# liron88/HM-16.2

Hardware: AMD Instinct MI355X
Metric: CTUs/sec (enc) at 4K main10; bit-exact CU partition vs HM (higher is better)
Workload: dtype int32+f64

## Files before the change

### __graft_entry__.py

```python
import os
import subprocess
import sys

ROOT = os.path.dirname(os.path.abspath(__file__))
PKG = os.path.join(ROOT, "hm-16.2_amd")
for p in (ROOT, PKG, os.path.join(ROOT, "oracle")):
    if p not in sys.path:
        sys.path.insert(0, p)


def _newer(target, sources):
    if not os.path.exists(target):
        return True
    t = os.path.getmtime(target)
    return any(os.path.getmtime(s) > t for s in sources)


def build_product():
    src = os.path.join(PKG, "csrc")
    out = os.path.join(PKG, "libhm355.so")
    deps = [os.path.join(src, f) for f in ("hm355.hip", "hm355_core.h", "hm355_inter.h", "hm355_inter_cu.h", "hm355_dbk.h", "hm355_sao.h", "hm355_bits.h", "hm355_bits_kernel.h", "hm355_ingest.h", "hm355_picstat.h", "hm355_types.h", "hm355_host_common.h", "hm355_simt.h", "hm355_simt4.h", "hm355_simt8.h", "hm355_team.h")] + [os.path.join(ROOT, "include", "hm355.h")]
    if _newer(out, deps):
        import hashlib
        h = hashlib.sha1()
        for d in sorted(deps):
            h.update(open(d, "rb").read())
        build_id = h.hexdigest()[:12]
        hipcc = "/opt/rocm/bin/hipcc" if os.path.exists("/opt/rocm/bin/hipcc") else "hipcc"
        cmd = [hipcc, "-O3", "--offload-arch=gfx950", "-ffp-contract=off", "-fPIC", "-shared", "-std=c++17", "-Wno-unused-value", "-Wno-sizeof-array-div",
               f'-DHM355_BUILD_ID="{build_id}"', "-o", out, os.path.join(src, "hm355.hip")]
        subprocess.run(cmd, check=True)
    host = os.path.join(PKG, "host")
    exe = os.path.join(PKG, "hm355_encmain")
    if _newer(exe, [os.path.join(host, f) for f in ("encmain.cpp", "TEncTop.cpp", "TEncTop.h")] + [out]):
        subprocess.run(["g++", "-O2", "-std=c++14", "-Wall", "-o", exe, os.path.join(host, "encmain.cpp"), os.path.join(host, "TEncTop.cpp"),
                        "-L" + PKG, "-lhm355", "-Wl,-rpath,$ORIGIN"], check=True)
    return out


def build_oracle():
    subprocess.run(["make", "-s", "-C", os.path.join(ROOT, "oracle"),
                    os.path.join(ROOT, "oracle", "libhm_oracle.so"), os.path.join(ROOT, "oracle", "hm_oracle_cli")], check=True)
    if os.path.isdir("/root/reference/source"):
        subprocess.run(["make", "-s", "-C", os.path.join(ROOT, "oracle"), "ref"], check=True, stdout=subprocess.DEVNULL)


def build():
    build_product()
    build_oracle()
    import hm355
    hm355.load_library()


def smoke():
    import numpy as np
    import hm355
    import oracle
    import synth
    w, h, bd, qp = 128, 64, 8, 32
    planes = synth.frame(w, h, bd, 0, 1234)
    enc = hm355.Encoder(w, h, bd, 1, 1)
    (rec, ctus, stats), = enc.compress([planes], qp)
    (subs, nxt, bins), = enc.encode_slices_run([dict(slice_type=2, qp=qp)])
    pstat, = enc.picture_stats_run([dict(hash_method=1)])
    enc.close()
    import hashlib
    for k in range(3):
        d = planes[k].astype(np.int64) - rec[k].astype(np.int64)
        assert pstat["ssd"][k] == int((d * d).sum()), "smoke: SSD of the picture statistics differs from numpy"
        assert pstat["digest"][k] == hashlib.md5(rec[k].astype(np.uint8).tobytes()).digest(), "smoke: MD5 of the reconstruction differs from hashlib"
    want_rec, want_ctus = oracle.compress(planes, bd, qp, 1)
    for f in ("total_bits", "total_dist", "depth", "part_size", "intra_dir_luma", "intra_dir_chroma", "tr_idx", "cbf", "coeff_y"):
        assert np.array_equal(ctus[f], want_ctus[f]), f"smoke: {f} differs from the oracle"
    for k in range(3):
        assert np.array_equal(rec[k], want_rec[k]), "smoke: reconstruction differs from the oracle"
    want_subs, want_nxt, want_bins = oracle.encode_slice(w, h, bd, 1, 2, qp, want_ctus)
    assert subs == want_subs and (nxt, bins) == (want_nxt, want_bins), "smoke: slice data differs from the oracle"
    print("smoke ok: 2 CTUs,", int(stats[0]), "bits,", sum(len(x) for x in subs), "bytes of slice data, bit-exact vs oracle;" + pstat["psnr_string"], "MD5", pstat["digest_string"][:32])
    import math
    n = len(ctus)
    mot = np.zeros(n, [("pred_mode", "u1", 256), ("mv0", "<i2", (256, 2)), ("ref_idx0", "i1", 256), ("mv1", "<i2", (256, 2)), ("ref_idx1", "i1", 256)])
    mot["pred_mode"] = 1; mot["ref_idx0"] = -1; mot["ref_idx1"] = -1
    ref_poc = np.zeros((2, 16), np.int32)
    final = {"poc": 0, "slice_type": 2, "rec": rec, "motion": mot, "num_ref_idx": (0, 0), "ref_poc": ref_poc, "ref_long_term": ref_poc}
    lam = 0.578 * 2.0 ** ((qp + 2 - 12) / 3.0) * 2.0
    srec = {"poc": 1, "slice_type": 0, "qp": qp + 2, "lambda": lam, "weight_cb": hm355.intra_lambda(qp + 2)[1], "cabac_init_type": 0,
            "num_ref_idx": (1, 1), "ref_poc": ref_poc, "col_from_l0": 1, "col_ref_idx": 0, "tmvp": 1, "mvd_l1_zero": 1, "max_merge_cand": 5,
            "check_ldc": 1, "lambda_motion_sad": int(math.floor(65536.0 * math.sqrt(lam))), "lambda_motion_sse": int(math.floor(65536.0 * lam))}
    cur = synth.frame(w, h, bd, 1, 1234)
    want_rec, want_ctus, want_ictus = oracle.compress_inter(cur, bd, srec, {0: final}, wpp=1)
    sp = dict(srec); sp["chroma_weight"] = srec["weight_cb"]
    refs = {0: dict(slice_type=2, rec=rec, pred_mode=mot["pred_mode"], mv=[mot["mv0"], mot["mv1"]], ref_idx=[mot["ref_idx0"], mot["ref_idx1"]],
                    num_ref_idx=(0, 0), ref_poc=ref_poc, ref_long_term=ref_poc)}
    enc = hm355.Encoder(w, h, bd, 1, 1)
    brec, bctus, bictus, bstats = enc.compress_inter(cur, sp, refs)
    (bsubs, bnxt, bbins), = enc.encode_slices_run([dict(slice_type=0, qp=qp + 2, cabac_init_type=0, num_ref_idx=(1, 1), mvd_l1_zero=1, max_merge_cand=5)])
    enc.close()
    for f in ("total_bits", "total_dist", "depth", "part_size", "pred_mode", "tr_idx", "cbf", "coeff_y"):
        assert np.array_equal(bctus[f], want_ctus[f]), f"smoke (B slice): {f} differs from the oracle"
    for f in ("skip", "merge_flag", "merge_idx", "inter_dir", "mv", "mvd", "ref_idx", "mvp_idx"):
        assert np.array_equal(bictus[f], want_ictus[f]), f"smoke (B slice): {f} differs from the oracle"
    for k in range(3):
        assert np.array_equal(brec[k], want_rec[k]), "smoke (B slice): reconstruction differs from the oracle"
    want_bsubs, want_bnxt, want_bbins = oracle.encode_slice(w, h, bd, 1, 0, qp + 2, want_ctus, want_ictus, cabac_init_type=0, num_ref_idx=(1, 1), mvd_l1_zero=1, max_merge_cand=5)
    assert bsubs == want_bsubs and (bnxt, bbins) == (want_bnxt, want_bbins), "smoke (B slice): slice data differs from the oracle"
    print("smoke ok: B slice,", int(bstats[0]), "bits,", sum(len(x) for x in bsubs), "bytes of slice data,", int((bictus["inter_dir"] == 3).sum()), "bi-predicted partitions, bit-exact vs oracle")


if __name__ == "__main__":
    build()
    if len(sys.argv) > 1 and sys.argv[1] == "smoke":
        smoke()
```

### hm-16.2_amd/csrc/hm355_core.h

```cpp
#pragma once
#include <stddef.h>
#include "hm355_types.h"

#ifdef HM355_HOSTSIM
#include <string.h>
#include <math.h>
#include <stdlib.h>
#define HM_DEV static
#define HM_FINL static inline
#define HM_FINL_M inline
#define HM_LAMBDA_INL
#define HM_NOINLINE __attribute__((noinline))
#define HM_CONST static const
#define HM_ASSUME_LDS(p) ((void)0)
#define HM_ASSUME_GLB(p) ((void)0)
#define HM_NT 1
static inline int hm_lane() { return 0; }
#define HM_SYNC() ((void)0)
static inline uint32_t hm_wave_sum(uint32_t v) { return v; }
static inline int hm_wave_sum_i(int v) { return v; }
static inline int hm_wave_max_i(int v) { return v; }
#define HM_UNI(x) (x)
#define HM_UCALL(x) (x)
#define hm_uni_ptr(p) (p)
#define hm_uni_struct(v) (v)
#define HM_ENTRY(e) ((void)0)
#define HM_LDS_ADD(p, v) (*(p) += (v))
#ifdef HM355_HOSTSIM_REVERSE
#define HM_PAR_FOR_XY(x, y, w, n) for (int i_ = (n) - 1, y = i_ / (w), x = i_ - y * (w); i_ >= 0; i_--, x--, (x < 0 ? (x = (w) - 1, y--) : 0))
#define HM_PAR_FOR(i, n) for (int i = (n) - 1; i >= 0; i--)
#define HM_WAVE_FOR(k) for (int k = 63; k >= 0; k--)
#else
#define HM_PAR_FOR_XY(x, y, w, n) for (int i_ = 0, y = 0, x = 0; i_ < (n); i_++, x++, (x >= (w) ? (x = 0, y++) : 0))
#define HM_PAR_FOR(i, n) for (int i = 0; i < (n); i++)
#define HM_WAVE_FOR(k) for (int k = 0; k < 64; k++)
#endif
#define HM_LV(T, name) T name[64]
#define HM_LVARG(T, name) const T *name
#define HM_LVK(name, k) name[k]
#define HM_LV_GET(name, i) (name[i])
#define HM_LV_GETD(name, i) (name[i])
#define HM_LV_SET(name, i, v) (name[i] = (v))
#define HM_LV_SETD(name, i, v) (name[i] = (v))
#define HM_LV_GATHER(name, idx) (name[idx])
#define HM_BALLOT(m, k, cond) do { if (cond) (m) |= 1ull << (k); } while (0)
#define HM_ORDERED_ADD16(acc, name) do { for (int k_ = 15; k_ >= 0; k_--) (acc) += name[k_]; } while (0)
#define HM_ORDERED_CHAIN16(acc, a, b, pre) do { for (int k_ = 15; k_ >= 0; k_--) { pre[k_] = (acc); (acc) -= a[k_]; (acc) += b[k_]; } } while (0)
#else
#define HM_DEV __device__
#define HM_FINL __device__ __forceinline__
#define HM_FINL_M __device__ __forceinline__
#define HM_LAMBDA_INL __attribute__((always_inline))
#define HM_NOINLINE __attribute__((noinline))
#define HM_CONST __device__ const
#if defined(__HIP_DEVICE_COMPILE__)
#define HM_ASSUME_LDS(p) __builtin_assume(__builtin_amdgcn_is_shared((const void *)(p)))
#define HM_ASSUME_GLB(p) __builtin_assume(!__builtin_amdgcn_is_shared((const void *)(p)) && !__builtin_amdgcn_is_private((const void *)(p)))
#else
#define HM_ASSUME_LDS(p) ((void)0)
#define HM_ASSUME_GLB(p) ((void)0)
#endif
#define HM_NT 64
__device__ __forceinline__ int hm_lane() { return (int)(threadIdx.x & 63u); }
#define HM_SYNC() do { __builtin_amdgcn_fence(__ATOMIC_RELEASE, "wavefront"); __builtin_amdgcn_wave_barrier(); __builtin_amdgcn_fence(__ATOMIC_ACQUIRE, "wavefront"); } while (0)
template <int CTRL> __device__ __forceinline__ int hm_dpp(int old, int v) { return __builtin_amdgcn_update_dpp(old, v, CTRL, 0xf, 0xf, false); }
__device__ __forceinline__ int hm_wave_sum_i(int v)
{
  v += hm_dpp<0x111>(0, v); v += hm_dpp<0x112>(0, v); v += hm_dpp<0x114>(0, v); v += hm_dpp<0x118>(0, v);
  return __builtin_amdgcn_readlane(v, 15) + __builtin_amdgcn_readlane(v, 31) + __builtin_amdgcn_readlane(v, 47) + __builtin_amdgcn_readlane(v, 63);
}
__device__ __forceinline__ uint32_t hm_wave_sum(uint32_t v) { return (uint32_t)hm_wave_sum_i((int)v); }
__device__ __forceinline__ int hm_wave_max_i(int v)
{
  int t;
  t = hm_dpp<0x111>(v, v); v = t > v ? t : v; t = hm_dpp<0x112>(v, v); v = t > v ? t : v;
  t = hm_dpp<0x114>(v, v); v = t > v ? t : v; t = hm_dpp<0x118>(v, v); v = t > v ? t : v;
  const int a = __builtin_amdgcn_readlane(v, 15), b = __builtin_amdgcn_readlane(v, 31), c = __builtin_amdgcn_readlane(v, 47), d = __builtin_amdgcn_readlane(v, 63);
  const int ab = a > b ? a : b, cd = c > d ? c : d;
  return ab > cd ? ab : cd;
}
#define HM_LDS_ADD(p, v) atomicAdd((p), (v))
#define HM_UNI(x) __builtin_amdgcn_readfirstlane((int)(x))
template <class T> __device__ __forceinline__ T *hm_uni_ptr(T *p)
{
  const unsigned long long v = (unsigned long long)p;
  const unsigned lo = (unsigned)__builtin_amdgcn_readfirstlane((int)(unsigned)v), hi = (unsigned)__builtin_amdgcn_readfirstlane((int)(unsigned)(v >> 32));
  return (T *)(((unsigned long long)hi << 32) | lo);
}
template <class T> __device__ __forceinline__ T hm_uni_struct(T v)
{
  static_assert(sizeof(T) % 4 == 0, "dword-sized aggregates only");
  int w[sizeof(T) / 4];
  __builtin_memcpy(w, &v, sizeof(T));
#pragma unroll
  for (unsigned i = 0; i < sizeof(T) / 4; i++) w[i] = __builtin_amdgcn_readfirstlane(w[i]);
  __builtin_memcpy(&v, w, sizeof(T));
  return v;
}
#define HM_ENTRY(e) do { (e) = hm_uni_ptr(e); HM_ASSUME_LDS(e); } while (0)
#define HM_UCALL(x) ((uint32_t)__builtin_amdgcn_readfirstlane((int)(x)))
#define HM_PAR_FOR(i, n) for (int i = hm_lane(); i < (n); i += HM_NT)
#define HM_PAR_FOR_XY(x, y, w, n) \
  for (int i_ = hm_lane(), sy_ = HM_NT / (w), sx_ = HM_NT - sy_ * (w), y = i_ / (w), x = i_ - y * (w); i_ < (n); \
       i_ += HM_NT, x += sx_, y += sy_, (x >= (w) ? (x -= (w), y++) : 0))
#define HM_WAVE_FOR(k) for (int k = hm_lane(), k##_once = 1; k##_once; k##_once = 0)
#define HM_LV(T, name) T name
#define HM_LVARG(T, name) const T name
#define HM_LVK(name, k) name
#define HM_LV_GET(name, i) __builtin_amdgcn_readlane((int)(name), (int)(i))
#define HM_LV_GETD(name, i) hm_readlane_d((name), (int)(i))
#define HM_LV_SET(name, i, v) ((name) = (hm_lane() == (int)(i)) ? (v) : (name))
#define HM_LV_SETD(name, i, v) ((name) = (hm_lane() == (int)(i)) ? (v) : (name))
#define HM_LV_GATHER(name, idx) __builtin_amdgcn_ds_bpermute((int)(idx) << 2, (int)(name))
#define HM_BALLOT(m, k, cond) ((m) = __ballot(cond))
#define HM_ORDERED_ADD16(acc, name) do { _Pragma("unroll") for (int k_ = 15; k_ >= 0; k_--) (acc) += hm_readlane_d((name), k_); } while (0)
#define HM_ORDERED_CHAIN16(acc, a, b, pre) do { _Pragma("unroll") for (int k_ = 15; k_ >= 0; k_--) { \
    (pre) = (hm_lane() == k_) ? (acc) : (pre); (acc) -= hm_readlane_d((a), k_); (acc) += hm_readlane_d((b), k_); } } while (0)
__device__ __forceinline__ double hm_readlane_d(double v, int i)
{ return __hiloint2double(__builtin_amdgcn_readlane(__double2hiint(v), i), __builtin_amdgcn_readlane(__double2loint(v), i)); }
#endif

#if defined(HM355_PROFILE) && !defined(HM355_HOSTSIM)
#define HM_PROF_N 44
#define HM_PROF_BEGIN(e, id) const unsigned long long prof_t0_##id = __builtin_readcyclecounter()
#define HM_PROF_END(e, id) do { (e)->prof[id] += __builtin_readcyclecounter() - prof_t0_##id; (e)->profCnt[id] += 1; } while (0)
#else
#define HM_PROF_BEGIN(e, id) ((void)0)
#define HM_PROF_END(e, id) ((void)0)
#endif
enum { PR_RDOQ = 0, PR_BITS, PR_ADI, PR_PRED, PR_FWD, PR_INV, PR_SATD35, PR_TUBLK, PR_SAVE, PR_CHROMA, PR_LUMA, PR_ENCCU, PR_TOTAL,
       PR_S4L = 32, PR_S4C, PR_D0, PR_D1, PR_D2, PR_D3, PR_NXN, PR_S8L, PR_S4LEAF, PR_S4CLEAF, PR_S8C,
       PR_ME_INT = 16, PR_ME_FRAC, PR_AMVP, PR_MRG_EST, PR_MC, PR_IRQ, PR_IRES, PR_MRG2N, PR_INTERCU, PR_INTRA_IN_P, PR_IQ_FULL, PR_IQ_FWD, PR_IQ_RDOQ, PR_IQ_BITS, PR_IQ_INV, PR_IQ_ENC };

#define HM_MAX_DOUBLE 1.7e+308
#define PLANAR_IDX 0
#define DC_IDX 1
#define HOR_IDX 10
#define VER_IDX 26
#define DM_CHROMA_IDX 36
#define SIZE_2Nx2N 0
#define SIZE_NxN 3
#define SIZE_NONE 8
#define MODE_INTRA 1
#define MODE_NONE 2
#define SCAN_DIAG 0
#define SCAN_HOR 1
#define SCAN_VER 2

HM_CONST uint8_t HM_NEXT_LPS[128] __attribute__((aligned(4))) = {
  1, 0, 0, 1, 2, 3, 4, 5, 4, 5, 8, 9, 8, 9, 10, 11, 12, 13, 14, 15, 16, 17, 18, 19, 18, 19, 22, 23, 22, 23, 24, 25,
  26, 27, 26, 27, 30, 31, 30, 31, 32, 33, 32, 33, 36, 37, 36, 37, 38, 39, 38, 39, 42, 43, 42, 43, 44, 45, 44, 45, 46, 47, 48, 49,
  48, 49, 50, 51, 52, 53, 52, 53, 54, 55, 54, 55, 56, 57, 58, 59, 58, 59, 60, 61, 60, 61, 60, 61, 62, 63, 64, 65, 64, 65, 66, 67,
  66, 67, 66, 67, 68, 69, 68, 69, 70, 71, 70, 71, 70, 71, 72, 73, 72, 73, 72, 73, 74, 75, 74, 75, 74, 75, 76, 77, 76, 77, 126, 127 };
HM_CONST int32_t HM_ENTROPY_BITS[128] = {
  0x07b23, 0x085f9, 0x074a0, 0x08cbc, 0x06ee4, 0x09354, 0x067f4, 0x09c1b, 0x060b0, 0x0a62a, 0x05a9c, 0x0af5b, 0x0548d, 0x0b955, 0x04f56, 0x0c2a9,
  0x04a87, 0x0cbf7, 0x045d6, 0x0d5c3, 0x04144, 0x0e01b, 0x03d88, 0x0e937, 0x039e0, 0x0f2cd, 0x03663, 0x0fc9e, 0x03347, 0x10600, 0x03050, 0x10f95,
  0x02d4d, 0x11a02, 0x02ad3, 0x12333, 0x0286e, 0x12cad, 0x02604, 0x136df, 0x02425, 0x13f48, 0x021f4, 0x149c4, 0x0203e, 0x1527b, 0x01e4d, 0x15d00,
  0x01c99, 0x166de, 0x01b18, 0x17017, 0x019a5, 0x17988, 0x01841, 0x18327, 0x016df, 0x18d50, 0x015d9, 0x19547, 0x0147c, 0x1a083, 0x0138e, 0x1a8a3,
  0x01251, 0x1b418, 0x01166, 0x1bd27, 0x01068, 0x1c77b, 0x00f7f, 0x1d18e, 0x00eda, 0x1d91a, 0x00e19, 0x1e254, 0x00d4f, 0x1ec9a, 0x00c90, 0x1f6e0,
  0x00c01, 0x1fef8, 0x00b5f, 0x208b1, 0x00ab6, 0x21362, 0x00a15, 0x21e46, 0x00988, 0x2285d, 0x00934, 0x22ea8, 0x008a8, 0x239b2, 0x0081d, 0x24577,
  0x007c9, 0x24ce6, 0x00763, 0x25663, 0x00710, 0x25e8f, 0x006a0, 0x26a26, 0x00672, 0x26f23, 0x005e8, 0x27ef8, 0x005ba, 0x284b5, 0x0055e, 0x29057,
  0x0050c, 0x29bab, 0x004c1, 0x2a674, 0x004a7, 0x2aa5e, 0x0046f, 0x2b32f, 0x0041f, 0x2c0ad, 0x003e7, 0x2ca8d, 0x003ba, 0x2d323, 0x0010c, 0x3bfbb };
HM_CONST uint8_t HM_CTX_INIT_I[HM_NUM_CTX] = {
   139, 141, 157,
   184, 154, 154, 154,
   184,
   63, 139,
   153, 138, 138,
   111, 141, 154, 154, 154,   94, 138, 182, 154, 154,
   91, 171, 134, 141,
   111, 111, 125, 110, 110, 94, 124, 108, 124, 107, 125, 141, 179, 153, 125, 107, 125, 141, 179, 153, 125, 107, 125, 141, 179, 153, 125, 141,
   140, 139, 182, 182, 152, 136, 152, 136, 153, 136, 139, 111, 136, 139, 111, 111,
   110, 110, 124, 125, 140, 153, 125, 127, 140, 109, 111, 143, 127, 111, 79,  108, 123, 63, 154, 154, 154, 154, 154, 154, 154, 154, 154, 154, 154, 154,
   110, 110, 124, 125, 140, 153, 125, 127, 140, 109, 111, 143, 127, 111, 79,  108, 123, 63, 154, 154, 154, 154, 154, 154, 154, 154, 154, 154, 154, 154,
   140, 92, 137, 138, 140, 152, 138, 139, 153, 74, 149, 92, 139, 107, 122, 152,  140, 179, 166, 182, 140, 227, 122, 197,
   138, 153, 136, 167, 152, 152,
   139, 139,
   154, 154, 154,  154, 154,  154,  154, 154, 154, 154, 154,  154, 154,
   154, 154,  154,  154,  154, 154, 154
};
HM_CONST uint8_t HM_CTX_INIT_P[HM_NUM_CTX] = {
   107, 139, 126,
   154, 139, 154, 154,
   154,
   152, 139,
   124, 138, 94,
   153, 111, 154, 154, 154,   149, 107, 167, 154, 154,
   121, 140, 61, 154,
   155, 154, 139, 153, 139, 123, 123, 63, 153, 166, 183, 140, 136, 153, 154, 166, 183, 140, 136, 153, 154, 166, 183, 140, 136, 153, 154, 140,
   170, 153, 123, 123, 107, 121, 107, 121, 167, 151, 183, 140, 151, 183, 140, 140,
   125, 110, 94, 110, 95, 79, 125, 111, 110, 78, 110, 111, 111, 95, 94,  108, 123, 108, 154, 154, 154, 154, 154, 154, 154, 154, 154, 154, 154, 154,
   125, 110, 94, 110, 95, 79, 125, 111, 110, 78, 110, 111, 111, 95, 94,  108, 123, 108, 154, 154, 154, 154, 154, 154, 154, 154, 154, 154, 154, 154,
   154, 196, 196, 167, 154, 152, 167, 182, 182, 134, 149, 136, 153, 121, 136, 137,  169, 194, 166, 167, 154, 167, 137, 182,
   107, 167, 91, 122, 107, 167,
   139, 139,
   197, 185, 201,  110, 122,  149,  95, 79, 63, 31, 31,  140, 198,
   153, 153,  79,  168,  154, 154, 154
};
HM_CONST uint8_t HM_CTX_INIT_B[HM_NUM_CTX] = {
   107, 139, 126,
   154, 139, 154, 154,
   183,
   152, 139,
   224, 167, 122,
   153, 111, 154, 154, 154,   149, 92, 167, 154, 154,
   121, 140, 61, 154,
   170, 154, 139, 153, 139, 123, 123, 63, 124, 166, 183, 140, 136, 153, 154, 166, 183, 140, 136, 153, 154, 166, 183, 140, 136, 153, 154, 140,
   170, 153, 138, 138, 122, 121, 122, 121, 167, 151, 183, 140, 151, 183, 140, 140,
   125, 110, 124, 110, 95, 94, 125, 111, 111, 79, 125, 126, 111, 111, 79,  108, 123, 93, 154, 154, 154, 154, 154, 154, 154, 154, 154, 154, 154, 154,
   125, 110, 124, 110, 95, 94, 125, 111, 111, 79, 125, 126, 111, 111, 79,  108, 123, 93, 154, 154, 154, 154, 154, 154, 154, 154, 154, 154, 154, 154,
   154, 196, 167, 167, 154, 152, 167, 182, 182, 134, 149, 136, 153, 121, 136, 122,  169, 208, 166, 167, 154, 152, 167, 182,
   107, 167, 91, 107, 107, 167,
   139, 139,
   197, 185, 201,  154, 137,  134,  95, 79, 63, 31, 31,  169, 198,
   153, 153,  79,  168,  154, 154, 154
};
HM_CONST int8_t HM_DCT_C[33] = {64, 90, 90, 90, 89, 88, 87, 85, 83, 82, 80, 78, 75, 73, 70, 67, 64, 61, 57, 54, 50, 46, 43, 38, 36, 31, 25, 22, 18, 13, 9, 4, 0};
HM_CONST int8_t HM_DST4[16] = {29, 55, 74, 84, 74, 74, 0, -74, 84, -29, -74, 55, 55, -84, 74, -29};
HM_CONST int32_t HM_QUANT_SCALES[6] = {26214, 23302, 20560, 18396, 16384, 14564};
HM_CONST int32_t HM_INV_QUANT_SCALES[6] = {40, 45, 51, 57, 64, 72};
HM_CONST uint8_t HM_GROUP_IDX[32] = {0,1,2,3,4,4,5,5,6,6,6,6,7,7,7,7,8,8,8,8,8,8,8,8,9,9,9,9,9,9,9,9};
HM_CONST uint8_t HM_CTX_IND_MAP_4x4[16] = {0,1,4,5, 2,3,4,5, 6,6,8,8, 7,7,8,8};
HM_CONST uint8_t HM_INTRA_MODE_NUM_FAST[6] = {3, 8, 8, 3, 3, 3};
HM_CONST uint8_t HM_INTRA_FILTER[5] = {10, 7, 1, 0, 10};
HM_CONST int8_t HM_ANG_TABLE[9] = {0, 2, 5, 9, 13, 17, 21, 26, 32};
HM_CONST int16_t HM_INV_ANG_TABLE[9] = {0, 4096, 1638, 910, 630, 482, 390, 315, 256};

struct TU {
  int16_t cuParts, parts, cParts, cOff;
  uint8_t cuZ, cuDepth, relZ, trDepth, log2, section, x, y;
  uint8_t cW, cCodeAll, cTrDepth, cRelZ, cx, cy, pad_[2];
};
static_assert(sizeof(TU) == 24, "TU layout");
struct TuWalk { TU node[5]; int8_t next[5]; int sp; };
struct RqtFrame {
  TU t; int8_t phase, child, checkFull, checkSplit, bestModeId; uint32_t singleDist, singleCbf, splitDist, splitCbf, singleBits; double singleCost, splitCost;
};
struct CuFrame { int16_t cuZ; int8_t phase, sub, boundary, parentPart, ampSens, pad_; double bestCost, splitCost; uint32_t bestBits, bestDist, splitBits, splitDist; };
struct MvFieldD { MvD mv; int ref; };
struct MergeList { MvFieldD f[5][2]; uint8_t dir[5]; int num; };
struct AmvpInfo { MvD cand[3]; int n; };
struct TZ {
  const Pel *org; int orgStride, w, h;
  const Pel *ref; int refStride;
  uint32_t bestSad; int bestX, bestY, bestDist, bestRound, pointNr;
  int16_t l, r, t, b;
  int16_t subShift, pad_;
  int16_t lx[16], ly[16]; int8_t lp[16], ld[16];
  int16_t wx0, wy0, ww, wh;
};
struct IrqFrame {
  TU t; int8_t phase, child, checkFull, checkSplit, zero; uint8_t bestTS[3];
  uint32_t absSum[3], bestCBF[3], singleBits, singleDist, subBits, subDist; double singleCost, subCost;
};

#define HM_TSTRIDE 33
#define HM_RQ_LDS 256
struct RqLds {
  int32_t lvl[HM_RQ_LDS];
  uint16_t pos[HM_RQ_LDS];
  uint16_t dec[HM_RQ_LDS];
  int16_t cur[HM_RQ_LDS];
  uint8_t ctxSig[HM_RQ_LDS];
  uint8_t code[HM_RQ_LDS];
  uint8_t cgCtxSet[64];
  uint8_t cgFlag[64];
};
struct RefLds {
  Pel refTop[2][132], refLeft[2][132];
  Pel refMain[200], refSide[200];
  Pel line[272];
};
#define HM_SLOT(d, ci) ((d) * CI_NUM + (ci) - ((d) == 4 ? 2 : 0))
#define HM_NUM_SLOTS (4 * CI_NUM + 3)
struct Team;
#define HM_CTU_WAVES 12
struct LdsTables {
  int8_t tmat[32 * HM_TSTRIDE];
  int8_t dst4[16];
  int32_t ebits[128];
};
#if defined(HM355_HOSTSIM)
static LdsTables g_lt;
#else
__shared__ LdsTables g_lt;
#endif
#define HM_LT() (&g_lt)
struct Shared {
  Cabac cur;
  int32_t bufA[32 * HM_TSTRIDE];
  union {
    int32_t bufB[32 * HM_TSTRIDE];
    RqLds rq;
    RefLds ref;
  } u;
  TuWalk walkOuter, walkInner;
  CuFrame cuf[4];
  double outCost; uint32_t outBits, outDist; double outRdCost;
  int32_t mpmZ;
  int32_t s8Winner, s8Reuse;
  InterMeta *im;
  uint32_t mcost; MvD mvPredictor; int32_t costScale;
  union {
    struct {
      uint8_t flags[72];
      RqtFrame rqt[4]; uint32_t rqtRetDist[5], rqtRetBits[5]; double rqtRetCost[5];
      int32_t rdModeList[12];
      uint32_t outDistY;
      uint32_t satd[36];
      int32_t mpmNum, mpmPreds[3];
    };
    struct {
      int32_t absCoeff[10];
      TZ tz; MvD outMv; MergeList ml; AmvpInfo amvp; MvFieldD mrgField[2]; int32_t mrgDir, mrgIdx; uint32_t mrgCost, irqZeroDist;
      IrqFrame irq[4];
    };
  };
  int32_t width, height, bitDepth, wCtu, stride[3];
  const Params *P; FrameBuf fb; WorkSpace *ws; const Tables *tab;
  CtuMeta meta;
  TCoeff *cc;
  int32_t ctuX, ctuY, ctuAddr;
#if defined(HM355_PROFILE) && !defined(HM355_HOSTSIM)
  unsigned long long prof[HM_PROF_N]; unsigned long long profCnt[HM_PROF_N];
#endif
};

#if defined(HM355_TRACE) && defined(HM355_HOSTSIM)
#include <stdio.h>
static FILE *g_hm_trace;
#define HM_TRACE(e, tag, a, b, c) do { if (g_hm_trace) fprintf(g_hm_trace, "%d %d %u %u %.3f\n", (int)(tag), (e)->ctuAddr, (unsigned)(a), (unsigned)(b), (double)(c)); } while (0)
#elif defined(HM355_TRACE)
#define HM_TRACE_CAP (1u << 21)
__device__ inline void hm_trace(Shared *e, int tag, uint32_t a, uint32_t b, double c)
{
  if (hm_lane() == 0) {
    unsigned long long *t = e->P->prof; const unsigned long long n = atomicAdd(t, 1ull);
    if (n < HM_TRACE_CAP) { t[1 + n * 3] = ((unsigned long long)(uint32_t)tag << 32) | (uint32_t)e->ctuAddr; t[2 + n * 3] = ((unsigned long long)a << 32) | b; t[3 + n * 3] = (unsigned long long)__double_as_longlong(c); }
  }
}
#define HM_TRACE(e, tag, a, b, c) hm_trace((e), (tag), (uint32_t)(a), (uint32_t)(b), (double)(c))
#else
#define HM_TRACE(e, tag, a, b, c) ((void)0)
#endif

#ifndef HM355_HOSTSIM
__shared__ Shared g_sh;
__shared__ Shared g_shs[HM_CTU_WAVES];
#endif
#if !defined(HM355_PROFILE)
static_assert(HM_CTU_WAVES * (sizeof(Shared) + 16) + sizeof(LdsTables) <= 163840 / (12 / HM_CTU_WAVES) && sizeof(Shared) % 8 == 0, "two workgroups of HM_CTU_WAVES searches (+ work items, + the shared tables) per CU: 12 CTU searches in 160 KB of LDS");
#endif
static_assert(offsetof(Shared, bufA) % 8 == 0 && (16 * HM_TSTRIDE * 4) % 8 == 0, "the RDOQ cost array aliases the lower half of bufA as doubles");
static_assert(offsetof(Shared, u) == offsetof(Shared, bufA) + sizeof(((Shared *)0)->bufA), "the motion search stages its reference window across bufA and the union behind it");
#define HM_TZ_WIN_SAMPLES ((int)((sizeof(((Shared *)0)->bufA) + sizeof(((Shared *)0)->u)) / sizeof(Pel)))

HM_DEV inline int hm_clip3(int lo, int hi, int v) { return v < lo ? lo : (v > hi ? hi : v); }
HM_DEV inline int hm_abs(int v) { return v < 0 ? -v : v; }
HM_DEV inline int hm_z2r(int z)
{
  const int x = (z & 1) | ((z >> 1) & 2) | ((z >> 2) & 4) | ((z >> 3) & 8);
  const int y = ((z >> 1) & 1) | ((z >> 2) & 2) | ((z >> 3) & 4) | ((z >> 4) & 8);
  return (y << 4) | x;
}
HM_DEV inline int hm_spread4(int v) { return (v & 1) | ((v & 2) << 1) | ((v & 4) << 2) | ((v & 8) << 3); }
HM_DEV inline int hm_r2z(int r) { return hm_spread4(r & 15) | (hm_spread4(r >> 4) << 1); }
HM_DEV inline int hm_log2(int n) { return n >= 64 ? 6 : (n >= 32 ? 5 : (n >= 16 ? 4 : (n >= 8 ? 3 : 2))); }

HM_DEV inline void par_set8(uint8_t *p, int v, int n) { HM_PAR_FOR(i, n) p[i] = (uint8_t)v; HM_SYNC(); }
HM_DEV inline void par_copy8(uint8_t *d, const uint8_t *s, int n) { HM_PAR_FOR(i, n) d[i] = s[i]; HM_SYNC(); }
HM_DEV inline void par_copy32(TCoeff *d, const TCoeff *s, int n) { HM_PAR_FOR(i, n) d[i] = s[i]; HM_SYNC(); }
HM_DEV inline void par_zero32(TCoeff *d, int n) { HM_PAR_FOR(i, n) d[i] = 0; HM_SYNC(); }
HM_DEV inline void par_copy_blk(Pel *d, int ds, const Pel *s, int ss, int n)
{
  const int l2 = hm_log2(n);
  HM_PAR_FOR(i, n * n) { const int y = i >> l2, x = i & (n - 1); d[y * ds + x] = s[y * ss + x]; }
  HM_SYNC();
}

HM_DEV inline void cabac_copy(Cabac *d, const Cabac *s)
{
  const uint64_t *sp = (const uint64_t *)s; uint64_t *dp = (uint64_t *)d;
  HM_PAR_FOR(i, (int)(sizeof(Cabac) / 8)) dp[i] = sp[i];
  HM_SYNC();
}
#if defined(HM355_HOSTSIM)
typedef Cabac CabacHold;
static inline CabacHold cabac_hold(const Cabac *s) { return *s; }
static inline void cabac_put(Cabac *d, const CabacHold &h) { *d = h; }
#else
typedef uint64_t CabacHold;
__device__ __forceinline__ CabacHold cabac_hold(const Cabac *s)
{ const int l = hm_lane(); return l < (int)(sizeof(Cabac) / 8) ? ((const uint64_t *)s)[l] : 0ull; }
__device__ __forceinline__ void cabac_put(Cabac *d, CabacHold h)
{ const int l = hm_lane(); if (l < (int)(sizeof(Cabac) / 8)) ((uint64_t *)d)[l] = h; HM_SYNC(); }
#endif
HM_DEV inline void cabac_init(Cabac *c, int qp, int initType = 2)
{
  qp = hm_clip3(0, 51, qp);
  HM_PAR_FOR(i, HM_NUM_CTX) {
    const int iv = initType == 2 ? HM_CTX_INIT_I[i] : (initType == 1 ? HM_CTX_INIT_P[i] : HM_CTX_INIT_B[i]);
    const int slope = (iv >> 4) * 5 - 45, offset = ((iv & 15) << 3) - 16;
    int st = ((slope * qp) >> 4) + offset; st = st < 1 ? 1 : (st > 126 ? 126 : st);
    const int mps = st >= 64;
    c->s[i] = (uint8_t)(((mps ? (st - 64) : (63 - st)) << 1) + mps);
  }
  c->frac = 0;
  HM_SYNC();
}
HM_DEV inline int hm_next_state(int st, int bin) { return bin == (st & 1) ? (st < 124 ? st + 2 : st) : HM_NEXT_LPS[st]; }
HM_DEV inline void enc_bin(const Shared *e, Cabac *c, int ctx, int bin)
{
  const int st = c->s[ctx];
  c->frac += (uint64_t)HM_LT()->ebits[st ^ bin];
  c->s[ctx] = hm_next_state(st, bin);
}
HM_DEV inline void enc_ep(Cabac *c, int n) { c->frac += (uint64_t)32768 * (uint64_t)n; }
HM_DEV inline void enc_trm(const Shared *e, Cabac *c, int bin) { c->frac += (uint64_t)HM_ENTROPY_BITS[126 ^ bin]; }
HM_DEV inline void reset_bits(Cabac *c) { c->frac &= 32767; }
HM_DEV inline uint32_t num_bits(const Cabac *c) { return (uint32_t)(c->frac >> 15); }

HM_DEV inline double calc_rd_cost(const Shared *e, uint32_t bits, uint32_t dist)
{
  const double t = (double)bits * e->fb.lambda;
  const double u = (double)dist + t;
  return floor(u + 0.5);
}

struct Rect;
template <class C> HM_DEV inline void code_skip_flag(Shared *e, C *c, int z);

HM_DEV inline uint32_t dist_sse(const Pel *org, int so, const Pel *cur, int sc, int n, int bitDepth)
{
  const int shift = (bitDepth - 8) << 1, l2 = hm_log2(n);
  uint32_t sum = 0;
  HM_PAR_FOR(i, n * n) { const int y = i >> l2, x = i & (n - 1); const int d = org[y * so + x] - cur[y * sc + x]; sum += (uint32_t)((d * d) >> shift); }
  return hm_wave_sum(sum);
}
HM_DEV inline uint32_t had8(const Pel *org, int so, const Pel *cur, int sc)
{
  int d[64];
#pragma unroll
  for (int y = 0; y < 8; y++)
#pragma unroll
    for (int x = 0; x < 8; x++) d[y * 8 + x] = org[y * so + x] - cur[y * sc + x];
#pragma unroll
  for (int y = 0; y < 8; y++) {
#pragma unroll
    for (int len = 1; len < 8; len <<= 1)
#pragma unroll
      for (int b = 0; b < 8; b += len << 1)
#pragma unroll
        for (int k = 0; k < len; k++) { const int a0 = d[y * 8 + b + k], a1 = d[y * 8 + b + k + len]; d[y * 8 + b + k] = a0 + a1; d[y * 8 + b + k + len] = a0 - a1; }
  }
  uint32_t s = 0;
#pragma unroll
  for (int x = 0; x < 8; x++) {
#pragma unroll
    for (int len = 1; len < 8; len <<= 1)
#pragma unroll
      for (int b = 0; b < 8; b += len << 1)
#pragma unroll
        for (int k = 0; k < len; k++) { const int a0 = d[(b + k) * 8 + x], a1 = d[(b + k + len) * 8 + x]; d[(b + k) * 8 + x] = a0 + a1; d[(b + k + len) * 8 + x] = a0 - a1; }
#pragma unroll
    for (int y = 0; y < 8; y++) s += (uint32_t)hm_abs(d[y * 8 + x]);
  }
  return (s + 2) >> 2;
}
HM_DEV inline uint32_t had4(const Pel *org, int so, const Pel *cur, int sc)
{
  int d[16];
#pragma unroll
  for (int y = 0; y < 4; y++)
#pragma unroll
    for (int x = 0; x < 4; x++) d[y * 4 + x] = org[y * so + x] - cur[y * sc + x];
#pragma unroll
  for (int y = 0; y < 4; y++) {
    const int a = d[y * 4] + d[y * 4 + 1], b = d[y * 4] - d[y * 4 + 1], c = d[y * 4 + 2] + d[y * 4 + 3], e = d[y * 4 + 2] - d[y * 4 + 3];
    d[y * 4] = a + c; d[y * 4 + 1] = b + e; d[y * 4 + 2] = a - c; d[y * 4 + 3] = b - e;
  }
  uint32_t s = 0;
#pragma unroll
  for (int x = 0; x < 4; x++) {
    const int a = d[x] + d[4 + x], b = d[x] - d[4 + x], c = d[8 + x] + d[12 + x], e = d[8 + x] - d[12 + x];
    s += (uint32_t)(hm_abs(a + c) + hm_abs(b + e) + hm_abs(a - c) + hm_abs(b - e));
  }
  return (s + 1) >> 1;
}
HM_DEV inline uint32_t dist_hads(const Pel *org, int so, const Pel *cur, int sc, int n, int bitDepth)
{
  uint32_t sum = 0; const int l2 = hm_log2(n);
  if (n >= 8) { const int nb = n >> 3; HM_PAR_FOR(b, nb * nb) { const int by = b >> (l2 - 3), bx = b & (nb - 1); sum += had8(org + by * 8 * so + bx * 8, so, cur + by * 8 * sc + bx * 8, sc); } }
  else { HM_PAR_FOR(b, 1) sum += had4(org, so, cur, sc); }
  return hm_wave_sum(sum) >> (bitDepth - 8);
}
HM_DEV inline uint32_t dist_sad(const Pel *org, int so, const Pel *cur, int sc, int n, int subShift, int bitDepth)
{
  const int l2 = hm_log2(n), rows = n >> subShift;
  uint32_t sum = 0;
  HM_PAR_FOR(i, rows * n) { const int y = (i >> l2) << subShift, x = i & (n - 1); sum += (uint32_t)hm_abs(org[y * so + x] - cur[y * sc + x]); }
  return (hm_wave_sum(sum) << subShift) >> (bitDepth - 8);
}

HM_DEV inline void load_tables()
{
  HM_PAR_FOR(i, 1024) {
    const int k = i >> 5, n = i & 31, m = (k * (2 * n + 1)) & 127;
    int v;
    if (m <= 32) v = HM_DCT_C[m]; else if (m <= 64) v = -HM_DCT_C[64 - m]; else if (m <= 96) v = -HM_DCT_C[m - 64]; else v = HM_DCT_C[128 - m];
    HM_LT()->tmat[k * HM_TSTRIDE + n] = (int8_t)v;
  }
  HM_PAR_FOR(i, 16) HM_LT()->dst4[i] = HM_DST4[i];
  HM_PAR_FOR(i, 128) HM_LT()->ebits[i] = HM_ENTROPY_BITS[i];
  HM_SYNC();
}
HM_DEV inline int tm(const Shared *e, int n, int dst, int k, int j) { return dst ? HM_LT()->dst4[k * 4 + j] : HM_LT()->tmat[(k * (32 / n)) * HM_TSTRIDE + j]; }

HM_DEV inline void fold_rows(int32_t *X, int n, int l2)
{
  const int h = n >> 1, q = n >> 2;
  HM_PAR_FOR(o, n * q) {
    const int j = o >> (l2 - 2), i = o & (q - 1);
    int32_t *r = X + j * HM_TSTRIDE;
    const int32_t a = r[i], b = r[n - 1 - i], c = r[h - 1 - i], d = r[h + i];
    r[i] = a + b; r[h + i] = a - b; r[h - 1 - i] = c + d; r[n - 1 - i] = c - d;
  }
  HM_SYNC();
}
HM_DEV HM_NOINLINE void fwd_transform(Shared *e, int n, int useDst, int bitDepth)
{
  HM_ENTRY(e); n = HM_UNI(n); useDst = HM_UNI(useDst); bitDepth = HM_UNI(bitDepth);
  const int l2 = hm_log2(n), s1 = l2 + bitDepth + 6 - 15, s2 = l2 + 6;
  const int a1 = s1 > 0 ? 1 << (s1 - 1) : 0, a2 = 1 << (s2 - 1);
  int32_t *A = e->bufA, *B = e->u.bufB;
  if (useDst) {
    HM_PAR_FOR(o, n * n) {
      const int j = o >> l2, k = o & (n - 1);
      int32_t acc = 0;
      for (int i = 0; i < n; i++) acc += tm(e, n, 1, k, i) * A[j * HM_TSTRIDE + i];
      B[k * HM_TSTRIDE + j] = (acc + a1) >> s1;
    }
    HM_SYNC();
    HM_PAR_FOR(o, n * n) {
      const int j = o >> l2, k = o & (n - 1);
      int32_t acc = 0;
      for (int i = 0; i < n; i++) acc += tm(e, n, 1, k, i) * B[j * HM_TSTRIDE + i];
      A[k * HM_TSTRIDE + j] = (acc + a2) >> s2;
    }
    HM_SYNC();
    return;
  }
  const int h = n >> 1, step = 32 / n;
  fold_rows(A, n, l2);
  HM_PAR_FOR(o, n * n) {
    const int j = o >> l2, k = o & (n - 1);
    const int32_t *x = A + j * HM_TSTRIDE + ((k & 1) ? h : 0); const int8_t *t = HM_LT()->tmat + (k * step) * HM_TSTRIDE;
    int32_t acc = 0;
    for (int i = 0; i < h; i++) acc += t[i] * x[i];
    B[k * HM_TSTRIDE + j] = (acc + a1) >> s1;
  }
  HM_SYNC();
  fold_rows(B, n, l2);
  HM_PAR_FOR(o, n * n) {
    const int j = o >> l2, k = o & (n - 1);
    const int32_t *x = B + j * HM_TSTRIDE + ((k & 1) ? h : 0); const int8_t *t = HM_LT()->tmat + (k * step) * HM_TSTRIDE;
    int32_t acc = 0;
    for (int i = 0; i < h; i++) acc += t[i] * x[i];
    A[k * HM_TSTRIDE + j] = (acc + a2) >> s2;
  }
  HM_SYNC();
}
HM_DEV HM_NOINLINE void inv_transform(Shared *e, int n, int useDst, int bitDepth)
{
  HM_ENTRY(e); n = HM_UNI(n); useDst = HM_UNI(useDst); bitDepth = HM_UNI(bitDepth);
  const int l2 = hm_log2(n), s1 = 7, s2 = 20 - bitDepth;
  int32_t *A = e->bufA, *B = e->u.bufB;
  if (useDst) {
    HM_PAR_FOR(o, n * n) {
      const int j = o >> l2, i = o & (n - 1);
      int32_t acc = 0;
      for (int k = 0; k < n; k++) acc += tm(e, n, 1, k, i) * A[k * HM_TSTRIDE + j];
      B[j * HM_TSTRIDE + i] = hm_clip3(-32768, 32767, (acc + (1 << (s1 - 1))) >> s1);
    }
    HM_SYNC();
    HM_PAR_FOR(o, n * n) {
      const int j = o >> l2, i = o & (n - 1);
      int32_t acc = 0;
      for (int k = 0; k < n; k++) acc += tm(e, n, 1, k, i) * B[k * HM_TSTRIDE + j];
      A[j * HM_TSTRIDE + i] = hm_clip3(-32768, 32767, (acc + (1 << (s2 - 1))) >> s2);
    }
    HM_SYNC();
    return;
  }
  const int h = n >> 1, step = 32 / n;
  HM_PAR_FOR(o, n * h) {
    const int j = o >> (l2 - 1), i = o & (h - 1);
    int32_t ev = 0, od = 0;
    for (int k = 0; k < n; k += 2) { ev += HM_LT()->tmat[(k * step) * HM_TSTRIDE + i] * A[k * HM_TSTRIDE + j]; od += HM_LT()->tmat[((k + 1) * step) * HM_TSTRIDE + i] * A[(k + 1) * HM_TSTRIDE + j]; }
    B[j * HM_TSTRIDE + i] = hm_clip3(-32768, 32767, (ev + od + (1 << (s1 - 1))) >> s1);
    B[j * HM_TSTRIDE + n - 1 - i] = hm_clip3(-32768, 32767, (ev - od + (1 << (s1 - 1))) >> s1);
  }
  HM_SYNC();
  HM_PAR_FOR(o, n * h) {
    const int j = o >> (l2 - 1), i = o & (h - 1);
    int32_t ev = 0, od = 0;
    for (int k = 0; k < n; k += 2) { ev += HM_LT()->tmat[(k * step) * HM_TSTRIDE + i] * B[k * HM_TSTRIDE + j]; od += HM_LT()->tmat[((k + 1) * step) * HM_TSTRIDE + i] * B[(k + 1) * HM_TSTRIDE + j]; }
    A[j * HM_TSTRIDE + i] = hm_clip3(-32768, 32767, (ev + od + (1 << (s2 - 1))) >> s2);
    A[j * HM_TSTRIDE + n - 1 - i] = hm_clip3(-32768, 32767, (ev - od + (1 << (s2 - 1))) >> s2);
  }
  HM_SYNC();
}

HM_DEV inline TU tu_root(const Shared *e, int cuZ, int cuDepth)
{
  TU t;
  t.cuZ = (int16_t)cuZ; t.cuDepth = (int16_t)cuDepth; t.cuParts = (int16_t)(256 >> (2 * cuDepth));
  t.relZ = 0; t.trDepth = 0; t.log2 = (int16_t)(6 - cuDepth); t.parts = t.cuParts; t.section = 0;
  const int r = hm_z2r(cuZ);
  t.x = (int16_t)((r & 15) * 4); t.y = (int16_t)((r >> 4) * 4);
  t.cW = (int16_t)(1 << (t.log2 - 1)); t.cCodeAll = 1; t.cTrDepth = 0; t.cRelZ = 0; t.cParts = t.parts; t.cOff = (int16_t)(cuZ * 4);
  t.cx = t.x >> 1; t.cy = t.y >> 1;
  return t;
}
HM_DEV inline TU tu_child(const TU *p, int section, int processLast)
{
  TU t = *p;
  t.log2 = p->log2 - 1; t.trDepth = p->trDepth + 1; t.parts = p->parts >> 2; if (t.parts < 1) t.parts = 1;
  t.relZ = (int16_t)(p->relZ + section * t.parts); t.section = (int16_t)section;
  t.x = (int16_t)(p->x + (section & 1) * (1 << t.log2)); t.y = (int16_t)(p->y + (section >> 1) * (1 << t.log2));
  if (t.log2 >= 3) {
    t.cW = (int16_t)(1 << (t.log2 - 1)); t.cCodeAll = 1; t.cTrDepth = t.trDepth; t.cRelZ = t.relZ; t.cParts = t.parts;
    t.cOff = (int16_t)((t.cuZ + t.relZ) * 4); t.cx = t.x >> 1; t.cy = t.y >> 1;
  } else {
    t.cCodeAll = 0; t.cTrDepth = p->cTrDepth; t.cRelZ = t.relZ & ~3; t.cParts = (int16_t)(t.parts * 4);
    t.cOff = p->cOff; t.cx = p->cx; t.cy = p->cy;
    t.cW = (section == (processLast ? 3 : 0)) ? 4 : 0;
  }
  return t;
}
template <class Enter, class Leave> HM_FINL void tu_walk(TuWalk &w, const TU *root, int processLast, Enter enter, Leave leave)
{
  w.node[0] = *root; w.next[0] = -1; w.sp = 0;
  while (w.sp >= 0) {
    TU *t = &w.node[w.sp];
    if (w.next[w.sp] < 0) { if (!enter((const TU *)t)) { w.sp--; continue; } w.next[w.sp] = 0; }
    if (w.next[w.sp] == 4) { leave((const TU *)t); w.sp--; continue; }
    const int s = w.next[w.sp]++;
    w.node[w.sp + 1] = tu_child(t, s, processLast); w.next[w.sp + 1] = -1; w.sp++;
  }
}
template <class Enter> HM_FINL void tu_walk(TuWalk &w, const TU *root, int processLast, Enter enter) { tu_walk(w, root, processLast, enter, [](const TU *) {}); }

HM_DEV inline const CtuMeta *meta_at(const Shared *e, int x4, int y4, int *z)
// ... 853 lines not shown
    HM_LV(int32_t, vCtx); HM_LV(int32_t, vAbs);
    uint64_t nz = 0, g1 = 0, g2 = 0, ng = 0;
    HM_WAVE_FOR(k) {
      const int kk = k & 15, sp = subPos + kk;
      const int a = (kk <= top) ? hm_abs((int)lv[sp]) : 0;
      if (real) HM_BALLOT(ng, k, kk <= top && lv[sp] < 0 && k < 16);
      HM_LVK(vAbs, k) = a;
      HM_LVK(vCtx, k) = sig_ctx_inc(pattern, firstCtx, sposArr[sp], log2n, chroma);
      HM_BALLOT(nz, k, a != 0 && k < 16); HM_BALLOT(g1, k, a > 1 && k < 16); HM_BALLOT(g2, k, a > 2 && k < 16);
    }
    HM_BPROF(PR_SATD35);
    {
      int seen = isLastSet ? 1 : 0;
      for (int p = isLastSet ? top - 1 : 15; p >= 0; p--) {
        const int sig = (int)((nz >> p) & 1);
        if (p > 0 || subSet == 0 || seen) enc_bin(e, &r, sigOff + HM_LV_GET(vCtx, p), sig);
        seen += sig;
      }
    }
    HM_BPROF(PR_TUBLK);
    const int numNonZero = __builtin_popcountll(nz);
    if (numNonZero > 0) {
      const int lastNZ = 63 - __builtin_clzll(nz), firstNZ = __builtin_ctzll(nz);
      const int signHidden = (lastNZ - firstNZ >= 4);
      const int ctxSet = ctx_set_index(chroma, subSet, c1 == 0);
      c1 = 1;
      int firstC2 = -1, escape = 0, idx = 0;
      for (uint64_t m = nz; m && idx < 8; idx++) {
        const int p = 63 - __builtin_clzll(m); m &= ~(1ull << p);
        const int sym = (int)((g1 >> p) & 1);
        enc_bin(e, &r, C_ONE + 4 * ctxSet + c1, sym);
        if (sym) { c1 = 0; if (firstC2 == -1) firstC2 = p; else escape = 1; }
        else if (c1 < 3 && c1 > 0) c1++;
      }
      if (c1 == 0 && firstC2 != -1) { const int sym = (int)((g2 >> firstC2) & 1); enc_bin(e, &r, C_ABS + ctxSet, sym); if (sym) escape = 1; }
      escape = escape || (numNonZero > 8);
      uint32_t signs = 0;
      if (real) { for (uint64_t m = nz; m;) { const int p = 63 - __builtin_clzll(m); m &= ~(1ull << p); signs = (signs << 1) | (uint32_t)((ng >> p) & 1); } if (signHidden) signs >>= 1; }
      enc_epv(&r, signs, signHidden ? numNonZero - 1 : numNonZero);
      if (escape) {
        int firstCoeff2 = 1; uint32_t goRice = 0; idx = 0;
        for (uint64_t m = nz; m; idx++) {
          const int p = 63 - __builtin_clzll(m); m &= ~(1ull << p);
          const int a = HM_LV_GET(vAbs, p);
          const int baseLevel = (idx < 8) ? (2 + firstCoeff2) : 1;
          if (a >= baseLevel) {
            uint32_t sym = (uint32_t)(a - baseLevel);
            if (sym < (3u << goRice)) { const uint32_t len = sym >> goRice; enc_epv(&r, (((1u << (len + 1)) - 2) << goRice) | (sym & ((1u << goRice) - 1)), (int)(len + 1 + goRice)); }
            else { sym -= (3u << goRice); const uint32_t len = coef_remain_suffix(&sym, goRice);
                   if (real) { enc_epv(&r, (1u << (3 + len + 1 - goRice)) - 2, (int)(3 + len + 1 - goRice)); enc_epv(&r, sym, (int)len); }
                   else enc_epv(&r, 0, (int)(3 + len + 1 - goRice + len)); }
            if ((uint32_t)a > (3u << goRice)) goRice = goRice + 1 < 4 ? goRice + 1 : 4;
          }
          if (a >= 2) firstCoeff2 = 0;
        }
      }
    }
    HM_BPROF(PR_CHROMA);
  }
  cabr_store(r, c);
#if defined(HM355_PROFILE) && !defined(HM355_HOSTSIM)
  if (real) { e->prof[PR_FWD] += __builtin_readcyclecounter() - profT0; e->profCnt[PR_FWD] += 1; }
#endif
}


template <class C> HM_DEV inline void code_intra_dir_luma(Shared *e, C *c, int z, int multiple)
{
  const CtuMeta *m = (&e->meta);
  const int partNum = multiple ? (m->part[z] == SIZE_NxN ? 4 : 1) : 1;
  const int partOffset = (256 >> (m->depth[z] << 1)) >> 2;
  int predIdx[4] = {-1, -1, -1, -1};
  for (int j = 0; j < partNum; j++) {
    int preds[3];
    const int dir = m->dirL[z + partOffset * j];
    if (!multiple && z == e->mpmZ) { preds[0] = e->mpmPreds[0]; preds[1] = e->mpmPreds[1]; preds[2] = e->mpmPreds[2]; }
    else intra_dir_predictor(e, z + partOffset * j, preds);
    for (int i = 0; i < 3; i++) if (dir == preds[i]) predIdx[j] = i;
    enc_bin(e, c, C_INTRA_LUMA, predIdx[j] != -1);
  }
  for (int j = 0; j < partNum; j++) {
    if (predIdx[j] != -1) { if (predIdx[j]) enc_epv(c, 2u | (uint32_t)(predIdx[j] - 1), 2); else enc_epv(c, 0, 1); }
    else {
      uint32_t rem = 0;
      if (EngOf<C>::REAL) {
        int p[3]; intra_dir_predictor(e, z + partOffset * j, p);
        int d = m->dirL[z + partOffset * j];
        rem = (uint32_t)(d - (d > p[0]) - (d > p[1]) - (d > p[2]));
      }
      enc_epv(c, rem, 5);
    }
  }
}
template <class C> HM_DEV inline void code_intra_dir_chroma(Shared *e, C *c, int z)
{
  if ((&e->meta)->dirC[z] == DM_CHROMA_IDX) enc_bin(e, c, C_CHROMA_PRED, 0);
  else {
    enc_bin(e, c, C_CHROMA_PRED, 1);
    uint32_t idx = 0;
    if (EngOf<C>::REAL) {
      const int luma = (&e->meta)->dirL[z], dc = (&e->meta)->dirC[z];
      const int list[4] = { PLANAR_IDX, VER_IDX, HOR_IDX, DC_IDX };
      for (int i = 3; i >= 0; i--) if ((list[i] == luma ? 34 : list[i]) == dc) idx = (uint32_t)i;
    }
    enc_epv(c, idx, 2);
  }
}
template <class C> HM_DEV inline void code_qt_cbf(Shared *e, C *c, const TU *t, int comp, int lowestLevel)
{
  const int z = t->cuZ + (comp ? t->cRelZ : t->relZ);
  const int ctx = comp ? t->trDepth : (t->trDepth == 0 ? 1 : 0);
  const int width = comp ? (1 << (t->log2 - 1)) : (1 << t->log2);
  const int canQuadSplit = width >= 8;
  const int lowestTUDepth = t->trDepth + ((!lowestLevel && !canQuadSplit) ? 1 : 0);
  enc_bin(e, c, C_QT_CBF + (comp ? 5 : 0) + ctx, ((&e->meta)->cbf[comp][z] >> lowestTUDepth) & 1);
}

HM_DEV inline int tr_min_size_in_cu(int cuLog2, int nxn)
{
  if (cuLog2 < 2 + 3 - 1 + nxn) return 2;
  const int v = cuLog2 - (3 - 1 + nxn);
  return v > 5 ? 5 : v;
}
HM_DEV inline int codes_subdiv_flag(const CtuMeta *m, const TU *t, int intra)
{
  const int nxn = intra && m->part[t->cuZ] == SIZE_NxN;
  if (nxn && t->trDepth == 0) return 0;
  if (t->log2 > 5) return 0;
  if (t->log2 == 2) return 0;
  if (t->log2 == tr_min_size_in_cu(6 - t->cuDepth, nxn)) return 0;
  return 1;
}
template <class C> HM_DEV inline void code_chroma_cbfs(Shared *e, C *c, const TU *t, int subdiv)
{
  const CtuMeta *m = (&e->meta); const int z = t->cuZ + t->relZ;
  for (int comp = 1; comp < 3; comp++)
    if (t->trDepth == 0 || (t->cCodeAll && ((m->cbf[comp][z] >> (t->trDepth - 1)) & 1))) code_qt_cbf(e, c, t, comp, subdiv == 0);
}
template <class C> HM_DEV inline void code_tu_coeff(Shared *e, C *c, const TU *t, int comp, const TCoeff *planes, int intra)
{
  const CtuMeta *m = (&e->meta); const int z = t->cuZ + t->relZ;
  if ((comp && !t->cW) || !((m->cbf[comp][z] >> t->trDepth) & 1)) return;
  const int n = comp ? t->cW : (1 << t->log2), zc = t->cuZ + (comp ? t->cRelZ : t->relZ);
  const TCoeff *coef = planes + HM_PLANE_OFF(comp) + (comp ? t->cOff : z * 16);
  code_coeff_nxn(e, c, coef, n, comp, intra ? coef_scan_idx(m, zc, n, comp) : SCAN_DIAG, m->ts[comp][zc]);
}

template <class C> HM_DEV inline void enc_subdiv_cbf_qt(Shared *e, C *c, const TU *root, int bLuma, int bChroma)
{
  const CtuMeta *m = (&e->meta);
  tu_walk(e->walkInner, root, 0, [&](const TU *t) {
    const int subdiv = m->tr[t->cuZ + t->relZ] > t->trDepth;
    if (bLuma && codes_subdiv_flag(m, t, 1)) enc_bin(e, c, C_SUBDIV + (5 - t->log2), subdiv);
    if (bChroma) code_chroma_cbfs(e, c, t, subdiv);
    if (!subdiv && bLuma) code_qt_cbf(e, c, t, 0, 1);
    return subdiv;
  });
}
HM_DEV inline void enc_coeff_qt(Shared *e, const TU *root, int comp)
{
  const CtuMeta *m = (&e->meta);
  tu_walk(e->walkInner, root, 0, [&](const TU *t) {
    if (m->tr[t->cuZ + t->relZ] > t->trDepth) return 1;
    code_tu_coeff(e, &e->cur, t, comp, e->ws->qtCoef[5 - t->log2], 1);
    return 0;
  });
}
template <class C> HM_DEV inline void enc_intra_header(Shared *e, C *c, const TU *t, int bLuma, int bChroma)
{
  const CtuMeta *m = (&e->meta); const int relZ = t->relZ;
  if (bLuma) {
    if (relZ == 0 && e->im) { code_skip_flag(e, c, t->cuZ); enc_bin(e, c, C_PRED_MODE, 1); }
    if (relZ == 0 && t->cuDepth == 3) enc_bin(e, c, C_PART, m->part[t->cuZ] == SIZE_2Nx2N);
    if (m->part[t->cuZ] == SIZE_2Nx2N) { if (relZ == 0) code_intra_dir_luma(e, c, t->cuZ, 0); }
    else { const int q = t->cuParts >> 2; if (t->trDepth > 0 && (relZ & (q - 1)) == 0) code_intra_dir_luma(e, c, t->cuZ + relZ, 0); }
  }
  if (bChroma && relZ == 0) code_intra_dir_chroma(e, c, t->cuZ + relZ);
}
HM_DEV HM_NOINLINE uint32_t intra_bits_qt(Shared *e, TU tv, int bLuma, int bChroma)
{
  HM_ENTRY(e); bLuma = HM_UNI(bLuma); bChroma = HM_UNI(bChroma); tv = hm_uni_struct(tv);
  const TU *t = &tv;
  HM_PROF_BEGIN(e, PR_BITS);
  {
    CabacR r; cabr_load(e, r, &e->cur);
    r.frac &= 32767;
    enc_intra_header(e, &r, t, bLuma, bChroma);
    enc_subdiv_cbf_qt(e, &r, t, bLuma, bChroma);
    cabr_store(r, &e->cur);
  }
  if (bLuma) enc_coeff_qt(e, t, 0);
  if (bChroma) { enc_coeff_qt(e, t, 1); enc_coeff_qt(e, t, 2); }
  HM_PROF_END(e, PR_BITS);
  return num_bits(&e->cur);
}

HM_DEV HM_NOINLINE uint32_t intra_coding_tu_block(Shared *e, TU tv, int comp, int save1load2)
{
  HM_ENTRY(e); comp = HM_UNI(comp); save1load2 = HM_UNI(save1load2); tv = hm_uni_struct(tv);
  const TU *t = &tv;
  CtuMeta *m = (&e->meta); WorkSpace *ws = e->ws;
  if (comp && !t->cW) return 0;
  const int n = comp ? t->cW : (1 << t->log2), l2 = hm_log2(n);
  const int relZ = comp ? t->cRelZ : t->relZ, z = t->cuZ + relZ;
  const int bx = comp ? t->cx : t->x, by = comp ? t->cy : t->y;
  const int st = HM_PLANE_STRIDE(comp), po = HM_PLANE_OFF(comp);
  const int layer = 5 - t->log2, parts = comp ? t->cParts : t->parts;
  const int ps = e->stride[comp], bitDepth = e->bitDepth;
  const Pel *org = e->fb.org[comp] + (e->ctuY * st + by) * ps + e->ctuX * st + bx;
  Pel *recPic = e->fb.rec[comp] + (e->ctuY * st + by) * ps + e->ctuX * st + bx;
  Pel *pred = ws->pred + po + by * st + bx, *resi = ws->resi + po + by * st + bx;
  Pel *recQt = ws->qtRec[layer] + po + by * st + bx;
  TCoeff *coef = ws->qtCoef[layer] + po + (comp ? t->cOff : z * 16);
  const int tskip = m->ts[comp][z];
  int mode = comp ? m->dirC[z] : m->dirL[z];
  if (comp && mode == DM_CHROMA_IDX) mode = m->dirL[z & ~3];
  if (save1load2 != 2) {
    const int filt = use_filtered_refs(comp, mode, n);
    const int r = hm_z2r(z);
    { HM_PROF_BEGIN(e, PR_ADI); init_adi_pattern(e, comp, e->ctuX * st + bx, e->ctuY * st + by, n, e->ctuX * 16 + (r & 15), e->ctuY * 16 + (r >> 4), comp ? n / 2 : n / 4, filt); HM_PROF_END(e, PR_ADI); }
    { HM_PROF_BEGIN(e, PR_PRED); pred_intra(e, comp, mode, n, filt, pred, st); HM_PROF_END(e, PR_PRED); }
    if (save1load2 == 1) { HM_PAR_FOR(i, 16) e->ws->tsPred[comp][i] = pred[(i >> 2) * st + (i & 3)]; HM_SYNC(); }
  } else { HM_PAR_FOR(i, 16) pred[(i >> 2) * st + (i & 3)] = e->ws->tsPred[comp][i]; HM_SYNC(); }
  if (comp == 0) par_set8(m->tr + z, t->trDepth, parts);
  const int tshift = 15 - bitDepth - l2;
  HM_PAR_FOR(i, n * n) {
    const int y = i >> l2, x = i & (n - 1);
    const int r = org[y * ps + x] - pred[y * st + x];
    resi[y * st + x] = (Pel)r;
    e->bufA[y * HM_TSTRIDE + x] = tskip ? r * (1 << tshift) : r;
  }
  HM_SYNC();
  { HM_PROF_BEGIN(e, PR_FWD); if (!tskip) fwd_transform(e, n, comp == 0 && n == 4, bitDepth); HM_PROF_END(e, PR_FWD); }
  const int cbfCtx = comp ? 5 + t->trDepth : (t->trDepth == 0 ? 1 : 0);
  HM_PROF_BEGIN(e, PR_RDOQ);
  const int absSum = rdoq_is_empty(e, n, comp) ? 0 : (int)HM_UCALL(rdoq(e, coef, n, comp, coef_scan_idx(m, z, n, comp), cbfCtx));
  HM_PROF_END(e, PR_RDOQ);
#if defined(HM355_PROFILE) && !defined(HM355_HOSTSIM)
  { const int pid = l2 == 2 ? (absSum ? 13 : 7) : (l2 == 3 ? 14 : (l2 == 4 ? 15 : 43)); e->prof[pid] += __builtin_readcyclecounter() - prof_t0_PR_RDOQ; e->profCnt[pid] += 1; }
#endif
  par_set8(m->cbf[comp] + z, (absSum > 0 ? 1 : 0) << t->trDepth, parts);
  HM_PROF_BEGIN(e, PR_INV);
  if (absSum > 0) {
    const int rightShift = 6 - (tshift + e->fb.qpPer[comp != 0]);
    const int scale = HM_INV_QUANT_SCALES[e->fb.qpRem[comp != 0]];
    int tgt = 25 + rightShift; if (tgt > 16) tgt = 16;
    const int imin = -(1 << (tgt - 1)), imax = (1 << (tgt - 1)) - 1;
    HM_PAR_FOR(i, n * n) {
      const int y = i >> l2, x = i & (n - 1);
      const int c = hm_clip3(imin, imax, coef[i]);
      int v;
      if (rightShift > 0) v = (c * scale + (1 << (rightShift - 1))) >> rightShift;
      else v = (int)((unsigned)(c * scale) << (-rightShift));
      e->bufA[y * HM_TSTRIDE + x] = hm_clip3(-32768, 32767, v);
    }
    HM_SYNC();
    if (!tskip) inv_transform(e, n, comp == 0 && n == 4, bitDepth);
    const int off = tshift == 0 ? 0 : (1 << (tshift - 1));
    HM_PAR_FOR(i, n * n) {
      const int y = i >> l2, x = i & (n - 1);
      const int v = e->bufA[y * HM_TSTRIDE + x];
      resi[y * st + x] = (Pel)(tskip ? ((v + off) >> tshift) : v);
    }
  } else {
    HM_PAR_FOR(i, n * n) { const int y = i >> l2, x = i & (n - 1); coef[i] = 0; resi[y * st + x] = 0; }
  }
  HM_SYNC();
  HM_PROF_END(e, PR_INV);
  const int maxv = (1 << bitDepth) - 1, shiftSse = (bitDepth - 8) << 1;
  uint32_t sse = 0;
  HM_PAR_FOR(i, n * n) {
    const int y = i >> l2, x = i & (n - 1);
    const int r = hm_clip3(0, maxv, pred[y * st + x] + resi[y * st + x]);
    pred[y * st + x] = (Pel)r; recQt[y * st + x] = (Pel)r; recPic[y * ps + x] = (Pel)r;
    const int d = org[y * ps + x] - r; sse += (uint32_t)((d * d) >> shiftSse);
  }
  uint32_t d = hm_wave_sum(sse);
  HM_SYNC();
  if (comp) d = (uint32_t)(e->fb.chromaWeight * (double)d);
  return d;
}

HM_DEV inline void store_intra_result_qt(Shared *e, const TU *t, int comp)
{
  const int st = HM_PLANE_STRIDE(comp), po = HM_PLANE_OFF(comp), layer = 5 - t->log2;
  const int bx = comp ? t->cx : t->x, by = comp ? t->cy : t->y;
  const TCoeff *coef = e->ws->qtCoef[layer] + po + (comp ? t->cOff : (t->cuZ + t->relZ) * 16);
  const Pel *rq = e->ws->qtRec[layer] + po + by * st + bx;
  HM_PAR_FOR(i, 16) { e->ws->tsCoef[comp][i] = coef[i]; e->ws->tsRec[comp][i] = rq[(i >> 2) * st + (i & 3)]; }
  HM_SYNC();
}
HM_DEV inline void load_intra_result_qt(Shared *e, const TU *t, int comp)
{
  const int st = HM_PLANE_STRIDE(comp), po = HM_PLANE_OFF(comp), layer = 5 - t->log2, ps = e->stride[comp];
  const int bx = comp ? t->cx : t->x, by = comp ? t->cy : t->y;
  TCoeff *coef = e->ws->qtCoef[layer] + po + (comp ? t->cOff : (t->cuZ + t->relZ) * 16);
  Pel *rq = e->ws->qtRec[layer] + po + by * st + bx;
  Pel *recPic = e->fb.rec[comp] + (e->ctuY * st + by) * ps + e->ctuX * st + bx;
  HM_PAR_FOR(i, 16) { coef[i] = e->ws->tsCoef[comp][i]; const Pel v = e->ws->tsRec[comp][i]; rq[(i >> 2) * st + (i & 3)] = v; recPic[(i >> 2) * ps + (i & 3)] = v; }
  HM_SYNC();
}

HM_DEV HM_NOINLINE void simt4_luma_leaf(Shared *e, TU tv);
HM_DEV HM_NOINLINE void simt8_luma_winner_as_single_tu(Shared *e, TU tv);
HM_DEV HM_NOINLINE void recur_intra_coding_qt(Shared *e, TU rootv, int checkFirst)
{
  HM_ENTRY(e); checkFirst = HM_UNI(checkFirst); rootv = hm_uni_struct(rootv);
  CtuMeta *m = (&e->meta);
  RqtFrame *fr = e->rqt; int sp = 0;
  uint32_t *retDist = e->rqtRetDist, *retBits = e->rqtRetBits; double *retCost = e->rqtRetCost;
  fr[0].t = rootv; fr[0].phase = 0; retDist[0] = 0; retBits[0] = 0; retCost[0] = 0.0;
  while (sp >= 0) {
    RqtFrame *f = &fr[sp]; const TU *t = &f->t;
    const int z = t->cuZ + t->relZ, fullDepth = t->cuDepth + t->trDepth, log2 = t->log2;
    if (f->phase == 0) {
      const int nxn = m->part[t->cuZ] == SIZE_NxN;
      f->checkFull = log2 <= 5;
      f->checkSplit = log2 > tr_min_size_in_cu(6 - t->cuDepth, nxn);
      if (checkFirst && f->checkFull) f->checkSplit = 0;
      f->singleCost = HM_MAX_DOUBLE; f->singleDist = 0; f->singleCbf = 0; f->bestModeId = 0; f->singleBits = 0;
      const int checkTS = (log2 == 2) && (m->part[z] == SIZE_NxN);
      if (f->checkFull) {
        if (checkTS) {
          cabac_copy(&e->ws->slot[HM_SLOT(fullDepth, CI_QT_TRAFO_ROOT)], &e->cur);
          for (int modeId = 0; modeId < 2; modeId++) {
            double costTmp;
            par_set8(m->ts[0] + z, modeId, t->parts);
            const uint32_t distTmp = HM_UCALL(intra_coding_tu_block(e, *t, 0, modeId == 0 ? 1 : 2));
            const uint32_t cbfTmp = (m->cbf[0][z] >> t->trDepth) & 1;
            if (modeId == 1 && cbfTmp == 0) costTmp = HM_MAX_DOUBLE;
            else { const uint32_t bits = HM_UCALL(intra_bits_qt(e, *t, 1, 0)); costTmp = calc_rd_cost(e, bits, distTmp); }
            if (costTmp < f->singleCost) {
              f->singleCost = costTmp; f->singleDist = distTmp; f->singleCbf = cbfTmp; f->bestModeId = (int8_t)modeId;
              if (modeId == 0) { store_intra_result_qt(e, t, 0); cabac_copy(&e->ws->slot[HM_SLOT(fullDepth, CI_TEMP_BEST)], &e->cur); }
            }
            if (modeId == 0) cabac_copy(&e->cur, &e->ws->slot[HM_SLOT(fullDepth, CI_QT_TRAFO_ROOT)]);
          }
          par_set8(m->ts[0] + z, f->bestModeId, t->parts);
          if (f->bestModeId == 0) {
            load_intra_result_qt(e, t, 0);
            par_set8(m->cbf[0] + z, (int)(f->singleCbf << t->trDepth), t->parts);
            cabac_copy(&e->cur, &e->ws->slot[HM_SLOT(fullDepth, CI_TEMP_BEST)]);
          }
        } else if (log2 == 2 && e->P->fewWaves) {
          par_set8(m->ts[0] + z, 0, t->parts);
          HM_PROF_BEGIN(e, PR_S4LEAF);
          simt4_luma_leaf(e, *t);
          HM_PROF_END(e, PR_S4LEAF);
          f->singleDist = e->outDistY; f->singleBits = e->outBits;
          f->singleCost = calc_rd_cost(e, e->outBits, f->singleDist);
        } else if (sp == 0 && e->s8Reuse == 1) {
          e->s8Reuse = 0;
          cabac_copy(&e->ws->slot[HM_SLOT(fullDepth, CI_QT_TRAFO_ROOT)], &e->cur);
          par_set8(m->ts[0] + z, 0, t->parts);
          par_set8(m->tr + z, t->trDepth, t->parts);
          simt8_luma_winner_as_single_tu(e, *t);
          f->singleDist = e->outDistY; f->singleCbf = e->outDist;
          par_set8(m->cbf[0] + z, (int)(f->singleCbf << t->trDepth), t->parts);
          f->singleCost = calc_rd_cost(e, e->outBits, f->singleDist);
        } else if (sp == 0 && e->s8Reuse == 2) {
          e->s8Reuse = 0;
          cabac_copy(&e->ws->slot[HM_SLOT(fullDepth, CI_QT_TRAFO_ROOT)], &e->cur);
          par_set8(m->ts[0] + z, 0, t->parts);
          par_set8(m->tr + z, t->trDepth, t->parts);
          {
            const int n = 1 << log2, layer = 5 - log2;
            par_copy32(e->ws->qtCoef[layer] + z * 16, e->cc + z * 16, n * n);
            par_copy_blk(e->ws->qtRec[layer] + t->y * 64 + t->x, 64, e->ws->reco + t->y * 64 + t->x, 64, n);
          }
          f->singleCbf = e->ws->tmpCbf[0][0] & 1;
          par_set8(m->cbf[0] + z, (int)(f->singleCbf << t->trDepth), t->parts);
          f->singleDist = e->outDistY; f->singleCost = e->outRdCost;
          cabac_copy(&e->cur, &e->ws->slot[HM_SLOT(fullDepth, CI_QT_TRAFO_TEST)]);
        } else {
          if (f->checkSplit) cabac_copy(&e->ws->slot[HM_SLOT(fullDepth, CI_QT_TRAFO_ROOT)], &e->cur);
          par_set8(m->ts[0] + z, 0, t->parts);
          f->singleDist = HM_UCALL(intra_coding_tu_block(e, *t, 0, 0));
          if (f->checkSplit) f->singleCbf = (m->cbf[0][z] >> t->trDepth) & 1;
          const uint32_t bits = HM_UCALL(intra_bits_qt(e, *t, 1, 0));
          f->singleCost = calc_rd_cost(e, bits, f->singleDist); f->singleBits = bits;
        }
      }
      if (!f->checkSplit) { retDist[sp] += f->singleDist; retBits[sp] += f->singleBits; retCost[sp] += f->singleCost; sp--; continue; }
      if (f->checkFull) { cabac_copy(&e->ws->slot[HM_SLOT(fullDepth, CI_QT_TRAFO_TEST)], &e->cur); cabac_copy(&e->cur, &e->ws->slot[HM_SLOT(fullDepth, CI_QT_TRAFO_ROOT)]); }
      else cabac_copy(&e->ws->slot[HM_SLOT(fullDepth, CI_QT_TRAFO_ROOT)], &e->cur);
      f->splitCost = 0.0; f->splitDist = 0; f->splitCbf = 0; f->child = 0; f->phase = 1;
      retDist[sp + 1] = 0; retBits[sp + 1] = 0; retCost[sp + 1] = 0.0;
    }
    if (f->phase == 1) {
      int splitLost = 0;
      if (f->child > 0) {
        const TU ch = tu_child(t, f->child - 1, 0);
        f->splitCbf |= (m->cbf[0][ch.cuZ + ch.relZ] >> ch.trDepth) & 1;
        const uint32_t lbBits = retBits[sp + 1] > (uint32_t)f->child ? retBits[sp + 1] - (uint32_t)f->child : 0;
        if (f->checkFull) splitLost = !(calc_rd_cost(e, lbBits, retDist[sp + 1]) < f->singleCost);
        else if (sp == 0 && !(calc_rd_cost(e, lbBits, retDist[1]) < e->outCost)) {
          e->outDistY = 0; e->outRdCost = HM_MAX_DOUBLE; return;
        }
      }
      if (!splitLost) {
        if (f->child < 4) {
          fr[sp + 1].t = tu_child(t, f->child, 0); fr[sp + 1].phase = 0; f->child++;
          sp++; continue;
        }
        f->splitDist = retDist[sp + 1];
        if (f->splitCbf) { HM_PAR_FOR(o, t->parts) m->cbf[0][z + o] |= (uint8_t)(1 << t->trDepth); HM_SYNC(); }
        cabac_copy(&e->cur, &e->ws->slot[HM_SLOT(fullDepth, CI_QT_TRAFO_ROOT)]);
        const uint32_t splitBits = HM_UCALL(intra_bits_qt(e, *t, 1, 0));
        f->splitCost = calc_rd_cost(e, splitBits, f->splitDist);
        if (f->splitCost < f->singleCost) { retDist[sp] += f->splitDist; retBits[sp] += splitBits; retCost[sp] += f->splitCost; sp--; continue; }
      }
      cabac_copy(&e->cur, &e->ws->slot[HM_SLOT(fullDepth, CI_QT_TRAFO_TEST)]);
      par_set8(m->tr + z, t->trDepth, t->parts);
      par_set8(m->cbf[0] + z, (int)(f->singleCbf << t->trDepth), t->parts);
      par_set8(m->ts[0] + z, f->bestModeId, t->parts);
      {
        const int n = 1 << log2, layer = 5 - log2, ps = e->stride[0];
        par_copy_blk(e->fb.rec[0] + (e->ctuY * 64 + t->y) * ps + e->ctuX * 64 + t->x, ps, e->ws->qtRec[layer] + t->y * 64 + t->x, 64, n);
      }
      retDist[sp] += f->singleDist; retBits[sp] += f->singleBits; retCost[sp] += f->singleCost; sp--; continue;
    }
  }
  e->outDistY = retDist[0]; e->outRdCost = retCost[0];
}

HM_DEV inline void set_intra_result_qt(Shared *e, const TU *root)
{
  const CtuMeta *m = (&e->meta);
  for (int rel = root->relZ; rel < root->relZ + root->parts;) {
    const int z = root->cuZ + rel, trd = m->tr[z];
    const int log2 = 6 - root->cuDepth - trd, n = 1 << log2, layer = 5 - log2;
    const int parts = root->cuParts >> (2 * trd) > 0 ? root->cuParts >> (2 * trd) : 1;
    const int r = hm_z2r(z), x = (r & 15) * 4, y = (r >> 4) * 4;
    par_copy32(e->cc + z * 16, e->ws->qtCoef[layer] + z * 16, n * n);
    par_copy_blk(e->ws->reco + y * 64 + x, 64, e->ws->qtRec[layer] + y * 64 + x, 64, n);
    rel += parts;
  }
}

#include "hm355_simt.h"
#include "hm355_simt4.h"
#include "hm355_simt8.h"

HM_DEV HM_NOINLINE uint32_t est_intra_pred_qt(Shared *e, int cuZ, int cuDepth)
{
  HM_ENTRY(e); cuZ = HM_UNI(cuZ); cuDepth = HM_UNI(cuDepth);
  CtuMeta *m = (&e->meta); WorkSpace *ws = e->ws;
  const int cuParts = 256 >> (2 * cuDepth);
  const int nxn = m->part[cuZ] == SIZE_NxN;
  const int numPU = nxn ? 4 : 1, puParts = cuParts / numPU;
  const int puLog2 = 6 - cuDepth - nxn, n = 1 << puLog2;
  const int bitDepth = e->bitDepth, ps = e->stride[0];
  uint32_t overallDistY = 0;
  const TU root = tu_root(e, cuZ, cuDepth);
  for (int pu = 0; pu < numPU; pu++) {
    const TU t = nxn ? tu_child(&root, pu, 0) : root;
    const int z = cuZ + t.relZ;
    int numModesForFullRD = HM_INTRA_MODE_NUM_FAST[puLog2 - 1];
    int32_t *rdModeList = e->rdModeList;
    {
      const int r = hm_z2r(z);
      init_adi_pattern(e, 0, e->ctuX * 64 + t.x, e->ctuY * 64 + t.y, n, e->ctuX * 16 + (r & 15), e->ctuY * 16 + (r >> 4), n / 4, 1);
      const Pel *org = e->fb.org[0] + (e->ctuY * 64 + t.y) * ps + e->ctuX * 64 + t.x;
      Pel *pred = ws->pred + t.y * 64 + t.x;
      int preds[3];
      const int numMpm = intra_dir_predictor(e, z, preds);
      e->mpmZ = z; e->mpmNum = numMpm; e->mpmPreds[0] = preds[0]; e->mpmPreds[1] = preds[1]; e->mpmPreds[2] = preds[2];
      const uint64_t frac0 = e->ws->slot[HM_SLOT(cuDepth, CI_CURR_BEST)].frac & 32767;
      const uint8_t st0 = e->ws->slot[HM_SLOT(cuDepth, CI_CURR_BEST)].s[C_INTRA_LUMA];
      HM_PROF_BEGIN(e, PR_SATD35);
      if (n <= 16) satd_all_modes_small(e, org, ps, n);
      else {
        for (int mode = 0; mode < 35; mode++) {
          pred_intra(e, 0, mode, n, use_filtered_refs(0, mode, n), pred, 64);
          const uint32_t sad = dist_hads(org, ps, pred, 64, n, bitDepth);
          if (hm_lane() == 0) e->satd[mode] = sad;
        }
        HM_SYNC();
      }
      {
        HM_LV(double, vCost);
        HM_WAVE_FOR(k) {
          double cost = HM_MAX_DOUBLE;
          if (k < 35) {
            int predIdx = -1;
            for (int i = 0; i < 3; i++) if (k == preds[i]) predIdx = i;
            uint64_t fb = frac0 + (uint64_t)HM_LT()->ebits[st0 ^ (predIdx != -1)];
            fb += (uint64_t)32768 * (uint64_t)(predIdx == -1 ? 5 : (predIdx ? 2 : 1));
            const uint32_t modeBits = (uint32_t)(fb >> 15);
            cost = (double)e->satd[k] + (double)modeBits * e->fb.sqrtLambda;
          }
          HM_LVK(vCost, k) = cost;
        }
        HM_WAVE_FOR(k) {
          const double ck = HM_LVK(vCost, k);
          int rank = 0;
          for (int j = 0; j < 35; j++) { const double cj = HM_LV_GETD(vCost, j); rank += (cj < ck || (cj == ck && j < k)) ? 1 : 0; }
          if (k < 35 && rank < numModesForFullRD) rdModeList[rank] = k;
        }
        HM_SYNC();
      }
      HM_PROF_END(e, PR_SATD35);
      for (int j = 0; j < numMpm; j++) {
        int included = 0;
        for (int i = 0; i < numModesForFullRD; i++) included |= (preds[j] == rdModeList[i]);
        if (!included) rdModeList[numModesForFullRD++] = preds[j];
      }
    }
    if (n == 4) {
      cabac_copy(&e->cur, &e->ws->slot[HM_SLOT(cuDepth, CI_CURR_BEST)]);
      { HM_PROF_BEGIN(e, PR_S4L); simt4_luma_pu(e, t, numModesForFullRD); HM_PROF_END(e, PR_S4L); }
      overallDistY += e->outDistY;
      if (pu != numPU - 1)
        par_copy_blk(e->fb.rec[0] + (e->ctuY * 64 + t.y) * ps + e->ctuX * 64 + t.x, ps, ws->reco + t.y * 64 + t.x, 64, n);
      continue;
    }
    int bestPUMode = 0; uint32_t bestPUDistY = 0; double bestPUCost = HM_MAX_DOUBLE;
    int firstPass = 0;
    if (n == 8) {
      cabac_copy(&e->cur, &e->ws->slot[HM_SLOT(cuDepth, CI_CURR_BEST)]);
      HM_PROF_BEGIN(e, PR_S8L);
      bestPUMode = HM_UCALL(simt8_luma_first_pass(e, t, numModesForFullRD));
      HM_PROF_END(e, PR_S8L);
      firstPass = numModesForFullRD;
      e->s8Reuse = 1;
    }
    for (int pass = firstPass; pass <= numModesForFullRD; pass++) {
      const int last = (pass == numModesForFullRD);
      const int orgMode = last ? bestPUMode : rdModeList[pass];
      par_set8(m->dirL + z, orgMode, puParts);
      cabac_copy(&e->cur, &e->ws->slot[HM_SLOT(cuDepth, CI_CURR_BEST)]);
      e->outCost = bestPUCost;
      if (last && (n == 16 || n == 32) && numModesForFullRD > 0) { e->s8Reuse = 2; e->outDistY = bestPUDistY; e->outRdCost = bestPUCost; }
      recur_intra_coding_qt(e, t, !last);
      const uint32_t puDistY = e->outDistY; const double puCost = e->outRdCost;
      if (puCost < bestPUCost) {
        bestPUMode = orgMode; bestPUDistY = puDistY; bestPUCost = puCost;
        set_intra_result_qt(e, &t);
        HM_PAR_FOR(i, puParts) { ws->tmpTr[i] = m->tr[z + i]; for (int c = 0; c < 3; c++) { ws->tmpCbf[c][i] = m->cbf[c][z + i]; ws->tmpTs[c][i] = m->ts[c][z + i]; } }
        HM_SYNC();
        if (!last && (n == 16 || n == 32)) cabac_copy(&e->ws->slot[HM_SLOT(cuDepth, CI_QT_TRAFO_TEST)], &e->cur);
      }
    }
    overallDistY += bestPUDistY;
    HM_PAR_FOR(i, puParts) { m->tr[z + i] = ws->tmpTr[i]; for (int c = 0; c < 3; c++) { m->cbf[c][z + i] = ws->tmpCbf[c][i]; m->ts[c][z + i] = ws->tmpTs[c][i]; } m->dirL[z + i] = (uint8_t)bestPUMode; }
    HM_SYNC();
    if (pu != numPU - 1)
      par_copy_blk(e->fb.rec[0] + (e->ctuY * 64 + t.y) * ps + e->ctuX * 64 + t.x, ps, ws->reco + t.y * 64 + t.x, 64, n);
  }
  e->mpmZ = -1;
  if (numPU > 1) {
    uint8_t comb[3] = {0, 0, 0};
    for (int p = 0; p < 4; p++) for (int c = 0; c < 3; c++) comb[c] |= (m->cbf[c][cuZ + p * puParts] >> 1) & 1;
    HM_PAR_FOR(o, cuParts) for (int c = 0; c < 3; c++) m->cbf[c][cuZ + o] |= comb[c];
    HM_SYNC();
  }
  cabac_copy(&e->cur, &e->ws->slot[HM_SLOT(cuDepth, CI_CURR_BEST)]);
  return overallDistY;
}

HM_DEV inline uint32_t chroma_tu(Shared *e, const TU *t)
{
  CtuMeta *m = (&e->meta); const int z = t->cuZ + t->relZ;
  const int fullDepth = t->cuDepth + t->trDepth;
  int checkTS = (t->cW == 4) && (t->log2 == 2);
  if (checkTS) { int nb = 0; for (int s = 0; s < 4; s++) nb += m->ts[0][z + s]; checkTS = nb > 0; }
  const int zc = t->cuZ + t->cRelZ;
  if (t->cW == 4 && !checkTS) {
    cabac_copy(&e->ws->slot[HM_SLOT(fullDepth, CI_QT_TRAFO_ROOT)], &e->cur);
    HM_PROF_BEGIN(e, PR_S4CLEAF);
    const uint32_t d2 = HM_UCALL(simt4_chroma_leaf(e, *t));
    HM_PROF_END(e, PR_S4CLEAF);
    return d2;
  }
  uint32_t dist = 0;
  for (int comp = 1; comp < 3; comp++) {
    cabac_copy(&e->ws->slot[HM_SLOT(fullDepth, CI_QT_TRAFO_ROOT)], &e->cur);
    double singleCost = HM_MAX_DOUBLE, costTmp = 0; uint32_t singleDistC = 0, singleCbfC = 0; int bestTS = 0, bestModeId = 0, currModeId = 0;
    const int total = checkTS ? 2 : 1;
    for (int tsMode = 0; tsMode < total; tsMode++) {
      par_set8(m->ts[comp] + zc, tsMode, t->cParts);
      currModeId++;
      const int isOne = (total == 1), isLast = (currModeId == total);
      const uint32_t distTmp = HM_UCALL(intra_coding_tu_block(e, *t, comp, isOne ? 0 : (tsMode == 0 ? 1 : 2)));
      const uint32_t cbfTmp = (m->cbf[comp][zc] >> t->trDepth) & 1;
      if (tsMode == 1 && cbfTmp == 0) costTmp = HM_MAX_DOUBLE;
      else if (!isOne) { reset_bits(&e->cur); enc_coeff_qt(e, t, comp); costTmp = calc_rd_cost(e, num_bits(&e->cur), distTmp); }
      if (costTmp < singleCost) {
        singleCost = costTmp; singleDistC = distTmp; bestTS = tsMode; bestModeId = currModeId; singleCbfC = cbfTmp;
        if (!isOne && !isLast) { store_intra_result_qt(e, t, comp); cabac_copy(&e->ws->slot[HM_SLOT(fullDepth, CI_TEMP_BEST)], &e->cur); }
      }
      if (!isOne && !isLast) cabac_copy(&e->cur, &e->ws->slot[HM_SLOT(fullDepth, CI_QT_TRAFO_ROOT)]);
    }
    if (bestModeId < total) {
      load_intra_result_qt(e, t, comp);
      par_set8(m->cbf[comp] + zc, (int)(singleCbfC << t->trDepth), t->cParts);
      cabac_copy(&e->cur, &e->ws->slot[HM_SLOT(fullDepth, CI_TEMP_BEST)]);
    }
    par_set8(m->ts[comp] + zc, bestTS, t->cParts);
    dist += singleDistC;
  }
  return dist;
}
HM_DEV HM_NOINLINE uint32_t recur_intra_chroma_coding_qt(Shared *e, TU rootv)
{
  HM_ENTRY(e); rootv = hm_uni_struct(rootv);
  const TU *root = &rootv;
  CtuMeta *m = (&e->meta);
  uint32_t dist = 0;
  tu_walk(e->walkOuter, root, 0,
    [&](const TU *t) {
      if (m->tr[t->cuZ + t->relZ] != t->trDepth) return 1;
      if (t->cW) dist += chroma_tu(e, t);
      return 0;
    },
    [&](const TU *t) {
      const int z = t->cuZ + t->relZ, q = t->parts >> 2;
      int any = 0;
      for (int c = 1; c < 3; c++) for (int s = 0; s < 4; s++) any |= ((m->cbf[c][z + s * q] >> (t->trDepth + 1)) & 1) << c;
      HM_PAR_FOR(o, t->parts) for (int c = 1; c < 3; c++) if ((any >> c) & 1) m->cbf[c][z + o] |= (uint8_t)(1 << t->trDepth);
      HM_SYNC();
    });
  return dist;
}
HM_DEV inline void set_intra_result_chroma_qt(Shared *e, const TU *root)
{
  const CtuMeta *m = (&e->meta);
  tu_walk(e->walkOuter, root, 0, [&](const TU *t) {
    if (!t->cW) return 0;
    if (m->tr[t->cuZ + t->relZ] != t->trDepth) return 1;
    const int n = t->cW, layer = 5 - t->log2;
    for (int c = 1; c < 3; c++) {
      const int po = HM_PLANE_OFF(c);
      par_copy32(e->cc + po + t->cOff, e->ws->qtCoef[layer] + po + t->cOff, n * n);
      par_copy_blk(e->ws->reco + po + t->cy * 32 + t->cx, 32, e->ws->qtRec[layer] + po + t->cy * 32 + t->cx, 32, n);
    }
    return 0;
  });
}
HM_DEV HM_NOINLINE uint32_t est_intra_pred_chroma_qt(Shared *e, int cuZ, int cuDepth)
{
  HM_ENTRY(e); cuZ = HM_UNI(cuZ); cuDepth = HM_UNI(cuDepth);
  CtuMeta *m = (&e->meta); WorkSpace *ws = e->ws; const int cuParts = 256 >> (2 * cuDepth);
  const TU t = tu_root(e, cuZ, cuDepth);
  if (cuDepth == 3) {
    const int split = m->tr[cuZ] != 0;
    int tsLuma = 0;
    if (split) for (int s = 0; s < 4; s++) tsLuma += m->ts[0][cuZ + s];
    if (!tsLuma) {
      cabac_copy(&e->cur, &e->ws->slot[HM_SLOT(cuDepth, CI_CURR_BEST)]);
      HM_PROF_BEGIN(e, PR_S4C);
      const uint32_t d = HM_UCALL(simt4_chroma_cu(e, split ? tu_child(&t, 0, 0) : t, cuZ));
      HM_PROF_END(e, PR_S4C);
      cabac_copy(&e->cur, &e->ws->slot[HM_SLOT(cuDepth, CI_CURR_BEST)]);
      return d;
    }
  }
  if (cuDepth == 2) {
    int split = 0;
    for (int i = 0; i < 16; i += 4) split |= m->tr[cuZ + i];
    if (!split) {
      cabac_copy(&e->cur, &e->ws->slot[HM_SLOT(cuDepth, CI_CURR_BEST)]);
      HM_PROF_BEGIN(e, PR_S8C);
      const uint32_t d = HM_UCALL(simt8_chroma_cu16(e, cuZ));
      HM_PROF_END(e, PR_S8C);
      cabac_copy(&e->cur, &e->ws->slot[HM_SLOT(cuDepth, CI_CURR_BEST)]);
      return d;
    }
  }
  int bestMode = 0; uint32_t bestDist = 0; double bestCost = HM_MAX_DOUBLE;
  int modeList[5];
  allowed_chroma_dirs(m->dirL[cuZ], modeList);
  for (int mi = 0; mi < 5; mi++) {
    cabac_copy(&e->cur, &e->ws->slot[HM_SLOT(cuDepth, CI_CURR_BEST)]);
    par_set8(m->dirC + cuZ, modeList[mi], cuParts);
    const uint32_t dist = HM_UCALL(recur_intra_chroma_coding_qt(e, t));
    cabac_copy(&e->cur, &e->ws->slot[HM_SLOT(cuDepth, CI_CURR_BEST)]);
    const uint32_t bits = HM_UCALL(intra_bits_qt(e, t, 0, 1));
    const double cost = calc_rd_cost(e, bits, dist);
    if (cost < bestCost) {
      bestCost = cost; bestDist = dist; bestMode = modeList[mi];
      set_intra_result_chroma_qt(e, &t);
      HM_PAR_FOR(i, cuParts) for (int c = 1; c < 3; c++) { ws->saveCbf[c][i] = m->cbf[c][cuZ + i]; ws->saveTs[c][i] = m->ts[c][cuZ + i]; }
      HM_SYNC();
    }
  }
  HM_PAR_FOR(i, cuParts) { for (int c = 1; c < 3; c++) { m->cbf[c][cuZ + i] = ws->saveCbf[c][i]; m->ts[c][cuZ + i] = ws->saveTs[c][i]; } m->dirC[cuZ + i] = (uint8_t)bestMode; }
  HM_SYNC();
  cabac_copy(&e->cur, &e->ws->slot[HM_SLOT(cuDepth, CI_CURR_BEST)]);
  return bestDist;
}

template <class C> HM_DEV inline void code_delta_qp(Shared *e, C *c, int dqp)
{
  const int off = 6 * (e->bitDepth - 8);
  dqp = (dqp + 78 + off + (off / 2)) % (52 + off) - 26 - (off / 2);
  const uint32_t a = (uint32_t)hm_abs(dqp), tu = a < 5 ? a : 5;
  enc_bin(e, c, C_DQP, tu ? 1 : 0);
  if (tu) { for (uint32_t k = tu; --k;) enc_bin(e, c, C_DQP + 1, 1); if (5 > tu) enc_bin(e, c, C_DQP + 1, 0); }
  if (a >= 5) {
    uint32_t sym = a - 5, count = 0, bins = 0; int nb = 0;
    while (sym >= (1u << count)) { bins = 2 * bins + 1; nb++; sym -= 1u << count; count++; }
    bins = 2 * bins; nb++;
    bins = (bins << count) | sym; nb += (int)count;
    enc_epv(c, bins, nb);
  }
  if (a > 0) enc_epv(c, dqp > 0 ? 0u : 1u, 1);
}
template <class C> HM_DEV inline void code_dqp_if_due(Shared *e, C *c)
{
  if (!e->fb.dqp) return;
  WorkSpace *ws = e->ws;
  if (!HM_UNI(ws->dq.flag)) return;
  code_delta_qp(e, c, HM_UNI(ws->dq.ctuQp) - HM_UNI(ws->dq.refQp));
  HM_SYNC();
  if (hm_lane() == 0) ws->dq.flag = 0;
  HM_SYNC();
}
HM_DEV inline void check_dqp(Shared *e, int cuZ, int cuDepth)
{
  if (!e->fb.dqp || cuDepth != 0) return;
  const CtuMeta *m = &e->meta;
  if (!(((m->cbf[0][cuZ] | m->cbf[1][cuZ] | m->cbf[2][cuZ]) & 1))) return;
  reset_bits(&e->cur);
  code_delta_qp(e, &e->cur, HM_UNI(e->ws->dq.ctuQp) - HM_UNI(e->ws->dq.refQp));
  e->outBits += num_bits(&e->cur);
  e->outCost = calc_rd_cost(e, e->outBits, e->outDist);
}
HM_DEV inline int first_coded_cu(const Shared *e)
{
  const CtuMeta *m = &e->meta;
  int best = 256;
  HM_PAR_FOR(z, 256) if (m->cbf[0][z] | m->cbf[1][z] | m->cbf[2][z]) { const int zz = z & ~((256 >> (2 * m->depth[z])) - 1); if (zz < best) best = zz; }
  return -hm_wave_max_i(-best);
}

template <class C> HM_DEV inline void encode_transform(Shared *e, C *c, const TU *root, int intra, int codeDqp)
{
  const CtuMeta *m = (&e->meta);
  tu_walk(e->walkOuter, root, 1, [&](const TU *t) {
    const int z = t->cuZ + t->relZ, subdiv = m->tr[z] > t->trDepth;
    if (codes_subdiv_flag(m, t, intra)) enc_bin(e, c, C_SUBDIV + (5 - t->log2), subdiv);
    code_chroma_cbfs(e, c, t, subdiv);
    if (subdiv) return 1;
    if (intra || t->trDepth || ((m->cbf[1][z] | m->cbf[2][z]) & 1)) code_qt_cbf(e, c, t, 0, 1);
    if (codeDqp && (((m->cbf[0][z] | m->cbf[1][z] | m->cbf[2][z]) >> t->trDepth) & 1)) code_dqp_if_due(e, c);
    for (int comp = 0; comp < 3; comp++) code_tu_coeff(e, c, t, comp, e->cc, intra);
    return 0;
  });
}
template <class C> HM_DEV HM_NOINLINE void encode_cu_syntax(Shared *e, C *c, int cuZ, int cuDepth)
{
  HM_ENTRY(e); cuZ = HM_UNI(cuZ); cuDepth = HM_UNI(cuDepth); c = hm_uni_ptr(c); HM_ASSUME_LDS(c);
  const CtuMeta *m = (&e->meta);
  if (e->im) { code_skip_flag(e, c, cuZ); enc_bin(e, c, C_PRED_MODE, 1); }
  if (cuDepth == 3) enc_bin(e, c, C_PART, m->part[cuZ] == SIZE_2Nx2N);
#if defined(HM355_PROFILE) && !defined(HM355_HOSTSIM)
  const unsigned long long profDir0 = __builtin_readcyclecounter();
#endif
  code_intra_dir_luma(e, c, cuZ, 1);
  code_intra_dir_chroma(e, c, cuZ);
#if defined(HM355_PROFILE) && !defined(HM355_HOSTSIM)
  if (EngOf<C>::REAL) { e->prof[PR_SAVE] += __builtin_readcyclecounter() - profDir0; e->profCnt[PR_SAVE] += 1; }
#endif
  const TU root = tu_root(e, cuZ, cuDepth);
  encode_transform(e, c, &root, 1, 1);
}

#include "hm355_inter.h"

HM_DEV inline void init_est_data(Shared *e, int cuZ, int cuDepth)
{
  CtuMeta *m = (&e->meta); const int parts = 256 >> (2 * cuDepth);
  HM_PAR_FOR(i, parts) {
    const int z = cuZ + i;
    m->depth[z] = (uint8_t)cuDepth; m->part[z] = SIZE_NONE; m->pred[z] = MODE_NONE; m->dirL[z] = DC_IDX; m->dirC[z] = 0; m->tr[z] = 0;
    for (int c = 0; c < 3; c++) { m->cbf[c][z] = 0; m->ts[c][z] = 0; }
  }
  HM_PAR_FOR(i, parts * 16) e->cc[cuZ * 16 + i] = 0;
  HM_PAR_FOR(i, parts * 4) { e->cc[4096 + cuZ * 4 + i] = 0; e->cc[5120 + cuZ * 4 + i] = 0; }
  HM_SYNC();
  if (e->im) init_est_data_inter(e, cuZ, cuDepth);
}
HM_DEV inline void meta_copy_range(CtuMeta *d, const CtuMeta *s, int z0, int parts)
{
  HM_PAR_FOR(i, parts) {
    const int z = z0 + i;
    d->depth[z] = s->depth[z]; d->part[z] = s->part[z]; d->pred[z] = s->pred[z]; d->dirL[z] = s->dirL[z]; d->dirC[z] = s->dirC[z]; d->tr[z] = s->tr[z];
    for (int c = 0; c < 3; c++) { d->cbf[c][z] = s->cbf[c][z]; d->ts[c][z] = s->ts[c][z]; }
  }
}
HM_DEV HM_NOINLINE void save_best(Shared *e, int cuZ, int cuDepth)
{
  HM_ENTRY(e); cuZ = HM_UNI(cuZ); cuDepth = HM_UNI(cuDepth);
  HM_PROF_BEGIN(e, PR_SAVE);
  Best *b = &e->ws->best[cuDepth]; const int parts = 256 >> (2 * cuDepth);
  meta_copy_range(&b->m, (&e->meta), cuZ, parts);
  if (e->im) imeta_copy_range(&b->im, e->im, cuZ, parts);
  HM_PAR_FOR(i, parts * 16) b->coef[cuZ * 16 + i] = e->cc[cuZ * 16 + i];
  HM_PAR_FOR(i, parts * 4) { b->coef[4096 + cuZ * 4 + i] = e->cc[4096 + cuZ * 4 + i]; b->coef[5120 + cuZ * 4 + i] = e->cc[5120 + cuZ * 4 + i]; }
  const int r = hm_z2r(cuZ), x = (r & 15) * 4, y = (r >> 4) * 4, n = 64 >> cuDepth, l2 = 6 - cuDepth;
  HM_PAR_FOR(i, n * n) { const int yy = i >> l2, xx = i & (n - 1); b->reco[(y + yy) * 64 + x + xx] = e->ws->reco[(y + yy) * 64 + x + xx]; }
  HM_PAR_FOR(i, (n * n) >> 2) {
    const int yy = i >> (l2 - 1), xx = i & ((n >> 1) - 1), o = ((y >> 1) + yy) * 32 + (x >> 1) + xx;
    b->reco[4096 + o] = e->ws->reco[4096 + o]; b->reco[5120 + o] = e->ws->reco[5120 + o];
  }
  HM_SYNC();
  HM_PROF_END(e, PR_SAVE);
}
HM_DEV HM_NOINLINE void restore_best_from(Shared *e, const Best *b, int cuZ, int cuDepth)
{
  HM_ENTRY(e); cuZ = HM_UNI(cuZ); cuDepth = HM_UNI(cuDepth); b = hm_uni_ptr(b); HM_ASSUME_GLB(b);
  const int parts = 256 >> (2 * cuDepth);
  meta_copy_range((&e->meta), &b->m, cuZ, parts);
  if (e->im) imeta_copy_range(e->im, &b->im, cuZ, parts);
  HM_PAR_FOR(i, parts * 16) e->cc[cuZ * 16 + i] = b->coef[cuZ * 16 + i];
  HM_PAR_FOR(i, parts * 4) { e->cc[4096 + cuZ * 4 + i] = b->coef[4096 + cuZ * 4 + i]; e->cc[5120 + cuZ * 4 + i] = b->coef[5120 + cuZ * 4 + i]; }
  const int r = hm_z2r(cuZ), x = (r & 15) * 4, y = (r >> 4) * 4, n = 64 >> cuDepth, l2 = 6 - cuDepth;
  Pel *ry = e->fb.rec[0] + (e->ctuY * 64 + y) * e->stride[0] + e->ctuX * 64 + x;
  HM_PAR_FOR(i, n * n) { const int yy = i >> l2, xx = i & (n - 1); ry[yy * e->stride[0] + xx] = b->reco[(y + yy) * 64 + x + xx]; }
  Pel *ru = e->fb.rec[1] + (e->ctuY * 32 + (y >> 1)) * e->stride[1] + e->ctuX * 32 + (x >> 1);
  Pel *rv = e->fb.rec[2] + (e->ctuY * 32 + (y >> 1)) * e->stride[2] + e->ctuX * 32 + (x >> 1);
  HM_PAR_FOR(i, (n * n) >> 2) {
    const int yy = i >> (l2 - 1), xx = i & ((n >> 1) - 1), o = ((y >> 1) + yy) * 32 + (x >> 1) + xx;
    ru[yy * e->stride[1] + xx] = b->reco[4096 + o]; rv[yy * e->stride[2] + xx] = b->reco[5120 + o];
  }
  HM_SYNC();
}
HM_DEV inline void restore_best(Shared *e, int cuZ, int cuDepth) { restore_best_from(e, &e->ws->best[cuDepth], cuZ, cuDepth); }

HM_DEV HM_NOINLINE void check_rd_cost_intra(Shared *e, int cuZ, int cuDepth, int partSize)
{
  HM_ENTRY(e); cuZ = HM_UNI(cuZ); cuDepth = HM_UNI(cuDepth); partSize = HM_UNI(partSize);
  CtuMeta *m = (&e->meta); const int parts = 256 >> (2 * cuDepth);
#if defined(HM355_PROFILE) && !defined(HM355_HOSTSIM)
  const unsigned long long profCu0 = __builtin_readcyclecounter();
#endif
  init_est_data(e, cuZ, cuDepth);
  HM_PAR_FOR(i, parts) { m->part[cuZ + i] = (uint8_t)partSize; m->pred[cuZ + i] = MODE_INTRA; }
  HM_SYNC();
  HM_PROF_BEGIN(e, PR_LUMA);
  uint32_t d = HM_UCALL(est_intra_pred_qt(e, cuZ, cuDepth));
  HM_PROF_END(e, PR_LUMA);
  {
// ... 257 lines not shown
```

### hm-16.2_amd/csrc/hm355_simt.h

```cpp
#pragma once

template <int L2> struct SimtDim {
  enum { NC = 1 << (2 * L2), NCG = NC / 16, NSIG = L2 == 2 ? 9 : 21, NSET = NCG == 1 ? 1 : 4, NGRP = 2 * L2, NCGC = NCG == 1 ? 0 : 2,
         X_SIG = 0, X_ONE = NSIG, X_ABS = X_ONE + 4 * NSET, X_LX = X_ABS + NSET, X_LY = X_LX + 3, X_CG = X_LY + 3, X_CBF = X_CG + NCGC,
         X_MODE = X_CBF + 1, X_TSKIP = X_MODE + 1, NCTX = X_TSKIP + (L2 == 2 ? 1 : 0),
         T_SIG = 0, T_ONE = 2 * NSIG, T_ABS = T_ONE + 8 * NSET, T_LASTX = T_ABS + 2 * NSET, T_LASTY = T_LASTX + NGRP, T_CG = T_LASTY + NGRP,
         T_CBF = T_CG + 2 * NCGC, T_N = T_CBF + 2 };
};
template <int L2> struct Simt;
template <int L2> struct SimtPrices {
  const int32_t *tab;
  HM_FINL_M int one(int i) const { return tab[SimtDim<L2>::T_ONE + i]; }
  HM_FINL_M int abs2(int i) const { return tab[SimtDim<L2>::T_ABS + i]; }
};

struct SimtPar {
  int chroma, bitDepth, qBits, quantCoef, tshift; double errScale, lambda; int64_t rdFactor;
  int dqShift, dqScale, dqMin, dqMax;
};
template <int L2> HM_DEV inline SimtPar simt_params(const Shared *e, int chroma)
{
  SimtPar p;
  p.chroma = chroma; p.bitDepth = e->bitDepth; p.tshift = 15 - e->bitDepth - L2;
  p.qBits = 14 + e->fb.qpPer[chroma] + p.tshift; p.quantCoef = HM_QUANT_SCALES[e->fb.qpRem[chroma]];
  p.errScale = e->fb.errScale[chroma][L2 - 2]; p.lambda = chroma ? e->fb.lambdaC : e->fb.lambda; p.rdFactor = e->fb.rdFactor[chroma];
  p.dqShift = 6 - (p.tshift + e->fb.qpPer[chroma]); p.dqScale = HM_INV_QUANT_SCALES[e->fb.qpRem[chroma]];
  int tgt = 25 + p.dqShift; if (tgt > 16) tgt = 16;
  p.dqMin = -(1 << (tgt - 1)); p.dqMax = (1 << (tgt - 1)) - 1;
  return p;
}
HM_FINL int32_t simt_level_double(int sc, const SimtPar &p)
{
  const int64_t cap = 2147483647LL - (1LL << (p.qBits - 1));
  const int64_t tl = (int64_t)hm_abs(sc) * p.quantCoef;
  return (int32_t)(tl < cap ? tl : cap);
}
HM_FINL int simt_dequant(const SimtPar &p, int level)
{
  const int c = hm_clip3(p.dqMin, p.dqMax, level);
  int v;
  if (p.dqShift > 0) v = (c * p.dqScale + (1 << (p.dqShift - 1))) >> p.dqShift;
  else v = (int)((unsigned)(c * p.dqScale) << (-p.dqShift));
  return hm_clip3(-32768, 32767, v);
}

template <int L2> HM_FINL int simt_ctx_index(int j, int chroma, int cbfCodeCtx, int modeCtx)
{
  typedef SimtDim<L2> D;
  const int lastOff = chroma ? 15 : (L2 == 2 ? 0 : 3);
  if (j < D::X_ONE) return C_SIG + (chroma ? 28 : 0) + (chroma && j >= 16 ? 0 : j);
  if (j < D::X_ABS) return C_ONE + (chroma ? 16 + ((j - D::X_ONE) & 7) : j - D::X_ONE);
  if (j < D::X_LX) return C_ABS + (chroma ? 4 + ((j - D::X_ABS) & 1) : j - D::X_ABS);
  if (j < D::X_LY) return C_LASTX + lastOff + (j - D::X_LX);
  if (j < D::X_CG) return C_LASTY + lastOff + (j - D::X_LY);
  if (j < D::X_CBF) return C_SIG_CG + (chroma ? 2 : 0) + (j - D::X_CG);
  if (j == D::X_CBF) return C_QT_CBF + cbfCodeCtx;
  if (j == D::X_MODE) return modeCtx;
  return C_TSKIP + (chroma ? 1 : 0);
}
template <int L2> HM_DEV inline void simt_setup(Shared *e, const Simt<L2> &S, const Cabac *cb, int jobs, int chroma, int cbfCtx, int cbfCodeCtx, int modeCtx)
{
  typedef SimtDim<L2> D;
  HM_PAR_FOR(i, D::T_N) {
    const int bin = i & 1;
    int v = 0;
    if (i < D::T_LASTX) {
      const int j = i >> 1, none = chroma && ((j < D::X_ONE && j >= 16) || (j >= D::X_ONE && j < D::X_ABS && j - D::X_ONE >= 8) || (j >= D::X_ABS && j - D::X_ABS >= 2));
      if (!none) v = HM_LT()->ebits[cb->s[simt_ctx_index<L2>(j, chroma, 0, 0)] ^ bin];
    } else if (i < D::T_CG) {
      const int g = (i - D::T_LASTX) % D::NGRP, x0 = i < D::T_LASTY ? D::X_LX : D::X_LY;
      for (int c = 0; c < g; c++) v += HM_LT()->ebits[cb->s[simt_ctx_index<L2>(x0 + (c >> (L2 - 2)), chroma, 0, 0)] ^ 1];
      if (g < D::NGRP - 1) v += HM_LT()->ebits[cb->s[simt_ctx_index<L2>(x0 + (g >> (L2 - 2)), chroma, 0, 0)] ^ 0];
      if (g > 3) v += 32768 * ((g - 2) >> 1);
    } else if (i < D::T_CBF) v = HM_LT()->ebits[cb->s[simt_ctx_index<L2>(D::X_CG + ((i - D::T_CG) >> 1), chroma, 0, 0)] ^ bin];
    else v = HM_LT()->ebits[cb->s[C_QT_CBF + cbfCtx] ^ bin];
    S.A->tab[i] = v;
  }
  HM_PAR_FOR(i, 128) S.A->lps[i] = HM_NEXT_LPS[i];
  HM_PAR_FOR(i, D::NCTX * S.JOBS) {
    const int j = i / S.JOBS, k = i - j * S.JOBS;
    if (k < jobs) S.A->ctx[j][k] = cb->s[simt_ctx_index<L2>(j, chroma, cbfCodeCtx, modeCtx)];
  }
  S.load_scans(e);
  HM_SYNC();
}
template <int L2> HM_FINL void simt_store_contexts(const Simt<L2> &S, int k, Cabac *cb, int cbfCodeCtx)
{
  HM_PAR_FOR(j, SimtDim<L2>::NCTX) cb->s[simt_ctx_index<L2>(j, 0, cbfCodeCtx, C_INTRA_LUMA)] = S.A->ctx[j][k];
}

template <int L2> HM_DEV inline void simt_bin(const Shared *e, const Simt<L2> &S, int k, uint32_t *frac, int c, int bin)
{
  const int st = S.A->ctx[c][k];
  *frac += (uint32_t)HM_LT()->ebits[st ^ bin];
  S.A->ctx[c][k] = (uint8_t)(bin == (st & 1) ? (st < 124 ? st + 2 : st) : S.A->lps[st]);
}
HM_FINL int simt_cg_pattern(int cgBlkPos, int cgMask)
{
  const int cgx = cgBlkPos & 1, cgy = cgBlkPos >> 1;
  const int sigRight = cgx < 1 ? ((cgMask >> (cgBlkPos + 1)) & 1) : 0, sigLower = cgy < 1 ? ((cgMask >> (cgBlkPos + 2)) & 1) : 0;
  return sigRight + (sigLower << 1);
}
template <int L2> HM_FINL void simt_last_xy(int blkPos, int scanType, int *px, int *py)
{
  const int y = blkPos >> L2, x = blkPos & ((1 << L2) - 1);
  *px = scanType == SCAN_VER ? y : x; *py = scanType == SCAN_VER ? x : y;
}

template <int L2> HM_DEV inline int simt_rdoq(const Simt<L2> &S, const SimtPar &p, int k, int scanType)
{
  typedef SimtDim<L2> D;
  const int32_t *tab = S.A->tab; const SimtPrices<L2> prices = { tab };
  const int qBits = p.qBits, half = 1 << (qBits - 1);
  const double lambda = p.lambda, errScale = p.errScale;
  const int firstCtx = first_sig_ctx(1 << L2, scanType, p.chroma), lumaSets = p.chroma ? 0 : 2;
  double blockUncoded = 0, baseCost = 0;
  double cgSig1 = 0, cgSig2 = 0, cgSig3 = 0;
  int last = -1, cgLast = -1, ctxSet = 0;
  int cgMask = 0, cgSets = 0;
  LevelChain ch;
  for (int cg = D::NCG - 1; cg >= 0; cg--) {
    const int cgBlkPos = S.cg_pos(scanType, cg), cgBit = 1 << cgBlkPos, pattern = simt_cg_pattern(cgBlkPos, cgMask);
    double sigCost = 0, sigCost0 = 0, codedLevelAndDist = 0, uncodedDist = 0; int nnzBeforePos0 = 0;
    cgSets |= ctxSet << (2 * cg);
    for (int q = 15; q >= 0; q--) {
      const int sp = cg * 16 + q;
      const int32_t lvlD = simt_level_double(S.cs(sp, k), p);
      uint32_t mx = (uint32_t)((lvlD + half) >> qBits); if (mx > 32767u) mx = 32767u;
      const double err = (double)lvlD, c0 = err * err * errScale;
      blockUncoded += c0;
      if (mx > 0 && last < 0) { last = sp; cgLast = cg; ctxSet = cg > 0 ? lumaSets : 0; cgSets = ctxSet << (2 * cg); }
      uint32_t level = 0; double cSig = 0, cCoeff = c0;
      if (last >= 0) {
        const int isLast = (sp == last);
        const int si = isLast ? 0 : S.sig_inc(scanType, firstCtx, pattern, sp, p.chroma);
        if (!isLast && mx < 3) { cSig = lambda * (double)tab[D::T_SIG + si * 2]; cCoeff = c0 + cSig; }
        else cCoeff = HM_MAX_DOUBLE;
        if (mx > 0) {
          double currCostSig = 0;
          if (!isLast) currCostSig = lambda * (double)tab[D::T_SIG + si * 2 + 1];
          const uint32_t minAbs = mx > 1 ? mx - 1 : 1;
          for (int al = (int)mx; al >= (int)minAbs; al--) {
            const double de = (double)(lvlD - (int32_t)((uint32_t)al << qBits));
            const double dist = de * de * errScale;
            const double rc = lambda * (double)ic_rate(prices, (uint32_t)al, 4 * ctxSet + ch.c1, ctxSet, ch);
            double cc = dist + rc;
            cc += currCostSig;
            if (cc < cCoeff) { level = (uint32_t)al; cCoeff = cc; cSig = currCostSig; }
          }
        }
        S.keep_cost(sp, k, cCoeff);
        baseCost += cCoeff;
        ch.step(level);
        if (q == 0 && cg > 0) { ctxSet = ((cg - 1) > 0 ? lumaSets : 0) + (ch.c1 == 0 ? 1 : 0); ch = LevelChain(); }
      } else baseCost += c0;
      sigCost += cSig;
      if (q == 0) sigCost0 = cSig;
      if (level) {
        cgMask |= cgBit;
        codedLevelAndDist += cCoeff - cSig;
        uncodedDist += c0;
        if (q != 0) nnzBeforePos0++;
      }
      S.B->dc[sp][k] = (int32_t)level;
    }
    if (cgLast >= 0) {
      if (cg) {
        const int cgCtx = (pattern != 0) * 2;
        double cgs = 0;
        if (!(cgMask & cgBit)) {
          const double r0 = lambda * (double)tab[D::T_CG + cgCtx];
          baseCost += r0 - sigCost;
          cgs = r0;
        } else if (cg < cgLast) {
          if (nnzBeforePos0 == 0) { baseCost -= sigCost0; sigCost -= sigCost0; }
          double costZeroCG = baseCost;
          const double r0 = lambda * (double)tab[D::T_CG + cgCtx], r1 = lambda * (double)tab[D::T_CG + cgCtx + 1];
          baseCost += r1;
          costZeroCG += r0;
          cgs = r1;
          costZeroCG += uncodedDist; costZeroCG -= codedLevelAndDist; costZeroCG -= sigCost;
          if (costZeroCG < baseCost) {
            cgMask &= ~cgBit; baseCost = costZeroCG; cgs = r0;
            for (int q = 15; q >= 0; q--) S.B->dc[cg * 16 + q][k] |= 0x40000000;
          }
        }
        if (cg == 1) cgSig1 = cgs; else if (cg == 2) cgSig2 = cgs; else cgSig3 = cgs;
      } else cgMask |= cgBit;
    }
  }
  if (last < 0) return 0;
  double bestCost = blockUncoded + lambda * (double)tab[D::T_CBF];
  baseCost += lambda * (double)tab[D::T_CBF + 1];
  int bestLastP1 = 0, found = 0;
  for (int cg = cgLast; cg >= 0 && !found; cg--) {
    if (cg) baseCost -= (cg == 1 ? cgSig1 : (cg == 2 ? cgSig2 : cgSig3));
    if (!((cgMask >> S.cg_pos(scanType, cg)) & 1)) continue;
    const int wSet = (cgSets >> (2 * cg)) & 3, pattern = simt_cg_pattern(S.cg_pos(scanType, cg), cgMask); LevelChain walk;
    for (int q = (cg == cgLast ? (last & 15) : 15); q >= 0; q--) {
      const int sp = cg * 16 + q, lev = S.B->dc[sp][k] & 0xffff;
      const int si = sp == last ? 0 : S.sig_inc(scanType, firstCtx, pattern, sp, p.chroma);
      if (lev) {
        int px, py; simt_last_xy<L2>(S.B->scan[scanType][sp], scanType, &px, &py);
        const double costLast = lambda * (double)(tab[D::T_LASTX + hm_group_idx(px)] + tab[D::T_LASTY + hm_group_idx(py)]);
        const double cSig = (sp == last) ? 0.0 : lambda * (double)tab[D::T_SIG + si * 2 + 1];
        const double t1 = baseCost + costLast;
        const double totalCost = t1 - cSig;
        if (totalCost < bestCost) { bestLastP1 = sp + 1; bestCost = totalCost; }
        if (lev > 1) { found = 1; break; }
        const int32_t lvlD = simt_level_double(S.cs(sp, k), p);
        const double err = (double)lvlD;
        double cc;
        if (S.KEEPS_COST) cc = S.cost_at(sp, k);
        else {
          const double de = (double)(lvlD - (int32_t)((uint32_t)lev << qBits));
          const double dist = de * de * errScale;
          const double rc = lambda * (double)ic_rate(prices, (uint32_t)lev, 4 * wSet + walk.c1, wSet, walk);
          cc = dist + rc;
          cc += cSig;
          walk.step((uint32_t)lev);
        }
        baseCost -= cc; baseCost += err * err * errScale;
      } else baseCost -= lambda * (double)tab[D::T_SIG + si * 2];
    }
  }
  int absSum = 0;
  for (int sp = 0; sp < D::NC; sp++) {
    const int v = S.B->dc[sp][k], dec = v & 0xffff, lv = (sp < bestLastP1 && !(v & 0x40000000)) ? dec : 0;
    absSum += lv;
    S.B->dc[sp][k] = dec | (int32_t)((uint32_t)(S.cs(sp, k) < 0 ? -lv : lv) << 16);
  }
  if (absSum >= 2) {
    int lastCG = -1;
    for (int subSet = D::NCG - 1; subSet >= 0; subSet--) {
      const int subPos = subSet << 4;
      int lastNZ = -1, firstNZ = 16, parity = 0;
      for (int q = 0; q < 16; q++) { const int lv = S.B->dc[subPos + q][k] >> 16; if (lv) { lastNZ = q; if (firstNZ == 16) firstNZ = q; } parity ^= lv & 1; }
      if (lastNZ >= 0 && lastCG == -1) lastCG = 1;
      if (lastNZ - firstNZ >= 4) {
        const uint32_t signbit = (S.B->dc[subPos + firstNZ][k] >> 16) > 0 ? 0 : 1;
        if (signbit != (uint32_t)parity) {
          const int64_t I64MAX = 0x7fffffffffffffffLL;
          int64_t minCostInc = I64MAX, curCost = I64MAX; int minK = -1, finalChange = 0, curChange = 0;
          const int wSet = (cgSets >> (2 * subSet)) & 3; LevelChain walk;
          const int top = (subPos + 15 <= last) ? 15 : (last - subPos), kStart = (lastCG == 1 ? lastNZ : 15);
          const int pattern = simt_cg_pattern(S.cg_pos(scanType, subSet), cgMask);
          for (int q = top; q >= 0; --q) {
            const int v = S.B->dc[subPos + q][k]; const uint32_t dec = (uint32_t)(v & 0xffff); const int dv = v >> 16;
            const int ctxOne = 4 * wSet + walk.c1; const LevelChain at = walk;
            walk.step(dec);
            if (q > kStart) continue;
            const int sc = S.cs(subPos + q, k);
            const int32_t lvlD = simt_level_double(sc, p);
            const int32_t deltaU = (int32_t)((lvlD - (int32_t)(dec << qBits)) >> (qBits - 8));
            const int si = (subPos + q == last) ? 0 : S.sig_inc(scanType, firstCtx, pattern, subPos + q, p.chroma);
            const int sigRateDelta = (subPos + q == last) ? 0 : tab[D::T_SIG + si * 2 + 1] - tab[D::T_SIG + si * 2];
            int rateIncUp, rateIncDown = 0;
            if (dec > 0) {
              const int rateNow = ic_rate(prices, dec, ctxOne, wSet, at);
              rateIncUp = ic_rate(prices, dec + 1, ctxOne, wSet, at) - rateNow;
              rateIncDown = ic_rate(prices, dec - 1, ctxOne, wSet, at) - rateNow;
            } else rateIncUp = prices.one(ctxOne * 2);
            if (dv != 0) {
              const int64_t costUp = p.rdFactor * (-deltaU) + rateIncUp;
              int64_t costDown = p.rdFactor * (deltaU) + rateIncDown - ((hm_abs(dv) == 1) ? sigRateDelta : 0);
              if (lastCG == 1 && lastNZ == q && hm_abs(dv) == 1) costDown -= (4 << 15);
              if (costUp < costDown) { curCost = costUp; curChange = 1; }
              else { curChange = -1; if (q == firstNZ && hm_abs(dv) == 1) curCost = I64MAX; else curCost = costDown; }
            } else {
              curCost = p.rdFactor * (-(hm_abs(deltaU))) + (1 << 15) + rateIncUp + sigRateDelta;
              curChange = 1;
              if (q < firstNZ) { const uint32_t thissign = sc < 0 ? 1u : 0u; if (thissign != signbit) curCost = I64MAX; }
            }
            if (curCost < minCostInc) { minCostInc = curCost; finalChange = curChange; minK = q; }
          }
          if (minK >= 0) {
            const int v = S.B->dc[subPos + minK][k]; int mv = v >> 16;
            if (mv == 32767 || mv == -32768) finalChange = -1;
            mv = (S.cs(subPos + minK, k) < 0) ? mv - finalChange : mv + finalChange;
            S.B->dc[subPos + minK][k] = (v & 0xffff) | (int32_t)((uint32_t)mv << 16);
          }
        }
      }
      if (lastCG == 1) lastCG = 0;
    }
  }
  return absSum;
}

template <int L2> HM_DEV inline void simt_code_coeff(const Shared *e, const Simt<L2> &S, int k, int src, int chroma, int scanType, uint32_t *frac)
{
  typedef SimtDim<L2> D;
  int last = -1, cgMask = 0;
  for (int sp = 0; sp < D::NC; sp++)
    if ((S.B->dc[sp][src] >> 16) != 0) { last = sp; cgMask |= 1 << S.cg_pos(scanType, sp >> 4); }
  {
    int px, py; simt_last_xy<L2>(S.B->scan[scanType][last], scanType, &px, &py);
    const int gx = hm_group_idx(px), gy = hm_group_idx(py);
    int q;
    for (q = 0; q < gx; q++) simt_bin(e, S, k, frac, D::X_LX + (q >> (L2 - 2)), 1);
    if (gx < D::NGRP - 1) simt_bin(e, S, k, frac, D::X_LX + (q >> (L2 - 2)), 0);
    for (q = 0; q < gy; q++) simt_bin(e, S, k, frac, D::X_LY + (q >> (L2 - 2)), 1);
    if (gy < D::NGRP - 1) simt_bin(e, S, k, frac, D::X_LY + (q >> (L2 - 2)), 0);
    if (gx > 3) *frac += 32768u * (uint32_t)((gx - 2) >> 1);
    if (gy > 3) *frac += 32768u * (uint32_t)((gy - 2) >> 1);
  }
  const int firstCtx = first_sig_ctx(1 << L2, scanType, chroma), lastSet = last >> 4;
  int c1 = 1;
  for (int subSet = lastSet; subSet >= 0; subSet--) {
    const int subPos = subSet << 4, isLastSet = subSet == lastSet;
    const int cgBlkPos = S.cg_pos(scanType, subSet), pattern = simt_cg_pattern(cgBlkPos, cgMask);
    if (isLastSet || subSet == 0) cgMask |= 1 << cgBlkPos;
    else simt_bin(e, S, k, frac, D::X_CG + (pattern != 0), (cgMask >> cgBlkPos) & 1);
    if (!((cgMask >> cgBlkPos) & 1)) continue;
    const int top = isLastSet ? (last & 15) : 15;
    int numNonZero = isLastSet ? 1 : 0, firstNZ = isLastSet ? top : 16, lastNZ = isLastSet ? top : -1;
    for (int q = isLastSet ? top - 1 : 15; q >= 0; q--) {
      const int sig = (S.B->dc[subPos + q][src] >> 16) != 0;
      if (q > 0 || subSet == 0 || numNonZero) simt_bin(e, S, k, frac, D::X_SIG + S.sig_inc(scanType, firstCtx, pattern, subPos + q, chroma), sig);
      if (sig) { numNonZero++; firstNZ = q; if (lastNZ < 0) lastNZ = q; }
    }
    if (numNonZero > 0) {
      const int signHidden = (lastNZ - firstNZ >= 4);
      const int ctxSet = ((subSet > 0 && !chroma) ? 2 : 0) + (c1 == 0 ? 1 : 0);
      c1 = 1;
      int firstC2 = -1, escape = 0, idx = 0;
      for (int q = lastNZ; q >= 0 && idx < 8; q--) {
        const int a = hm_abs(S.B->dc[subPos + q][src] >> 16);
        if (!a) continue;
        const int sym = a > 1;
        simt_bin(e, S, k, frac, D::X_ONE + 4 * ctxSet + c1, sym);
        if (sym) { c1 = 0; if (firstC2 == -1) firstC2 = q; else escape = 1; }
        else if (c1 < 3 && c1 > 0) c1++;
        idx++;
      }
      if (c1 == 0 && firstC2 != -1) { const int sym = hm_abs(S.B->dc[subPos + firstC2][src] >> 16) > 2; simt_bin(e, S, k, frac, D::X_ABS + ctxSet, sym); if (sym) escape = 1; }
      escape = escape || (numNonZero > 8);
      *frac += 32768u * (uint32_t)(signHidden ? numNonZero - 1 : numNonZero);
      if (escape) {
        int firstCoeff2 = 1; uint32_t goRice = 0; idx = 0;
        for (int q = lastNZ; q >= 0; q--) {
          const int a = hm_abs(S.B->dc[subPos + q][src] >> 16);
          if (!a) continue;
          const int baseLevel = (idx < 8) ? (2 + firstCoeff2) : 1;
          if (a >= baseLevel) {
            *frac += 32768u * coef_remain_len((uint32_t)(a - baseLevel), goRice);
            if ((uint32_t)a > (3u << goRice)) goRice = goRice + 1 < 4 ? goRice + 1 : 4;
          }
          if (a >= 2) firstCoeff2 = 0;
          idx++;
        }
      }
    }
  }
}

template <int L2> HM_FINL void simt_luma_mode_bits(const Shared *e, const Simt<L2> &S, int k, uint32_t *frac, int mode)
{
  int predIdx = -1;
  for (int i = 0; i < 3; i++) if (mode == e->mpmPreds[i]) predIdx = i;
  simt_bin(e, S, k, frac, SimtDim<L2>::X_MODE, predIdx != -1);
  *frac += 32768u * (uint32_t)(predIdx == -1 ? 5 : (predIdx ? 2 : 1));
}
HM_FINL void simt_chroma_ref_lines(Shared *e, int px, int py, int n, int x4, int y4)
{
  init_adi_pattern(e, 2, px, py, n, x4, y4, n >> 1, 0);
  HM_PAR_FOR(i, 2 * n + 1) { e->u.ref.refTop[1][i] = e->u.ref.refTop[0][i]; e->u.ref.refLeft[1][i] = e->u.ref.refLeft[0][i]; }
  HM_SYNC();
  init_adi_pattern(e, 1, px, py, n, x4, y4, n >> 1, 0);
}
HM_FINL void allowed_chroma_dirs(int lumaDir, int *list)
{
  list[0] = PLANAR_IDX; list[1] = VER_IDX; list[2] = HOR_IDX; list[3] = DC_IDX; list[4] = DM_CHROMA_IDX;
  for (int i = 0; i < 4; i++) if (lumaDir == list[i]) { list[i] = 34; break; }
}
HM_FINL int chroma_mode_at(const int *list, int mi)
{ return mi == 0 ? list[0] : (mi == 1 ? list[1] : (mi == 2 ? list[2] : (mi == 3 ? list[3] : list[4]))); }
```

### hm-16.2_amd/csrc/hm355_simt4.h

```cpp
#pragma once

#define HM_SL 22
struct Simt4A {
  double cost[16][HM_SL];
  double outCost[HM_SL];
  uint32_t outDist[HM_SL], outBits[HM_SL];
  int32_t tab[SimtDim<2>::T_N];
  uint8_t ctx[SimtDim<2>::NCTX][HM_SL];
  uint8_t outCbf[HM_SL];
  uint8_t lps[128];
};
struct Simt4B {
  int32_t cs[16][HM_SL];
  int32_t dc[16][HM_SL];
  uint8_t scan[3][16];
  uint8_t sigIdx[3][16];
};
static_assert(sizeof(Simt4A) <= sizeof(((Shared *)0)->bufA), "Simt4A overlays bufA");
static_assert(offsetof(RefLds, refMain) + sizeof(Simt4B) <= sizeof(((Shared *)0)->u), "Simt4B overlays the tail of the LDS union");
static_assert(offsetof(RefLds, refMain) % 8 == 0, "alignment of the overlay");
HM_DEV constexpr int s4_scan(int type, int i)
{
  constexpr uint8_t t[3][16] = { {0, 4, 1, 8, 5, 2, 12, 9, 6, 3, 13, 10, 7, 14, 11, 15}, {0, 1, 2, 3, 4, 5, 6, 7, 8, 9, 10, 11, 12, 13, 14, 15},
                                 {0, 4, 8, 12, 1, 5, 9, 13, 2, 6, 10, 14, 3, 7, 11, 15} };
  return t[type][i];
}
HM_DEV constexpr int s4_inv_scan(int type, int r)
{
  constexpr uint8_t t[3][16] = { {0, 2, 5, 9, 1, 4, 8, 12, 3, 7, 11, 14, 6, 10, 13, 15}, {0, 1, 2, 3, 4, 5, 6, 7, 8, 9, 10, 11, 12, 13, 14, 15},
                                 {0, 4, 8, 12, 1, 5, 9, 13, 2, 6, 10, 14, 3, 7, 11, 15} };
  return t[type][r];
}
template <> struct Simt<2> {
  enum { JOBS = HM_SL, KEEPS_COST = 1 };
  Simt4A *A; Simt4B *B;
  HM_FINL_M explicit Simt(Shared *e) : A((Simt4A *)e->bufA), B((Simt4B *)((char *)&e->u + offsetof(RefLds, refMain))) {}
  HM_FINL_M int cs(int sp, int k) const { return B->cs[sp][k]; }
  HM_FINL_M int cg_pos(int, int) const { return 0; }
  HM_FINL_M int sig_inc(int scanType, int, int, int sp, int) const { return B->sigIdx[scanType][sp]; }
  HM_FINL_M void keep_cost(int sp, int k, double c) const { A->cost[sp][k] = c; }
  HM_FINL_M double cost_at(int sp, int k) const { return A->cost[sp][k]; }
  HM_FINL_M void load_scans(const Shared *e) const
  {
    HM_PAR_FOR(i, 48) {
      const int ty = i >> 4, sp = i & 15, blk = e->tab->scan[ty][0][sp];
      B->scan[ty][sp] = (uint8_t)blk; B->sigIdx[ty][sp] = HM_CTX_IND_MAP_4x4[blk];
#ifdef HM355_HOSTSIM
      if (blk != s4_scan(ty, sp) || s4_inv_scan(ty, blk) != sp) abort();
#endif
    }
  }
};
typedef Simt<2> Simt4;

HM_FINL int s4_pred_sample(const Shared *e, int rs, int chroma, int mode, int x, int y, int dcVal, int bitDepth)
{ return intra_pred_sample(e->u.ref.refTop[rs], e->u.ref.refLeft[rs], 4, 2, !chroma, mode, x, y, dcVal, bitDepth); }

HM_FINL int s4_tm(int dst, int k, int j)
{
  if (dst) return HM_DST4[k * 4 + j];
  const int m = (k * 8 * (2 * j + 1)) & 127;
  if (m <= 32) return HM_DCT_C[m]; if (m <= 64) return -HM_DCT_C[64 - m]; if (m <= 96) return -HM_DCT_C[m - 64]; return HM_DCT_C[128 - m];
}
HM_FINL void s4_fwd(int32_t *blk, int dst, int bitDepth)
{
  const int s1 = 2 + bitDepth + 6 - 15, a1 = 1 << (s1 - 1), s2 = 8, a2 = 128;
  int32_t t[16];
#pragma unroll
  for (int j = 0; j < 4; j++)
#pragma unroll
    for (int k = 0; k < 4; k++) { int32_t acc = 0;
#pragma unroll
      for (int i = 0; i < 4; i++) acc += s4_tm(dst, k, i) * blk[j * 4 + i];
      t[k * 4 + j] = (acc + a1) >> s1; }
#pragma unroll
  for (int j = 0; j < 4; j++)
#pragma unroll
    for (int k = 0; k < 4; k++) { int32_t acc = 0;
#pragma unroll
      for (int i = 0; i < 4; i++) acc += s4_tm(dst, k, i) * t[j * 4 + i];
      blk[k * 4 + j] = (acc + a2) >> s2; }
}
HM_FINL void s4_inv(int32_t *blk, int dst, int bitDepth)
{
  const int s1 = 7, s2 = 20 - bitDepth;
  int32_t t[16];
#pragma unroll
  for (int j = 0; j < 4; j++)
#pragma unroll
    for (int i = 0; i < 4; i++) { int32_t acc = 0;
#pragma unroll
      for (int k = 0; k < 4; k++) acc += s4_tm(dst, k, i) * blk[k * 4 + j];
      t[j * 4 + i] = hm_clip3(-32768, 32767, (acc + (1 << (s1 - 1))) >> s1); }
#pragma unroll
  for (int j = 0; j < 4; j++)
#pragma unroll
    for (int i = 0; i < 4; i++) { int32_t acc = 0;
#pragma unroll
      for (int k = 0; k < 4; k++) acc += s4_tm(dst, k, i) * t[k * 4 + j];
      blk[j * 4 + i] = hm_clip3(-32768, 32767, (acc + (1 << (s2 - 1))) >> s2); }
}

HM_FINL void s4_code_coeff(const Shared *e, const Simt4 &S, int k, int src, int chroma, int scanType, int tskipFlag, uint32_t *frac)
{
  simt_bin(e, S, k, frac, SimtDim<2>::X_TSKIP, tskipFlag);
  simt_code_coeff(e, S, k, src, chroma, scanType, frac);
}

#ifdef HM355_HOSTSIM
#define HM_LVA(T, name, n) T name[64][n]
#define HM_LVAK(name, k) name[k]
#else
#define HM_LVA(T, name, n) T name[n]
#define HM_LVAK(name, k) name
#endif

HM_FINL uint32_t s4_eval(Shared *e, const Simt4 &S, const SimtPar &p, int k, int rs, const Pel *org, int ps, int mode, int ts, int scanType,
                               int dcVal, int32_t *rec, int32_t *lv, int *cbf)
{
  int32_t pred[16], blk[16];
#pragma unroll
  for (int i = 0; i < 16; i++) {
    pred[i] = s4_pred_sample(e, rs, p.chroma, mode, i & 3, i >> 2, dcVal, p.bitDepth);
    const int r = org[(i >> 2) * ps + (i & 3)] - pred[i];
    blk[i] = ts ? r * (1 << p.tshift) : r;
  }
  if (!ts) s4_fwd(blk, !p.chroma, p.bitDepth);
#pragma unroll
  for (int i = 0; i < 16; i++)
    S.B->cs[i][k] = scanType == SCAN_HOR ? blk[s4_scan(SCAN_HOR, i)] : (scanType == SCAN_VER ? blk[s4_scan(SCAN_VER, i)] : blk[s4_scan(SCAN_DIAG, i)]);
  const int absSum = simt_rdoq(S, p, k, scanType);
  *cbf = absSum > 0;
#pragma unroll
  for (int i = 0; i < 16; i++) lv[i] = 0;
  if (absSum > 0) {
    int32_t ls[16];
#pragma unroll
    for (int i = 0; i < 16; i++) ls[i] = S.B->dc[i][k] >> 16;
#pragma unroll
    for (int j = 0; j < 16; j++)
      lv[j] = scanType == SCAN_HOR ? ls[s4_inv_scan(SCAN_HOR, j)] : (scanType == SCAN_VER ? ls[s4_inv_scan(SCAN_VER, j)] : ls[s4_inv_scan(SCAN_DIAG, j)]);
#pragma unroll
    for (int i = 0; i < 16; i++) blk[i] = simt_dequant(p, lv[i]);
    if (!ts) s4_inv(blk, !p.chroma, p.bitDepth);
    else {
      const int off = p.tshift == 0 ? 0 : (1 << (p.tshift - 1));
#pragma unroll
      for (int i = 0; i < 16; i++) blk[i] = (int16_t)((blk[i] + off) >> p.tshift);
    }
  } else {
#pragma unroll
    for (int i = 0; i < 16; i++) blk[i] = 0;
  }
  const int maxv = (1 << p.bitDepth) - 1, shiftSse = (p.bitDepth - 8) << 1;
  uint32_t sse = 0;
#pragma unroll
  for (int i = 0; i < 16; i++) {
    const int r = hm_clip3(0, maxv, pred[i] + (int16_t)blk[i]);
    rec[i] = r;
    const int d = org[(i >> 2) * ps + (i & 3)] - r; sse += (uint32_t)((d * d) >> shiftSse);
  }
  return sse;
}

HM_DEV HM_NOINLINE void simt4_luma_pu(Shared *e, TU tv, int numModes)
{
  HM_ENTRY(e); numModes = HM_UNI(numModes); tv = hm_uni_struct(tv);
  const TU *t = &tv; CtuMeta *m = (&e->meta); WorkSpace *ws = e->ws;
  const int z = t->cuZ + t->relZ, ps = e->stride[0], jobs = 2 * numModes;
  uint32_t commonFrac;
  {
    CabacR r; cabr_load(e, r, &e->cur);
    r.frac &= 32767;
    if (t->relZ == 0) {
      if (e->im) { code_skip_flag(e, &r, t->cuZ); enc_bin(e, &r, C_PRED_MODE, 1); }
      if (t->cuDepth == 3) enc_bin(e, &r, C_PART, 0);
    }
    commonFrac = (uint32_t)r.frac;
  }
  const Simt4 S(e); Simt4A *A = S.A;
  simt_setup(e, S, &e->cur, jobs, 0, 0, 0, C_INTRA_LUMA);
  const SimtPar p = simt_params<2>(e, 0);
  const Pel *org = e->fb.org[0] + (e->ctuY * 64 + t->y) * ps + e->ctuX * 64 + t->x;
  const int dcVal = ref_dc_val(e, 0, 4);
  HM_LVA(int32_t, rec, 16); HM_LVA(int32_t, lv, 16);
  HM_WAVE_FOR(k) {
    if (k < jobs) {
      const int mode = e->rdModeList[k >> 1], ts = k & 1, scanType = intra_scan_type(mode);
      int cbf;
      const uint32_t dist = s4_eval(e, S, p, k, 0, org, ps, mode, ts, scanType, dcVal, HM_LVAK(rec, k), HM_LVAK(lv, k), &cbf);
      uint32_t frac = commonFrac;
      simt_luma_mode_bits(e, S, k, &frac, mode);
      simt_bin(e, S, k, &frac, SimtDim<2>::X_CBF, cbf);
      if (cbf) s4_code_coeff(e, S, k, k, 0, scanType, ts, &frac);
      const uint32_t bits = frac >> 15;
      A->outDist[k] = dist; A->outBits[k] = bits; A->outCbf[k] = (uint8_t)cbf;
      A->outCost[k] = calc_rd_cost(e, bits, dist);
    }
  }
  HM_SYNC();
  double bestCost = HM_MAX_DOUBLE; int bestJob = 0;
  for (int c = 0; c < numModes; c++) {
    double single = A->outCost[2 * c]; int pick = 2 * c;
    if (A->outCbf[2 * c + 1]) { const double c1 = A->outCost[2 * c + 1]; if (c1 < single) { single = c1; pick = 2 * c + 1; } }
    if (single < bestCost) { bestCost = single; bestJob = pick; }
  }
  bestJob = HM_UNI(bestJob);
  const int bestMode = e->rdModeList[bestJob >> 1], bestCbf = A->outCbf[bestJob];
  e->outBits = (uint32_t)bestMode; e->outDistY = A->outDist[bestJob]; e->outRdCost = bestCost;
  HM_WAVE_FOR(k) {
    if (k == bestJob) {
      TCoeff *coef = e->cc + z * 16; Pel *ro = ws->reco + t->y * 64 + t->x;
#pragma unroll
      for (int i = 0; i < 16; i++) { coef[i] = HM_LVAK(lv, k)[i]; ro[(i >> 2) * 64 + (i & 3)] = (Pel)HM_LVAK(rec, k)[i]; }
    }
  }
  if (hm_lane() == 0) {
    m->tr[z] = (uint8_t)t->trDepth; m->cbf[0][z] = (uint8_t)(bestCbf << t->trDepth); m->ts[0][z] = (uint8_t)(bestJob & 1); m->dirL[z] = (uint8_t)bestMode;
  }
  HM_SYNC();
}

HM_DEV HM_NOINLINE uint32_t simt4_chroma_cu(Shared *e, TU leafv, int cuZ)
{
  HM_ENTRY(e); cuZ = HM_UNI(cuZ); leafv = hm_uni_struct(leafv);
  const TU *t = &leafv; CtuMeta *m = (&e->meta); WorkSpace *ws = e->ws;
  const int zc = t->cuZ + t->cRelZ, r = hm_z2r(zc);
  const int x4 = e->ctuX * 16 + (r & 15), y4 = e->ctuY * 16 + (r >> 4), px = e->ctuX * 32 + t->cx, py = e->ctuY * 32 + t->cy;
  simt_chroma_ref_lines(e, px, py, 4, x4, y4);
  int modeList[5];
  const int lumaDir = m->dirL[cuZ];
  allowed_chroma_dirs(lumaDir, modeList);
  const Simt4 S(e); Simt4A *A = S.A;
  simt_setup(e, S, &e->cur, 10, 1, 5 + t->trDepth, 5, C_CHROMA_PRED);
  const SimtPar p = simt_params<2>(e, 1);
  const uint32_t baseFrac = (uint32_t)(e->cur.frac & 32767);
  const int dcVal[2] = { ref_dc_val(e, 0, 4), ref_dc_val(e, 1, 4) };
  HM_LVA(int32_t, rec, 16); HM_LVA(int32_t, lv, 16);
  HM_WAVE_FOR(k) {
    if (k < 10) {
      const int c = k & 1, mi = k >> 1, ps = e->stride[1 + c];
      const int dirC = chroma_mode_at(modeList, mi), mode = dirC == DM_CHROMA_IDX ? lumaDir : dirC, scanType = intra_scan_type(mode);
      const Pel *org = e->fb.org[1 + c] + (size_t)py * ps + px;
      int cbf;
      const uint32_t sse = s4_eval(e, S, p, k, c, org, ps, mode, 0, scanType, c ? dcVal[1] : dcVal[0], HM_LVAK(rec, k), HM_LVAK(lv, k), &cbf);
      A->outDist[k] = (uint32_t)(e->fb.chromaWeight * (double)sse);
      A->outCbf[k] = (uint8_t)cbf;
    }
  }
  HM_SYNC();
  HM_WAVE_FOR(k) {
    if (k < 10 && !(k & 1)) {
      const int mi = k >> 1;
      const int dirC = chroma_mode_at(modeList, mi), mode = dirC == DM_CHROMA_IDX ? lumaDir : dirC, scanType = intra_scan_type(mode);
      uint32_t frac = baseFrac;
      simt_bin(e, S, k, &frac, SimtDim<2>::X_MODE, dirC != DM_CHROMA_IDX);
      if (dirC != DM_CHROMA_IDX) frac += 2u * 32768u;
      const int cbfU = A->outCbf[k], cbfV = A->outCbf[k + 1];
      simt_bin(e, S, k, &frac, SimtDim<2>::X_CBF, cbfU);
      simt_bin(e, S, k, &frac, SimtDim<2>::X_CBF, cbfV);
      if (cbfU) s4_code_coeff(e, S, k, k, 1, scanType, 0, &frac);
      if (cbfV) s4_code_coeff(e, S, k, k + 1, 1, scanType, 0, &frac);
      const uint32_t bits = frac >> 15, dist = A->outDist[k] + A->outDist[k + 1];
      A->outBits[k] = dist;
      A->outCost[k] = calc_rd_cost(e, bits, dist);
    }
  }
  HM_SYNC();
  double bestCost = HM_MAX_DOUBLE; int best = 0;
  for (int mi = 0; mi < 5; mi++) { const double c = A->outCost[2 * mi]; if (c < bestCost) { bestCost = c; best = mi; } }
  best = HM_UNI(best);
  const uint32_t bestDist = A->outBits[2 * best];
  const int cbfU = A->outCbf[2 * best], cbfV = A->outCbf[2 * best + 1];
  HM_WAVE_FOR(k) {
    if ((k >> 1) == best && k < 10) {
      const int po = HM_PLANE_OFF(1 + (k & 1));
      TCoeff *coef = e->cc + po + t->cOff; Pel *ro = ws->reco + po + t->cy * 32 + t->cx;
#pragma unroll
      for (int i = 0; i < 16; i++) { coef[i] = HM_LVAK(lv, k)[i]; ro[(i >> 2) * 32 + (i & 3)] = (Pel)HM_LVAK(rec, k)[i]; }
    }
  }
  {
    const int vU = t->trDepth ? 3 * cbfU : cbfU, vV = t->trDepth ? 3 * cbfV : cbfV, bm = chroma_mode_at(modeList, best);
    HM_PAR_FOR(i, 4) { m->cbf[1][cuZ + i] = (uint8_t)vU; m->cbf[2][cuZ + i] = (uint8_t)vV; m->ts[1][cuZ + i] = 0; m->ts[2][cuZ + i] = 0; m->dirC[cuZ + i] = (uint8_t)bm; }
  }
  HM_SYNC();
  return bestDist;
}

HM_DEV HM_NOINLINE void simt4_luma_leaf(Shared *e, TU tv)
{
  HM_ENTRY(e); tv = hm_uni_struct(tv);
  const TU *t = &tv; CtuMeta *m = (&e->meta); WorkSpace *ws = e->ws;
  const int z = t->cuZ + t->relZ, ps = e->stride[0], r = hm_z2r(z), mode = m->dirL[z];
  init_adi_pattern(e, 0, e->ctuX * 64 + t->x, e->ctuY * 64 + t->y, 4, e->ctuX * 16 + (r & 15), e->ctuY * 16 + (r >> 4), 1, 0);
  {
    CabacR cr; cabr_load(e, cr, &e->cur);
    cr.frac &= 32767;
    enc_intra_header(e, &cr, t, 1, 0);
    cabr_store(cr, &e->cur);
  }
  const Simt4 S(e); Simt4A *A = S.A;
  simt_setup(e, S, &e->cur, 1, 0, 0, 0, C_INTRA_LUMA);
  const SimtPar p = simt_params<2>(e, 0);
  const Pel *org = e->fb.org[0] + (e->ctuY * 64 + t->y) * ps + e->ctuX * 64 + t->x;
  const int dcVal = ref_dc_val(e, 0, 4);
  const int scanType = intra_scan_type(mode);
  const uint32_t frac0 = (uint32_t)e->cur.frac;
  HM_WAVE_FOR(k) {
    if (k == 0) {
      int32_t rec[16], lv[16]; int cbf;
      const uint32_t dist = s4_eval(e, S, p, 0, 0, org, ps, mode, 0, scanType, dcVal, rec, lv, &cbf);
      uint32_t frac = frac0;
      simt_bin(e, S, 0, &frac, SimtDim<2>::X_CBF, cbf);
      if (cbf) s4_code_coeff(e, S, 0, 0, 0, scanType, 0, &frac);
      A->outDist[0] = dist; A->outBits[0] = frac; A->outCbf[0] = (uint8_t)cbf;
      TCoeff *coef = ws->qtCoef[3] + z * 16; Pel *rq = ws->qtRec[3] + t->y * 64 + t->x;
      Pel *recPic = e->fb.rec[0] + (e->ctuY * 64 + t->y) * ps + e->ctuX * 64 + t->x;
#pragma unroll
      for (int i = 0; i < 16; i++) { coef[i] = lv[i]; rq[(i >> 2) * 64 + (i & 3)] = (Pel)rec[i]; recPic[(i >> 2) * ps + (i & 3)] = (Pel)rec[i]; }
    }
  }
  HM_SYNC();
  simt_store_contexts(S, 0, &e->cur, 0);
  const int cbf = A->outCbf[0];
  e->cur.frac = (uint64_t)A->outBits[0];
  e->outDistY = A->outDist[0]; e->outBits = A->outBits[0] >> 15;
  if (hm_lane() == 0) { m->tr[z] = (uint8_t)t->trDepth; m->cbf[0][z] = (uint8_t)(cbf << t->trDepth); }
  HM_SYNC();
}

HM_DEV HM_NOINLINE uint32_t simt4_chroma_leaf(Shared *e, TU tv)
{
  HM_ENTRY(e); tv = hm_uni_struct(tv);
  const TU *t = &tv; CtuMeta *m = (&e->meta); WorkSpace *ws = e->ws;
  const int zc = t->cuZ + t->cRelZ, r = hm_z2r(zc), layer = 5 - t->log2;
  const int x4 = e->ctuX * 16 + (r & 15), y4 = e->ctuY * 16 + (r >> 4), px = e->ctuX * 32 + t->cx, py = e->ctuY * 32 + t->cy;
  simt_chroma_ref_lines(e, px, py, 4, x4, y4);
  int mode = m->dirC[zc];
// ... 28 lines not shown
```

### hm-16.2_amd/csrc/hm355_simt8.h

```cpp
#pragma once

#define HM_S8 11
struct Simt8A {
  int32_t tile[2][64];
  int32_t tab[SimtDim<3>::T_N];
  double outCost[HM_S8];
  uint32_t outDist[HM_S8], outFrac[HM_S8];
  int16_t cs[64][HM_S8];
  uint8_t ctx[SimtDim<3>::NCTX][HM_S8];
  uint8_t outCbf[HM_S8], best;
  uint8_t lps[128];
};
struct Simt8B {
  int32_t dc[64][HM_S8];
  uint8_t scan[3][64];
  uint8_t scanCG[3][4];
};
static_assert(sizeof(Simt8A) <= sizeof(((Shared *)0)->bufA), "Simt8A overlays bufA");
static_assert(offsetof(RefLds, refMain) + sizeof(Simt8B) <= sizeof(((Shared *)0)->u), "Simt8B overlays the tail of the LDS union");
template <> struct Simt<3> {
  enum { JOBS = HM_S8, KEEPS_COST = 0 };
  Simt8A *A; Simt8B *B;
  HM_FINL_M explicit Simt(Shared *e) : A((Simt8A *)e->bufA), B((Simt8B *)((char *)&e->u + offsetof(RefLds, refMain))) {}
  HM_FINL_M int cs(int sp, int k) const { return A->cs[sp][k]; }
  HM_FINL_M int cg_pos(int scanType, int cg) const { return B->scanCG[scanType][cg]; }
  HM_FINL_M int sig_inc(int scanType, int firstCtx, int pattern, int sp, int chroma) const { return sig_ctx_inc(pattern, firstCtx, B->scan[scanType][sp], 3, chroma); }
  HM_FINL_M void keep_cost(int, int, double) const {}
  HM_FINL_M double cost_at(int, int) const { return 0; }
  HM_FINL_M void load_scans(const Shared *e) const
  {
    HM_PAR_FOR(i, 192) { const int ty = i >> 6, sp = i & 63; B->scan[ty][sp] = (uint8_t)e->tab->scan[ty][1][sp]; }
    HM_PAR_FOR(i, 12) { const int ty = i >> 2, cg = i & 3; B->scanCG[ty][cg] = (uint8_t)e->tab->scanCG[ty][1][cg]; }
  }
};
typedef Simt<3> Simt8;

template <class Pred> HM_FINL void s8_residual_fwd(const Simt8 &S, const Pel *org, int ps, int bitDepth, int scanType, int job, Pred pred)
{
  Simt8A *A = S.A;
  const int s1 = 3 + bitDepth + 6 - 15, a1 = 1 << (s1 - 1), s2 = 9, a2 = 256;
  HM_PAR_FOR(l, 64) { const int y = l >> 3, x = l & 7; A->tile[0][l] = org[y * ps + x] - pred(x, y); }
  HM_SYNC();
  HM_PAR_FOR(l, 64) {
    const int j = l >> 3, kk = l & 7; int32_t acc = 0;
    for (int i = 0; i < 8; i++) acc += HM_LT()->tmat[(kk * 4) * HM_TSTRIDE + i] * A->tile[0][j * 8 + i];
    A->tile[1][kk * 8 + j] = (acc + a1) >> s1;
  }
  HM_SYNC();
  HM_PAR_FOR(l, 64) {
    const int blkPos = S.B->scan[scanType][l], kk = blkPos >> 3, j = blkPos & 7; int32_t acc = 0;
    for (int i = 0; i < 8; i++) acc += HM_LT()->tmat[(kk * 4) * HM_TSTRIDE + i] * A->tile[1][j * 8 + i];
    A->cs[l][job] = (int16_t)((acc + a2) >> s2);
  }
  HM_SYNC();
}
HM_FINL void s8_dequant_inv1(const Simt8 &S, const SimtPar &p, int scanType, int job, int cbf, TCoeff *coef)
{
  Simt8A *A = S.A;
  if (cbf) {
    HM_PAR_FOR(l, 64) {
      const int lv = S.B->dc[l][job] >> 16, blk = S.B->scan[scanType][l];
      if (coef) coef[blk] = lv;
      A->tile[0][blk] = simt_dequant(p, lv);
    }
    HM_SYNC();
    HM_PAR_FOR(l, 64) {
      const int j = l >> 3, i = l & 7; int32_t acc = 0;
      for (int kk = 0; kk < 8; kk++) acc += HM_LT()->tmat[(kk * 4) * HM_TSTRIDE + i] * A->tile[0][kk * 8 + j];
      A->tile[1][j * 8 + i] = hm_clip3(-32768, 32767, (acc + 64) >> 7);
    }
    HM_SYNC();
  } else if (coef) { HM_PAR_FOR(l, 64) coef[l] = 0; }
}
template <class Pred, class Out> HM_FINL void s8_inv2_recon(const Simt8 &S, int bitDepth, int cbf, Pred pred, Out out)
{
  const int maxv = (1 << bitDepth) - 1, is2 = 20 - bitDepth;
  HM_PAR_FOR(l, 64) {
    const int j = l >> 3, i = l & 7; int resi = 0;
    if (cbf) {
      int32_t acc = 0;
      for (int kk = 0; kk < 8; kk++) acc += HM_LT()->tmat[(kk * 4) * HM_TSTRIDE + i] * S.A->tile[1][kk * 8 + j];
      resi = hm_clip3(-32768, 32767, (acc + (1 << (is2 - 1))) >> is2);
    }
    out(i, j, hm_clip3(0, maxv, pred(i, j) + resi));
  }
}

HM_DEV HM_NOINLINE int simt8_luma_first_pass(Shared *e, TU tv, int numModes)
{
  HM_ENTRY(e); numModes = HM_UNI(numModes); tv = hm_uni_struct(tv);
  const TU *t = &tv;
  const int ps = e->stride[0], bitDepth = e->bitDepth;
  const Simt8 S(e); Simt8A *A = S.A;
  uint32_t commonFrac;
  {
    CabacR r; cabr_load(e, r, &e->cur);
    r.frac &= 32767;
    if (e->im) { code_skip_flag(e, &r, t->cuZ); enc_bin(e, &r, C_PRED_MODE, 1); }
    enc_bin(e, &r, C_PART, 1);
    enc_bin(e, &r, C_SUBDIV + 2, 0);
    commonFrac = (uint32_t)r.frac;
  }
  simt_setup(e, S, &e->cur, numModes, 0, 1, 1, C_INTRA_LUMA);
  const SimtPar p = simt_params<3>(e, 0);
  const Pel *org = e->fb.org[0] + (e->ctuY * 64 + t->y) * ps + e->ctuX * 64 + t->x;
  const int dcVal = ref_dc_val(e, 0, 8);
  for (int c = 0; c < numModes; c++) {
    const int mode = e->rdModeList[c];
    s8_residual_fwd(S, org, ps, bitDepth, intra_scan_type(mode), c, [&](int x, int y) HM_LAMBDA_INL { return pred_sample(e, mode, 8, 3, x, y, dcVal, bitDepth); });
  }
  HM_WAVE_FOR(k) {
    if (k < numModes) A->outCbf[k] = (uint8_t)(simt_rdoq(S, p, k, intra_scan_type(e->rdModeList[k])) > 0);
  }
  HM_SYNC();
  const int shiftSse = (bitDepth - 8) << 1;
  for (int c = 0; c < numModes; c++) {
    const int mode = e->rdModeList[c], cbf = A->outCbf[c];
    s8_dequant_inv1(S, p, intra_scan_type(mode), c, cbf, (TCoeff *)0);
    uint32_t sse = 0;
    s8_inv2_recon(S, bitDepth, cbf, [&](int x, int y) HM_LAMBDA_INL { return pred_sample(e, mode, 8, 3, x, y, dcVal, bitDepth); },
                  [&](int x, int y, int r) HM_LAMBDA_INL { const int d = org[y * ps + x] - r; sse += (uint32_t)((d * d) >> shiftSse); });
    const uint32_t dist = hm_wave_sum(sse);
    if (hm_lane() == 0) A->outDist[c] = dist;
    HM_SYNC();
  }
  HM_WAVE_FOR(k) {
    if (k < numModes) {
      const int mode = e->rdModeList[k], cbf = A->outCbf[k];
      uint32_t frac = commonFrac;
      simt_luma_mode_bits(e, S, k, &frac, mode);
      simt_bin(e, S, k, &frac, SimtDim<3>::X_CBF, cbf);
      if (cbf) simt_code_coeff(e, S, k, k, 0, intra_scan_type(mode), &frac);
      A->outFrac[k] = frac;
      A->outCost[k] = calc_rd_cost(e, frac >> 15, A->outDist[k]);
    }
  }
  HM_SYNC();
  double bestCost = HM_MAX_DOUBLE; int best = 0;
  for (int c = 0; c < numModes; c++) { const double v = A->outCost[c]; if (v < bestCost) { bestCost = v; best = c; } }
  best = HM_UNI(best);
  const int bestMode = e->rdModeList[best];
  e->s8Winner = best;
  HM_SYNC();
  return bestMode;
}

HM_FINL int s8_pred_sample_chroma(const Shared *e, int rs, int mode, int x, int y, int dcVal)
{
  return intra_pred_sample(e->u.ref.refTop[rs], e->u.ref.refLeft[rs], 8, 3, 0, mode, x, y, dcVal, 0);
}
HM_DEV HM_NOINLINE uint32_t simt8_chroma_cu16(Shared *e, int cuZ)
{
  HM_ENTRY(e); cuZ = HM_UNI(cuZ);
  CtuMeta *m = (&e->meta); WorkSpace *ws = e->ws;
  const TU t = tu_root(e, cuZ, 2);
  const int r = hm_z2r(cuZ), bitDepth = e->bitDepth;
  const int x4 = e->ctuX * 16 + (r & 15), y4 = e->ctuY * 16 + (r >> 4), px = e->ctuX * 32 + t.cx, py = e->ctuY * 32 + t.cy;
  simt_chroma_ref_lines(e, px, py, 8, x4, y4);
  int modeList[5];
  const int lumaDir = m->dirL[cuZ];
  allowed_chroma_dirs(lumaDir, modeList);
  const Simt8 S(e); Simt8A *A = S.A;
  simt_setup(e, S, &e->cur, 10, 1, 5, 5, C_CHROMA_PRED);
  const SimtPar p = simt_params<3>(e, 1);
  const uint32_t baseFrac = (uint32_t)(e->cur.frac & 32767);
  const int dcVal[2] = { ref_dc_val(e, 0, 8), ref_dc_val(e, 1, 8) };
  const int shiftSse = (bitDepth - 8) << 1;
  for (int job = 0; job < 10; job++) {
    const int c = job & 1, dirC = modeList[job >> 1], mode = dirC == DM_CHROMA_IDX ? lumaDir : dirC, ps = e->stride[1 + c];
    s8_residual_fwd(S, e->fb.org[1 + c] + (size_t)py * ps + px, ps, bitDepth, SCAN_DIAG, job,
                    [&](int x, int y) HM_LAMBDA_INL { return s8_pred_sample_chroma(e, c, mode, x, y, dcVal[c]); });
  }
  HM_WAVE_FOR(k) { if (k < 10) A->outCbf[k] = (uint8_t)(simt_rdoq(S, p, k, SCAN_DIAG) > 0); }
  HM_SYNC();
  for (int pass = 0; pass < 12; pass++) {
    int job = pass;
    if (pass == 10) {
      HM_WAVE_FOR(k) {
        if (k < 10 && !(k & 1)) {
          const int dirC = modeList[k >> 1];
          uint32_t frac = baseFrac;
          simt_bin(e, S, k, &frac, SimtDim<3>::X_MODE, dirC != DM_CHROMA_IDX);
          if (dirC != DM_CHROMA_IDX) frac += 2u * 32768u;
          const int cbfU = A->outCbf[k], cbfV = A->outCbf[k + 1];
          simt_bin(e, S, k, &frac, SimtDim<3>::X_CBF, cbfU);
          simt_bin(e, S, k, &frac, SimtDim<3>::X_CBF, cbfV);
          if (cbfU) simt_code_coeff(e, S, k, k, 1, SCAN_DIAG, &frac);
          if (cbfV) simt_code_coeff(e, S, k, k + 1, 1, SCAN_DIAG, &frac);
          const uint32_t dist = A->outDist[k] + A->outDist[k + 1];
          A->outCost[k] = calc_rd_cost(e, frac >> 15, dist);
        }
      }
      HM_SYNC();
      double bestCost = HM_MAX_DOUBLE; int best = 0;
      for (int mi = 0; mi < 5; mi++) { const double v = A->outCost[2 * mi]; if (v < bestCost) { bestCost = v; best = mi; } }
      best = HM_UNI(best);
      if (hm_lane() == 0) A->best = (uint8_t)best;
      HM_SYNC();
    }
    const int best = pass >= 10 ? A->best : 0;
    if (pass >= 10) job = 2 * best + (pass - 10);
    const int c = job & 1, dirC = modeList[job >> 1], mode = dirC == DM_CHROMA_IDX ? lumaDir : dirC, ps = e->stride[1 + c], cbf = A->outCbf[job];
    const Pel *org = e->fb.org[1 + c] + (size_t)py * ps + px;
    const int po = HM_PLANE_OFF(1 + c);
    s8_dequant_inv1(S, p, SCAN_DIAG, job, cbf, pass >= 10 ? e->cc + po + t.cOff : (TCoeff *)0);
    uint32_t sse = 0;
    s8_inv2_recon(S, bitDepth, cbf, [&](int x, int y) HM_LAMBDA_INL { return s8_pred_sample_chroma(e, c, mode, x, y, dcVal[c]); },
                  [&](int x, int y, int rr) HM_LAMBDA_INL {
                    const int d = org[y * ps + x] - rr; sse += (uint32_t)((d * d) >> shiftSse);
                    if (pass >= 10) ws->reco[po + (t.cy + y) * 32 + t.cx + x] = (Pel)rr;
                  });
    const uint32_t dsum = hm_wave_sum(sse);
    if (pass < 10 && hm_lane() == 0) A->outDist[job] = (uint32_t)(e->fb.chromaWeight * (double)dsum);
    HM_SYNC();
  }
  const int best = A->best, cbfU = A->outCbf[2 * best], cbfV = A->outCbf[2 * best + 1];
  const uint32_t bestDist = A->outDist[2 * best] + A->outDist[2 * best + 1];
  const int bm = modeList[best];
  HM_PAR_FOR(i, 16) { m->cbf[1][cuZ + i] = (uint8_t)cbfU; m->cbf[2][cuZ + i] = (uint8_t)cbfV; m->ts[1][cuZ + i] = 0; m->ts[2][cuZ + i] = 0; m->dirC[cuZ + i] = (uint8_t)bm; }
  HM_SYNC();
  return bestDist;
}

HM_DEV HM_NOINLINE void simt8_luma_winner_as_single_tu(Shared *e, TU tv)
{
  HM_ENTRY(e); tv = hm_uni_struct(tv);
  const TU *t = &tv; WorkSpace *ws = e->ws;
  const Simt8 S(e); Simt8A *A = S.A;
  const int best = HM_UNI(e->s8Winner), z = t->cuZ + t->relZ, ps = e->stride[0], bitDepth = e->bitDepth;
  const int mode = e->rdModeList[best], cbf = A->outCbf[best];
  const SimtPar p = simt_params<3>(e, 0);
  const int dcVal = ref_dc_val(e, 0, 8);
  Pel *rq = ws->qtRec[2] + t->y * 64 + t->x;
  Pel *recPic = e->fb.rec[0] + (e->ctuY * 64 + t->y) * ps + e->ctuX * 64 + t->x;
  s8_dequant_inv1(S, p, intra_scan_type(mode), best, cbf, ws->qtCoef[2] + z * 16);
  s8_inv2_recon(S, bitDepth, cbf, [&](int x, int y) HM_LAMBDA_INL { return pred_sample(e, mode, 8, 3, x, y, dcVal, bitDepth); },
                [&](int x, int y, int rr) HM_LAMBDA_INL { rq[y * 64 + x] = (Pel)rr; recPic[y * ps + x] = (Pel)rr; });
  HM_SYNC();
  {
    CabacR r; cabr_load(e, r, &e->cur);
    r.frac &= 32767;
    if (e->im) { code_skip_flag(e, &r, t->cuZ); enc_bin(e, &r, C_PRED_MODE, 1); }
    enc_bin(e, &r, C_PART, 1);
    enc_bin(e, &r, C_SUBDIV + 2, 0);
    cabr_store(r, &e->cur);
  }
  simt_store_contexts(S, best, &e->cur, 1);
  e->cur.frac = (uint64_t)A->outFrac[best];
  e->outDistY = A->outDist[best]; e->outBits = A->outFrac[best] >> 15; e->outDist = (uint32_t)cbf;
  HM_SYNC();
}
```

Baseline: 25320.

## Add batched SIMT first-pass RD search for 16x16 intra luma PUs

Extends the wave-parallel batched mode evaluation, which already existed for 8x8, to 16x16 intra luma PUs. A new simt16 path runs forward transform, RDOQ, reconstruction and bit estimation for several candidate modes at once in batches, and keeps the winner so it can be reused as the single-TU result. The shared RDOQ and context helpers are generalized through accessor methods and a templated CG pattern so they work for 4x4, 8x8 and 16x16. The goal is to replace the serial per-mode full RD loop for 16x16 CUs, at the cost of more LDS pressure and more code complexity.

```diff
diff --git a/__graft_entry__.py b/__graft_entry__.py
--- a/__graft_entry__.py
+++ b/__graft_entry__.py
@@ -19,7 +19,7 @@
 def build_product():
     src = os.path.join(PKG, "csrc")
     out = os.path.join(PKG, "libhm355.so")
-    deps = [os.path.join(src, f) for f in ("hm355.hip", "hm355_core.h", "hm355_inter.h", "hm355_inter_cu.h", "hm355_dbk.h", "hm355_sao.h", "hm355_bits.h", "hm355_bits_kernel.h", "hm355_ingest.h", "hm355_picstat.h", "hm355_types.h", "hm355_host_common.h", "hm355_simt.h", "hm355_simt4.h", "hm355_simt8.h", "hm355_team.h")] + [os.path.join(ROOT, "include", "hm355.h")]
+    deps = [os.path.join(src, f) for f in ("hm355.hip", "hm355_core.h", "hm355_inter.h", "hm355_inter_cu.h", "hm355_dbk.h", "hm355_sao.h", "hm355_bits.h", "hm355_bits_kernel.h", "hm355_ingest.h", "hm355_picstat.h", "hm355_types.h", "hm355_host_common.h", "hm355_simt.h", "hm355_simt4.h", "hm355_simt8.h", "hm355_simt16.h", "hm355_team.h")] + [os.path.join(ROOT, "include", "hm355.h")]
     if _newer(out, deps):
         import hashlib
         h = hashlib.sha1()
diff --git a/hm-16.2_amd/csrc/hm355_core.h b/hm-16.2_amd/csrc/hm355_core.h
--- a/hm-16.2_amd/csrc/hm355_core.h
+++ b/hm-16.2_amd/csrc/hm355_core.h
@@ -121,7 +121,7 @@
 #endif
 
 #if defined(HM355_PROFILE) && !defined(HM355_HOSTSIM)
-#define HM_PROF_N 44
+#define HM_PROF_N 45
 #define HM_PROF_BEGIN(e, id) const unsigned long long prof_t0_##id = __builtin_readcyclecounter()
 #define HM_PROF_END(e, id) do { (e)->prof[id] += __builtin_readcyclecounter() - prof_t0_##id; (e)->profCnt[id] += 1; } while (0)
 #else
@@ -129,7 +129,7 @@
 #define HM_PROF_END(e, id) ((void)0)
 #endif
 enum { PR_RDOQ = 0, PR_BITS, PR_ADI, PR_PRED, PR_FWD, PR_INV, PR_SATD35, PR_TUBLK, PR_SAVE, PR_CHROMA, PR_LUMA, PR_ENCCU, PR_TOTAL,
-       PR_S4L = 32, PR_S4C, PR_D0, PR_D1, PR_D2, PR_D3, PR_NXN, PR_S8L, PR_S4LEAF, PR_S4CLEAF, PR_S8C,
+       PR_S4L = 32, PR_S4C, PR_D0, PR_D1, PR_D2, PR_D3, PR_NXN, PR_S8L, PR_S4LEAF, PR_S4CLEAF, PR_S8C, PR_S16L = 44,
        PR_ME_INT = 16, PR_ME_FRAC, PR_AMVP, PR_MRG_EST, PR_MC, PR_IRQ, PR_IRES, PR_MRG2N, PR_INTERCU, PR_INTRA_IN_P, PR_IQ_FULL, PR_IQ_FWD, PR_IQ_RDOQ, PR_IQ_BITS, PR_IQ_INV, PR_IQ_ENC };
 
 #define HM_MAX_DOUBLE 1.7e+308
@@ -274,7 +274,11 @@
 #define HM_SLOT(d, ci) ((d) * CI_NUM + (ci) - ((d) == 4 ? 2 : 0))
 #define HM_NUM_SLOTS (4 * CI_NUM + 3)
 struct Team;
+#if defined(HM355_PROFILE) && !defined(HM355_HOSTSIM)
+#define HM_CTU_WAVES 11
+#else
 #define HM_CTU_WAVES 12
+#endif
 struct LdsTables {
   int8_t tmat[32 * HM_TSTRIDE];
   int8_t dst4[16];
@@ -348,7 +352,9 @@
 __shared__ Shared g_sh;
 __shared__ Shared g_shs[HM_CTU_WAVES];
 #endif
-#if !defined(HM355_PROFILE)
+#if defined(HM355_PROFILE)
+static_assert(HM_CTU_WAVES * (sizeof(Shared) + 16) + sizeof(LdsTables) <= 163840, "the diagnostic build: one workgroup of HM_CTU_WAVES searches with their cycle counters in 160 KB of LDS");
+#else
 static_assert(HM_CTU_WAVES * (sizeof(Shared) + 16) + sizeof(LdsTables) <= 163840 / (12 / HM_CTU_WAVES) && sizeof(Shared) % 8 == 0, "two workgroups of HM_CTU_WAVES searches (+ work items, + the shared tables) per CU: 12 CTU searches in 160 KB of LDS");
 #endif
 static_assert(offsetof(Shared, bufA) % 8 == 0 && (16 * HM_TSTRIDE * 4) % 8 == 0, "the RDOQ cost array aliases the lower half of bufA as doubles");
@@ -1808,7 +1814,7 @@
 }
 
 HM_DEV HM_NOINLINE void simt4_luma_leaf(Shared *e, TU tv);
-HM_DEV HM_NOINLINE void simt8_luma_winner_as_single_tu(Shared *e, TU tv);
+template <int L2> HM_DEV HM_NOINLINE void simt_luma_winner_as_single_tu(Shared *e, TU tv);
 HM_DEV HM_NOINLINE void recur_intra_coding_qt(Shared *e, TU rootv, int checkFirst)
 {
   HM_ENTRY(e); checkFirst = HM_UNI(checkFirst); rootv = hm_uni_struct(rootv);
@@ -1860,7 +1866,7 @@
           cabac_copy(&e->ws->slot[HM_SLOT(fullDepth, CI_QT_TRAFO_ROOT)], &e->cur);
           par_set8(m->ts[0] + z, 0, t->parts);
           par_set8(m->tr + z, t->trDepth, t->parts);
-          simt8_luma_winner_as_single_tu(e, *t);
+          if (log2 == 3) simt_luma_winner_as_single_tu<3>(e, *t); else simt_luma_winner_as_single_tu<4>(e, *t);
           f->singleDist = e->outDistY; f->singleCbf = e->outDist;
           par_set8(m->cbf[0] + z, (int)(f->singleCbf << t->trDepth), t->parts);
           f->singleCost = calc_rd_cost(e, e->outBits, f->singleDist);
@@ -1947,6 +1953,7 @@
 #include "hm355_simt.h"
 #include "hm355_simt4.h"
 #include "hm355_simt8.h"
+#include "hm355_simt16.h"
 
 HM_DEV HM_NOINLINE uint32_t est_intra_pred_qt(Shared *e, int cuZ, int cuDepth)
 {
@@ -2023,11 +2030,10 @@
     }
     int bestPUMode = 0; uint32_t bestPUDistY = 0; double bestPUCost = HM_MAX_DOUBLE;
     int firstPass = 0;
-    if (n == 8) {
+    if (n == 8 || n == 16) {
       cabac_copy(&e->cur, &e->ws->slot[HM_SLOT(cuDepth, CI_CURR_BEST)]);
-      HM_PROF_BEGIN(e, PR_S8L);
-      bestPUMode = HM_UCALL(simt8_luma_first_pass(e, t, numModesForFullRD));
-      HM_PROF_END(e, PR_S8L);
+      if (n == 8) { HM_PROF_BEGIN(e, PR_S8L); bestPUMode = HM_UCALL(simt8_luma_first_pass(e, t, numModesForFullRD)); HM_PROF_END(e, PR_S8L); }
+      else { HM_PROF_BEGIN(e, PR_S16L); bestPUMode = HM_UCALL(simt16_luma_first_pass(e, t, numModesForFullRD)); HM_PROF_END(e, PR_S16L); }
       firstPass = numModesForFullRD;
       e->s8Reuse = 1;
     }
@@ -2037,7 +2043,7 @@
       par_set8(m->dirL + z, orgMode, puParts);
       cabac_copy(&e->cur, &e->ws->slot[HM_SLOT(cuDepth, CI_CURR_BEST)]);
       e->outCost = bestPUCost;
-      if (last && (n == 16 || n == 32) && numModesForFullRD > 0) { e->s8Reuse = 2; e->outDistY = bestPUDistY; e->outRdCost = bestPUCost; }
+      if (last && n == 32 && numModesForFullRD > 0) { e->s8Reuse = 2; e->outDistY = bestPUDistY; e->outRdCost = bestPUCost; }
       recur_intra_coding_qt(e, t, !last);
       const uint32_t puDistY = e->outDistY; const double puCost = e->outRdCost;
       if (puCost < bestPUCost) {
@@ -2045,7 +2051,7 @@
         set_intra_result_qt(e, &t);
         HM_PAR_FOR(i, puParts) { ws->tmpTr[i] = m->tr[z + i]; for (int c = 0; c < 3; c++) { ws->tmpCbf[c][i] = m->cbf[c][z + i]; ws->tmpTs[c][i] = m->ts[c][z + i]; } }
         HM_SYNC();
-        if (!last && (n == 16 || n == 32)) cabac_copy(&e->ws->slot[HM_SLOT(cuDepth, CI_QT_TRAFO_TEST)], &e->cur);
+        if (!last && n == 32) cabac_copy(&e->ws->slot[HM_SLOT(cuDepth, CI_QT_TRAFO_TEST)], &e->cur);
       }
     }
     overallDistY += bestPUDistY;
diff --git a/hm-16.2_amd/csrc/hm355_simt.h b/hm-16.2_amd/csrc/hm355_simt.h
--- a/hm-16.2_amd/csrc/hm355_simt.h
+++ b/hm-16.2_amd/csrc/hm355_simt.h
@@ -1,12 +1,18 @@
 #pragma once
 
 template <int L2> struct SimtDim {
-  enum { NC = 1 << (2 * L2), NCG = NC / 16, NSIG = L2 == 2 ? 9 : 21, NSET = NCG == 1 ? 1 : 4, NGRP = 2 * L2, NCGC = NCG == 1 ? 0 : 2,
-         X_SIG = 0, X_ONE = NSIG, X_ABS = X_ONE + 4 * NSET, X_LX = X_ABS + NSET, X_LY = X_LX + 3, X_CG = X_LY + 3, X_CBF = X_CG + NCGC,
+  enum { NC = 1 << (2 * L2), NCG = NC / 16, WCG = 1 << (L2 - 2), NSIG = L2 == 2 ? 9 : (L2 == 3 ? 21 : 27), NSET = NCG == 1 ? 1 : 4, NGRP = 2 * L2, NCGC = NCG == 1 ? 0 : 2,
+         NLAST = L2 == 4 ? 4 : 3, LSH = L2 == 4 ? 1 : L2 - 2,
+         X_SIG = 0, X_ONE = NSIG, X_ABS = X_ONE + 4 * NSET, X_LX = X_ABS + NSET, X_LY = X_LX + NLAST, X_CG = X_LY + NLAST, X_CBF = X_CG + NCGC,
          X_MODE = X_CBF + 1, X_TSKIP = X_MODE + 1, NCTX = X_TSKIP + (L2 == 2 ? 1 : 0),
          T_SIG = 0, T_ONE = 2 * NSIG, T_ABS = T_ONE + 8 * NSET, T_LASTX = T_ABS + 2 * NSET, T_LASTY = T_LASTX + NGRP, T_CG = T_LASTY + NGRP,
          T_CBF = T_CG + 2 * NCGC, T_N = T_CBF + 2 };
 };
+static_assert(SimtDim<2>::NCTX == 23 && SimtDim<2>::T_N == 38 && SimtDim<2>::X_LX == 14 && SimtDim<2>::X_LY == 17 && SimtDim<2>::X_CBF == 20 && SimtDim<2>::T_LASTX == 28 &&
+              SimtDim<2>::T_LASTY == 32 && SimtDim<2>::T_CBF == 36 && SimtDim<2>::LSH == 0, "the 4x4 batch's numbering");
+static_assert(SimtDim<3>::NCTX == 51 && SimtDim<3>::T_N == 100 && SimtDim<3>::X_ONE == 21 && SimtDim<3>::X_ABS == 37 && SimtDim<3>::X_LX == 41 && SimtDim<3>::X_LY == 44 &&
+              SimtDim<3>::X_CG == 47 && SimtDim<3>::X_CBF == 49 && SimtDim<3>::T_ONE == 42 && SimtDim<3>::T_ABS == 74 && SimtDim<3>::T_LASTX == 82 && SimtDim<3>::T_LASTY == 88 &&
+              SimtDim<3>::T_CG == 94 && SimtDim<3>::T_CBF == 98 && SimtDim<3>::LSH == 1 && SimtDim<3>::WCG == 2, "the 8x8 batch's numbering");
 template <int L2> struct Simt;
 template <int L2> struct SimtPrices {
   const int32_t *tab;
@@ -47,7 +53,7 @@
 template <int L2> HM_FINL int simt_ctx_index(int j, int chroma, int cbfCodeCtx, int modeCtx)
 {
   typedef SimtDim<L2> D;
-  const int lastOff = chroma ? 15 : (L2 == 2 ? 0 : 3);
+  const int lastOff = chroma ? 15 : 3 * (L2 - 2);
   if (j < D::X_ONE) return C_SIG + (chroma ? 28 : 0) + (chroma && j >= 16 ? 0 : j);
   if (j < D::X_ABS) return C_ONE + (chroma ? 16 + ((j - D::X_ONE) & 7) : j - D::X_ONE);
   if (j < D::X_LX) return C_ABS + (chroma ? 4 + ((j - D::X_ABS) & 1) : j - D::X_ABS);
@@ -69,36 +75,36 @@
       if (!none) v = HM_LT()->ebits[cb->s[simt_ctx_index<L2>(j, chroma, 0, 0)] ^ bin];
     } else if (i < D::T_CG) {
       const int g = (i - D::T_LASTX) % D::NGRP, x0 = i < D::T_LASTY ? D::X_LX : D::X_LY;
-      for (int c = 0; c < g; c++) v += HM_LT()->ebits[cb->s[simt_ctx_index<L2>(x0 + (c >> (L2 - 2)), chroma, 0, 0)] ^ 1];
-      if (g < D::NGRP - 1) v += HM_LT()->ebits[cb->s[simt_ctx_index<L2>(x0 + (g >> (L2 - 2)), chroma, 0, 0)] ^ 0];
+      for (int c = 0; c < g; c++) v += HM_LT()->ebits[cb->s[simt_ctx_index<L2>(x0 + (c >> D::LSH), chroma, 0, 0)] ^ 1];
+      if (g < D::NGRP - 1) v += HM_LT()->ebits[cb->s[simt_ctx_index<L2>(x0 + (g >> D::LSH), chroma, 0, 0)] ^ 0];
       if (g > 3) v += 32768 * ((g - 2) >> 1);
     } else if (i < D::T_CBF) v = HM_LT()->ebits[cb->s[simt_ctx_index<L2>(D::X_CG + ((i - D::T_CG) >> 1), chroma, 0, 0)] ^ bin];
     else v = HM_LT()->ebits[cb->s[C_QT_CBF + cbfCtx] ^ bin];
-    S.A->tab[i] = v;
-  }
-  HM_PAR_FOR(i, 128) S.A->lps[i] = HM_NEXT_LPS[i];
+    S.tab()[i] = v;
+  }
+  HM_PAR_FOR(i, 128) S.lps()[i] = HM_NEXT_LPS[i];
   HM_PAR_FOR(i, D::NCTX * S.JOBS) {
     const int j = i / S.JOBS, k = i - j * S.JOBS;
-    if (k < jobs) S.A->ctx[j][k] = cb->s[simt_ctx_index<L2>(j, chroma, cbfCodeCtx, modeCtx)];
+    if (k < jobs) S.ctx(j, k) = cb->s[simt_ctx_index<L2>(j, chroma, cbfCodeCtx, modeCtx)];
   }
   S.load_scans(e);
   HM_SYNC();
 }
 template <int L2> HM_FINL void simt_store_contexts(const Simt<L2> &S, int k, Cabac *cb, int cbfCodeCtx)
 {
-  HM_PAR_FOR(j, SimtDim<L2>::NCTX) cb->s[simt_ctx_index<L2>(j, 0, cbfCodeCtx, C_INTRA_LUMA)] = S.A->ctx[j][k];
+  HM_PAR_FOR(j, SimtDim<L2>::NCTX) cb->s[simt_ctx_index<L2>(j, 0, cbfCodeCtx, C_INTRA_LUMA)] = S.ctx(j, k);
 }
 
 template <int L2> HM_DEV inline void simt_bin(const Shared *e, const Simt<L2> &S, int k, uint32_t *frac, int c, int bin)
 {
-  const int st = S.A->ctx[c][k];
+  const int st = S.ctx(c, k);
   *frac += (uint32_t)HM_LT()->ebits[st ^ bin];
-  S.A->ctx[c][k] = (uint8_t)(bin == (st & 1) ? (st < 124 ? st + 2 : st) : S.A->lps[st]);
-}
-HM_FINL int simt_cg_pattern(int cgBlkPos, int cgMask)
-{
-  const int cgx = cgBlkPos & 1, cgy = cgBlkPos >> 1;
-  const int sigRight = cgx < 1 ? ((cgMask >> (cgBlkPos + 1)) & 1) : 0, sigLower = cgy < 1 ? ((cgMask >> (cgBlkPos + 2)) & 1) : 0;
+  S.ctx(c, k) = (uint8_t)(bin == (st & 1) ? (st < 124 ? st + 2 : st) : S.lps()[st]);
+}
+template <int L2> HM_FINL int simt_cg_pattern(int cgBlkPos, int cgMask)
+{
+  const int W = SimtDim<L2>::WCG, cgx = cgBlkPos & (W - 1), cgy = cgBlkPos >> (L2 - 2);
+  const int sigRight = cgx < W - 1 ? ((cgMask >> (cgBlkPos + 1)) & 1) : 0, sigLower = cgy < W - 1 ? ((cgMask >> (cgBlkPos + W)) & 1) : 0;
   return sigRight + (sigLower << 1);
 }
 template <int L2> HM_FINL void simt_last_xy(int blkPos, int scanType, int *px, int *py)
@@ -110,26 +116,25 @@
 template <int L2> HM_DEV inline int simt_rdoq(const Simt<L2> &S, const SimtPar &p, int k, int scanType)
 {
   typedef SimtDim<L2> D;
-  const int32_t *tab = S.A->tab; const SimtPrices<L2> prices = { tab };
+  const int32_t *tab = S.tab(); const SimtPrices<L2> prices = { tab };
   const int qBits = p.qBits, half = 1 << (qBits - 1);
   const double lambda = p.lambda, errScale = p.errScale;
   const int firstCtx = first_sig_ctx(1 << L2, scanType, p.chroma), lumaSets = p.chroma ? 0 : 2;
   double blockUncoded = 0, baseCost = 0;
-  double cgSig1 = 0, cgSig2 = 0, cgSig3 = 0;
   int last = -1, cgLast = -1, ctxSet = 0;
-  int cgMask = 0, cgSets = 0;
+  int cgMask = 0; uint32_t cgSets = 0;
   LevelChain ch;
   for (int cg = D::NCG - 1; cg >= 0; cg--) {
-    const int cgBlkPos = S.cg_pos(scanType, cg), cgBit = 1 << cgBlkPos, pattern = simt_cg_pattern(cgBlkPos, cgMask);
+    const int cgBlkPos = S.cg_pos(scanType, cg), cgBit = 1 << cgBlkPos, pattern = simt_cg_pattern<L2>(cgBlkPos, cgMask);
     double sigCost = 0, sigCost0 = 0, codedLevelAndDist = 0, uncodedDist = 0; int nnzBeforePos0 = 0;
-    cgSets |= ctxSet << (2 * cg);
+    cgSets |= (uint32_t)ctxSet << (2 * cg);
     for (int q = 15; q >= 0; q--) {
       const int sp = cg * 16 + q;
       const int32_t lvlD = simt_level_double(S.cs(sp, k), p);
       uint32_t mx = (uint32_t)((lvlD + half) >> qBits); if (mx > 32767u) mx = 32767u;
       const double err = (double)lvlD, c0 = err * err * errScale;
       blockUncoded += c0;
-      if (mx > 0 && last < 0) { last = sp; cgLast = cg; ctxSet = cg > 0 ? lumaSets : 0; cgSets = ctxSet << (2 * cg); }
+      if (mx > 0 && last < 0) { last = sp; cgLast = cg; ctxSet = cg > 0 ? lumaSets : 0; cgSets = (uint32_t)ctxSet << (2 * cg); }
       uint32_t level = 0; double cSig = 0, cCoeff = c0;
       if (last >= 0) {
         const int isLast = (sp == last);
@@ -162,30 +167,26 @@
         uncodedDist += c0;
         if (q != 0) nnzBeforePos0++;
       }
-      S.B->dc[sp][k] = (int32_t)level;
+      S.put_dec(sp, k, level);
     }
     if (cgLast >= 0) {
       if (cg) {
         const int cgCtx = (pattern != 0) * 2;
-        double cgs = 0;
         if (!(cgMask & cgBit)) {
           const double r0 = lambda * (double)tab[D::T_CG + cgCtx];
           baseCost += r0 - sigCost;
-          cgs = r0;
         } else if (cg < cgLast) {
           if (nnzBeforePos0 == 0) { baseCost -= sigCost0; sigCost -= sigCost0; }
           double costZeroCG = baseCost;
           const double r0 = lambda * (double)tab[D::T_CG + cgCtx], r1 = lambda * (double)tab[D::T_CG + cgCtx + 1];
           baseCost += r1;
           costZeroCG += r0;
-          cgs = r1;
           costZeroCG += uncodedDist; costZeroCG -= codedLevelAndDist; costZeroCG -= sigCost;
           if (costZeroCG < baseCost) {
-            cgMask &= ~cgBit; baseCost = costZeroCG; cgs = r0;
-            for (int q = 15; q >= 0; q--) S.B->dc[cg * 16 + q][k] |= 0x40000000;
-          }
-        }
-        if (cg == 1) cgSig1 = cgs; else if (cg == 2) cgSig2 = cgs; else cgSig3 = cgs;
+            cgMask &= ~cgBit; baseCost = costZeroCG;
+            for (int q = 15; q >= 0; q--) S.mark_zeroed(cg * 16 + q, k);
+          }
+        }
       } else cgMask |= cgBit;
     }
   }
@@ -194,14 +195,15 @@
   baseCost += lambda * (double)tab[D::T_CBF + 1];
   int bestLastP1 = 0, found = 0;
   for (int cg = cgLast; cg >= 0 && !found; cg--) {
-    if (cg) baseCost -= (cg == 1 ? cgSig1 : (cg == 2 ? cgSig2 : cgSig3));
-    if (!((cgMask >> S.cg_pos(scanType, cg)) & 1)) continue;
-    const int wSet = (cgSets >> (2 * cg)) & 3, pattern = simt_cg_pattern(S.cg_pos(scanType, cg), cgMask); LevelChain walk;
+    const int cgBlkPos = S.cg_pos(scanType, cg), coded = (cgMask >> cgBlkPos) & 1, pattern = simt_cg_pattern<L2>(cgBlkPos, cgMask);
+    if (cg && cg < cgLast) baseCost -= lambda * (double)tab[D::T_CG + (pattern != 0) * 2 + coded];
+    if (!coded) continue;
+    const int wSet = (int)((cgSets >> (2 * cg)) & 3); LevelChain walk;
     for (int q = (cg == cgLast ? (last & 15) : 15); q >= 0; q--) {
-      const int sp = cg * 16 + q, lev = S.B->dc[sp][k] & 0xffff;
+      const int sp = cg * 16 + q, lev = S.dec(sp, k);
       const int si = sp == last ? 0 : S.sig_inc(scanType, firstCtx, pattern, sp, p.chroma);
       if (lev) {
-        int px, py; simt_last_xy<L2>(S.B->scan[scanType][sp], scanType, &px, &py);
+        int px, py; simt_last_xy<L2>(S.scan_pos(scanType, sp), scanType, &px, &py);
         const double costLast = lambda * (double)(tab[D::T_LASTX + hm_group_idx(px)] + tab[D::T_LASTY + hm_group_idx(py)]);
         const double cSig = (sp == last) ? 0.0 : lambda * (double)tab[D::T_SIG + si * 2 + 1];
         const double t1 = baseCost + costLast;
@@ -226,27 +228,27 @@
   }
   int absSum = 0;
   for (int sp = 0; sp < D::NC; sp++) {
-    const int v = S.B->dc[sp][k], dec = v & 0xffff, lv = (sp < bestLastP1 && !(v & 0x40000000)) ? dec : 0;
+    const int lv = (sp < bestLastP1 && !S.zeroed(sp, k)) ? S.dec(sp, k) : 0;
     absSum += lv;
-    S.B->dc[sp][k] = dec | (int32_t)((uint32_t)(S.cs(sp, k) < 0 ? -lv : lv) << 16);
+    S.put_lev(sp, k, S.cs(sp, k) < 0 ? -lv : lv);
   }
   if (absSum >= 2) {
     int lastCG = -1;
     for (int subSet = D::NCG - 1; subSet >= 0; subSet--) {
       const int subPos = subSet << 4;
       int lastNZ = -1, firstNZ = 16, parity = 0;
-      for (int q = 0; q < 16; q++) { const int lv = S.B->dc[subPos + q][k] >> 16; if (lv) { lastNZ = q; if (firstNZ == 16) firstNZ = q; } parity ^= lv & 1; }
+      for (int q = 0; q < 16; q++) { const int lv = S.lev(subPos + q, k); if (lv) { lastNZ = q; if (firstNZ == 16) firstNZ = q; } parity ^= lv & 1; }
       if (lastNZ >= 0 && lastCG == -1) lastCG = 1;
       if (lastNZ - firstNZ >= 4) {
-        const uint32_t signbit = (S.B->dc[subPos + firstNZ][k] >> 16) > 0 ? 0 : 1;
+        const uint32_t signbit = S.lev(subPos + firstNZ, k) > 0 ? 0 : 1;
         if (signbit != (uint32_t)parity) {
           const int64_t I64MAX = 0x7fffffffffffffffLL;
           int64_t minCostInc = I64MAX, curCost = I64MAX; int minK = -1, finalChange = 0, curChange = 0;
-          const int wSet = (cgSets >> (2 * subSet)) & 3; LevelChain walk;
+          const int wSet = (int)((cgSets >> (2 * subSet)) & 3); LevelChain walk;
           const int top = (subPos + 15 <= last) ? 15 : (last - subPos), kStart = (lastCG == 1 ? lastNZ : 15);
-          const int pattern = simt_cg_pattern(S.cg_pos(scanType, subSet), cgMask);
+          const int pattern = simt_cg_pattern<L2>(S.cg_pos(scanType, subSet), cgMask);
           for (int q = top; q >= 0; --q) {
-            const int v = S.B->dc[subPos + q][k]; const uint32_t dec = (uint32_t)(v & 0xffff); const int dv = v >> 16;
+            const uint32_t dec = (uint32_t)S.dec(subPos + q, k); const int dv = S.lev(subPos + q, k);
             const int ctxOne = 4 * wSet + walk.c1; const LevelChain at = walk;
             walk.step(dec);
             if (q > kStart) continue;
@@ -275,10 +277,10 @@
             if (curCost < minCostInc) { minCostInc = curCost; finalChange = curChange; minK = q; }
           }
           if (minK >= 0) {
-            const int v = S.B->dc[subPos + minK][k]; int mv = v >> 16;
+            int mv = S.lev(subPos + minK, k);
             if (mv == 32767 || mv == -32768) finalChange = -1;
             mv = (S.cs(subPos + minK, k) < 0) ? mv - finalChange : mv + finalChange;
-            S.B->dc[subPos + minK][k] = (v & 0xffff) | (int32_t)((uint32_t)mv << 16);
+            S.put_lev(subPos + minK, k, mv);
           }
         }
       }
@@ -293,15 +295,15 @@
   typedef SimtDim<L2> D;
   int last = -1, cgMask = 0;
   for (int sp = 0; sp < D::NC; sp++)
-    if ((S.B->dc[sp][src] >> 16) != 0) { last = sp; cgMask |= 1 << S.cg_pos(scanType, sp >> 4); }
+    if (S.lev(sp, src) != 0) { last = sp; cgMask |= 1 << S.cg_pos(scanType, sp >> 4); }
   {
-    int px, py; simt_last_xy<L2>(S.B->scan[scanType][last], scanType, &px, &py);
+    int px, py; simt_last_xy<L2>(S.scan_pos(scanType, last), scanType, &px, &py);
     const int gx = hm_group_idx(px), gy = hm_group_idx(py);
     int q;
-    for (q = 0; q < gx; q++) simt_bin(e, S, k, frac, D::X_LX + (q >> (L2 - 2)), 1);
-    if (gx < D::NGRP - 1) simt_bin(e, S, k, frac, D::X_LX + (q >> (L2 - 2)), 0);
-    for (q = 0; q < gy; q++) simt_bin(e, S, k, frac, D::X_LY + (q >> (L2 - 2)), 1);
-    if (gy < D::NGRP - 1) simt_bin(e, S, k, frac, D::X_LY + (q >> (L2 - 2)), 0);
+    for (q = 0; q < gx; q++) simt_bin(e, S, k, frac, D::X_LX + (q >> D::LSH), 1);
+    if (gx < D::NGRP - 1) simt_bin(e, S, k, frac, D::X_LX + (q >> D::LSH), 0);
+    for (q = 0; q < gy; q++) simt_bin(e, S, k, frac, D::X_LY + (q >> D::LSH), 1);
+    if (gy < D::NGRP - 1) simt_bin(e, S, k, frac, D::X_LY + (q >> D::LSH), 0);
     if (gx > 3) *frac += 32768u * (uint32_t)((gx - 2) >> 1);
     if (gy > 3) *frac += 32768u * (uint32_t)((gy - 2) >> 1);
   }
@@ -309,14 +311,14 @@
   int c1 = 1;
   for (int subSet = lastSet; subSet >= 0; subSet--) {
     const int subPos = subSet << 4, isLastSet = subSet == lastSet;
-    const int cgBlkPos = S.cg_pos(scanType, subSet), pattern = simt_cg_pattern(cgBlkPos, cgMask);
+    const int cgBlkPos = S.cg_pos(scanType, subSet), pattern = simt_cg_pattern<L2>(cgBlkPos, cgMask);
     if (isLastSet || subSet == 0) cgMask |= 1 << cgBlkPos;
     else simt_bin(e, S, k, frac, D::X_CG + (pattern != 0), (cgMask >> cgBlkPos) & 1);
     if (!((cgMask >> cgBlkPos) & 1)) continue;
     const int top = isLastSet ? (last & 15) : 15;
     int numNonZero = isLastSet ? 1 : 0, firstNZ = isLastSet ? top : 16, lastNZ = isLastSet ? top : -1;
     for (int q = isLastSet ? top - 1 : 15; q >= 0; q--) {
-      const int sig = (S.B->dc[subPos + q][src] >> 16) != 0;
+      const int sig = S.lev(subPos + q, src) != 0;
       if (q > 0 || subSet == 0 || numNonZero) simt_bin(e, S, k, frac, D::X_SIG + S.sig_inc(scanType, firstCtx, pattern, subPos + q, chroma), sig);
       if (sig) { numNonZero++; firstNZ = q; if (lastNZ < 0) lastNZ = q; }
     }
@@ -326,7 +328,7 @@
       c1 = 1;
       int firstC2 = -1, escape = 0, idx = 0;
       for (int q = lastNZ; q >= 0 && idx < 8; q--) {
-        const int a = hm_abs(S.B->dc[subPos + q][src] >> 16);
+        const int a = hm_abs(S.lev(subPos + q, src));
         if (!a) continue;
         const int sym = a > 1;
         simt_bin(e, S, k, frac, D::X_ONE + 4 * ctxSet + c1, sym);
@@ -334,13 +336,13 @@
         else if (c1 < 3 && c1 > 0) c1++;
         idx++;
       }
-      if (c1 == 0 && firstC2 != -1) { const int sym = hm_abs(S.B->dc[subPos + firstC2][src] >> 16) > 2; simt_bin(e, S, k, frac, D::X_ABS + ctxSet, sym); if (sym) escape = 1; }
+      if (c1 == 0 && firstC2 != -1) { const int sym = hm_abs(S.lev(subPos + firstC2, src)) > 2; simt_bin(e, S, k, frac, D::X_ABS + ctxSet, sym); if (sym) escape = 1; }
       escape = escape || (numNonZero > 8);
       *frac += 32768u * (uint32_t)(signHidden ? numNonZero - 1 : numNonZero);
       if (escape) {
         int firstCoeff2 = 1; uint32_t goRice = 0; idx = 0;
         for (int q = lastNZ; q >= 0; q--) {
-          const int a = hm_abs(S.B->dc[subPos + q][src] >> 16);
+          const int a = hm_abs(S.lev(subPos + q, src));
           if (!a) continue;
           const int baseLevel = (idx < 8) ? (2 + firstCoeff2) : 1;
           if (a >= baseLevel) {
diff --git a/hm-16.2_amd/csrc/hm355_simt16.h b/hm-16.2_amd/csrc/hm355_simt16.h
--- /dev/null
+++ b/hm-16.2_amd/csrc/hm355_simt16.h
@@ -0,0 +1,245 @@
+#pragma once
+
+#define HM_S16 4
+#define HM_S16T 17
+struct Simt16A {
+  union {
+    int32_t tile[2][16 * HM_S16T];
+    uint16_t dec[256][HM_S16];
+  };
+  int16_t cs[256][HM_S16];
+};
+struct Simt16B {
+  int16_t lev[256][HM_S16];
+  int32_t tab[SimtDim<4>::T_N];
+  double outCost[HM_S16];
+  uint32_t outDist[HM_S16], outFrac[HM_S16];
+  uint8_t ctx[SimtDim<4>::NCTX][HM_S16];
+  uint8_t outCbf[HM_S16];
+  uint8_t scanCG[16], scanIn[16];
+  uint8_t lps[128];
+};
+static_assert(sizeof(Simt16A) <= sizeof(((Shared *)0)->bufA), "Simt16A overlays bufA");
+static_assert(offsetof(RefLds, refMain) + sizeof(Simt16B) <= sizeof(((Shared *)0)->u), "Simt16B overlays the tail of the LDS union");
+static_assert(sizeof(((Simt16A *)0)->dec) <= sizeof(((Simt16A *)0)->tile) && offsetof(Simt16B, outCost) % 8 == 0, "the decision-time column lies under the tile");
+template <> struct Simt<4> {
+  enum { JOBS = HM_S16, KEEPS_COST = 0 };
+  Simt16A *A; Simt16B *B;
+  HM_FINL_M explicit Simt(Shared *e) : A((Simt16A *)e->bufA), B((Simt16B *)((char *)&e->u + offsetof(RefLds, refMain))) {}
+  HM_FINL_M int32_t *tab() const { return B->tab; }
+  HM_FINL_M uint8_t &ctx(int c, int k) const { return B->ctx[c][k]; }
+  HM_FINL_M uint8_t *lps() const { return B->lps; }
+  HM_FINL_M int scan_pos(int, int sp) const
+  {
+    const int cg = B->scanCG[sp >> 4], in = B->scanIn[sp & 15];
+    return ((cg >> 2) * 4 + (in >> 2)) * 16 + (cg & 3) * 4 + (in & 3);
+  }
+  HM_FINL_M void put_dec(int sp, int k, uint32_t level) const { A->dec[sp][k] = (uint16_t)level; }
+  HM_FINL_M void mark_zeroed(int sp, int k) const { A->dec[sp][k] |= 0x8000; }
+  HM_FINL_M int dec(int sp, int k) const { return A->dec[sp][k] & 0x7fff; }
+  HM_FINL_M int zeroed(int sp, int k) const { return A->dec[sp][k] & 0x8000; }
+  HM_FINL_M void put_lev(int sp, int k, int v) const { B->lev[sp][k] = (int16_t)v; }
+  HM_FINL_M int lev(int sp, int k) const { return B->lev[sp][k]; }
+  HM_FINL_M int cs(int sp, int k) const { return A->cs[sp][k]; }
+  HM_FINL_M int cg_pos(int, int cg) const { return B->scanCG[cg]; }
+  HM_FINL_M int sig_inc(int scanType, int firstCtx, int pattern, int sp, int chroma) const { return sig_ctx_inc(pattern, firstCtx, scan_pos(scanType, sp), 4, chroma); }
+  HM_FINL_M void keep_cost(int, int, double) const {}
+  HM_FINL_M double cost_at(int, int) const { return 0; }
+  HM_FINL_M void load_scans(const Shared *e) const
+  {
+    HM_PAR_FOR(q, 16) { B->scanCG[q] = (uint8_t)e->tab->scanCG[SCAN_DIAG][2][q]; B->scanIn[q] = (uint8_t)e->tab->scan[SCAN_DIAG][0][q]; }
+#ifdef HM355_HOSTSIM
+    static int checked;
+    if (!checked) { checked = 1; for (int i = 0; i < 256; i++) if (scan_pos(SCAN_DIAG, i) != e->tab->scan[SCAN_DIAG][2][i]) abort(); }
+#endif
+  }
+};
+typedef Simt<4> Simt16;
+
+#ifdef HM355_HOSTSIM
+#include <stdio.h>
+struct Simt16Stats {
+  unsigned long cand[8], batches[4];
+  ~Simt16Stats()
+  {
+    if (!getenv("HM355_S16_STATS")) return;
+    fprintf(stderr, "s16 candidates"); for (int i = 0; i < 8; i++) fprintf(stderr, " %lu", cand[i]);
+    fprintf(stderr, "\ns16 batches"); for (int i = 0; i < 4; i++) fprintf(stderr, " %lu", batches[i]);
+    fprintf(stderr, "\n");
+  }
+};
+static Simt16Stats g_s16_stats;
+#endif
+
+template <class Pred> HM_FINL void s16_residual_fwd(const Simt16 &S, const Pel *org, int ps, int bitDepth, int job, Pred pred)
+{
+  Simt16A *A = S.A;
+  const int s1 = 4 + bitDepth + 6 - 15, a1 = 1 << (s1 - 1), s2 = 10, a2 = 512;
+  HM_PAR_FOR(l, 256) { const int y = l >> 4, x = l & 15; A->tile[0][y * HM_S16T + x] = org[y * ps + x] - pred(x, y); }
+  HM_SYNC();
+  HM_PAR_FOR(l, 256) {
+    const int j = l >> 4, kk = l & 15; int32_t acc = 0;
+    for (int i = 0; i < 16; i++) acc += HM_LT()->tmat[(kk * 2) * HM_TSTRIDE + i] * A->tile[0][j * HM_S16T + i];
+    A->tile[1][kk * HM_S16T + j] = (acc + a1) >> s1;
+  }
+  HM_SYNC();
+  HM_PAR_FOR(l, 256) {
+    const int blkPos = S.scan_pos(SCAN_DIAG, l), kk = blkPos >> 4, j = blkPos & 15; int32_t acc = 0;
+    for (int i = 0; i < 16; i++) acc += HM_LT()->tmat[(kk * 2) * HM_TSTRIDE + i] * A->tile[1][j * HM_S16T + i];
+    A->cs[l][job] = (int16_t)((acc + a2) >> s2);
+  }
+  HM_SYNC();
+}
+HM_FINL void s16_dequant_inv1(const Simt16 &S, const SimtPar &p, int job, int cbf, TCoeff *coef)
+{
+  Simt16A *A = S.A;
+  if (cbf) {
+    HM_PAR_FOR(l, 256) {
+      const int lv = S.lev(l, job), blk = S.scan_pos(SCAN_DIAG, l);
+      if (coef) coef[blk] = lv;
+      A->tile[0][(blk >> 4) * HM_S16T + (blk & 15)] = simt_dequant(p, lv);
+    }
+    HM_SYNC();
+    HM_PAR_FOR(l, 256) {
+      const int j = l >> 4, i = l & 15; int32_t acc = 0;
+      for (int kk = 0; kk < 16; kk++) acc += HM_LT()->tmat[(kk * 2) * HM_TSTRIDE + i] * A->tile[0][kk * HM_S16T + j];
+      A->tile[1][j * HM_S16T + i] = hm_clip3(-32768, 32767, (acc + 64) >> 7);
+    }
+    HM_SYNC();
+  } else if (coef) { HM_PAR_FOR(l, 256) coef[l] = 0; }
+}
+template <class Pred, class Out> HM_FINL void s16_inv2_recon(const Simt16 &S, int bitDepth, int cbf, Pred pred, Out out)
+{
+  const int maxv = (1 << bitDepth) - 1, is2 = 20 - bitDepth;
+  HM_PAR_FOR(l, 256) {
+    const int j = l >> 4, i = l & 15; int resi = 0;
+    if (cbf) {
+      int32_t acc = 0;
+      for (int kk = 0; kk < 16; kk++) acc += HM_LT()->tmat[(kk * 2) * HM_TSTRIDE + i] * S.A->tile[1][kk * HM_S16T + j];
+      resi = hm_clip3(-32768, 32767, (acc + (1 << (is2 - 1))) >> is2);
+    }
+    out(i, j, hm_clip3(0, maxv, pred(i, j) + resi));
+  }
+}
+HM_FINL void sn_dequant_inv1(const Simt8 &S, const SimtPar &p, int job, int cbf, TCoeff *coef, int scanType) { s8_dequant_inv1(S, p, scanType, job, cbf, coef); }
+HM_FINL void sn_dequant_inv1(const Simt16 &S, const SimtPar &p, int job, int cbf, TCoeff *coef, int) { s16_dequant_inv1(S, p, job, cbf, coef); }
+template <class Pred, class Out> HM_FINL void sn_inv2_recon(const Simt8 &S, int bitDepth, int cbf, Pred pred, Out out) { s8_inv2_recon(S, bitDepth, cbf, pred, out); }
+template <class Pred, class Out> HM_FINL void sn_inv2_recon(const Simt16 &S, int bitDepth, int cbf, Pred pred, Out out) { s16_inv2_recon(S, bitDepth, cbf, pred, out); }
+HM_FINL uint8_t *sn_out_cbf(const Simt8 &S) { return S.A->outCbf; }
+HM_FINL uint8_t *sn_out_cbf(const Simt16 &S) { return S.B->outCbf; }
+HM_FINL uint32_t *sn_out_dist(const Simt8 &S) { return S.A->outDist; }
+HM_FINL uint32_t *sn_out_dist(const Simt16 &S) { return S.B->outDist; }
+HM_FINL uint32_t *sn_out_frac(const Simt8 &S) { return S.A->outFrac; }
+HM_FINL uint32_t *sn_out_frac(const Simt16 &S) { return S.B->outFrac; }
+
+HM_DEV HM_NOINLINE int simt16_luma_first_pass(Shared *e, TU tv, int numModes)
+{
+  HM_ENTRY(e); numModes = HM_UNI(numModes); tv = hm_uni_struct(tv);
+  const TU *t = &tv;
+  const int ps = e->stride[0], bitDepth = e->bitDepth;
+  const Simt16 S(e); Simt16B *B = S.B;
+  uint32_t commonFrac;
+  {
+    CabacR r; cabr_load(e, r, &e->cur);
+    r.frac &= 32767;
+    if (e->im) { code_skip_flag(e, &r, t->cuZ); enc_bin(e, &r, C_PRED_MODE, 1); }
+    enc_bin(e, &r, C_SUBDIV + 1, 0);
+    commonFrac = (uint32_t)r.frac;
+  }
+  simt_setup(e, S, &e->cur, numModes < HM_S16 ? numModes : HM_S16, 0, 1, 1, C_INTRA_LUMA);
+  const SimtPar p = simt_params<4>(e, 0);
+  const Pel *org = e->fb.org[0] + (e->ctuY * 64 + t->y) * ps + e->ctuX * 64 + t->x;
+  const int dcVal = ref_dc_val(e, 0, 16), shiftSse = (bitDepth - 8) << 1;
+  double bestCost = HM_MAX_DOUBLE; int keep = -1, best = 0;
+#ifdef HM355_HOSTSIM
+  int batchesRun = 0;
+#endif
+  for (int c0 = 0; c0 < numModes;) {
+    const int room = keep < 0 ? HM_S16 : HM_S16 - 1, nb = numModes - c0 < room ? numModes - c0 : room;
+    if (keep >= 0) {
+      HM_PAR_FOR(i, SimtDim<4>::NCTX * HM_S16) {
+        const int j = i / HM_S16, k = i - j * HM_S16;
+        if (k != keep) S.ctx(j, k) = e->cur.s[simt_ctx_index<4>(j, 0, 1, C_INTRA_LUMA)];
+      }
+      HM_SYNC();
+    }
+    for (int i = 0; i < nb; i++) {
+      const int slot = i + (keep >= 0 && i >= keep), mode = HM_UNI(e->rdModeList[c0 + i]);
+      s16_residual_fwd(S, org, ps, bitDepth, slot, [&](int x, int y) HM_LAMBDA_INL { return pred_sample(e, mode, 16, 4, x, y, dcVal, bitDepth); });
+    }
+    HM_WAVE_FOR(k) {
+      const int i = (keep >= 0 && k > keep) ? k - 1 : k;
+      if (k < HM_S16 && k != keep && i < nb) B->outCbf[k] = (uint8_t)(simt_rdoq(S, p, k, SCAN_DIAG) > 0);
+    }
+    HM_SYNC();
+    for (int i = 0; i < nb; i++) {
+      const int slot = i + (keep >= 0 && i >= keep), mode = HM_UNI(e->rdModeList[c0 + i]), cbf = HM_UNI(B->outCbf[slot]);
+      s16_dequant_inv1(S, p, slot, cbf, (TCoeff *)0);
+      uint32_t sse = 0;
+      s16_inv2_recon(S, bitDepth, cbf, [&](int x, int y) HM_LAMBDA_INL { return pred_sample(e, mode, 16, 4, x, y, dcVal, bitDepth); },
+                     [&](int x, int y, int r) HM_LAMBDA_INL { const int d = org[y * ps + x] - r; sse += (uint32_t)((d * d) >> shiftSse); });
+      const uint32_t dist = hm_wave_sum(sse);
+      if (hm_lane() == 0) B->outDist[slot] = dist;
+      HM_SYNC();
+    }
+    HM_WAVE_FOR(k) {
+      const int i = (keep >= 0 && k > keep) ? k - 1 : k;
+      if (k < HM_S16 && k != keep && i < nb) {
+        const int mode = e->rdModeList[c0 + i], cbf = B->outCbf[k];
+        uint32_t frac = commonFrac;
+        simt_luma_mode_bits(e, S, k, &frac, mode);
+        simt_bin(e, S, k, &frac, SimtDim<4>::X_CBF, cbf);
+        if (cbf) simt_code_coeff(e, S, k, k, 0, SCAN_DIAG, &frac);
+        B->outFrac[k] = frac;
+        B->outCost[k] = calc_rd_cost(e, frac >> 15, B->outDist[k]);
+      }
+    }
+    HM_SYNC();
+    int slotBest = keep;
+    for (int i = 0; i < nb; i++) {
+      const int slot = i + (keep >= 0 && i >= keep); const double v = B->outCost[slot];
+      if (v < bestCost) { bestCost = v; slotBest = slot; best = c0 + i; }
+    }
+    keep = HM_UNI(slotBest); best = HM_UNI(best);
+    c0 += nb;
+#ifdef HM355_HOSTSIM
+    batchesRun++;
+#endif
+  }
+#ifdef HM355_HOSTSIM
+  g_s16_stats.cand[numModes < 7 ? numModes : 7]++; g_s16_stats.batches[batchesRun < 3 ? batchesRun : 3]++;
+#endif
+  const int bestMode = HM_UNI(e->rdModeList[best]);
+  e->s8Winner = keep | (best << 8);
+  HM_SYNC();
+  return bestMode;
+}
+
+template <int L2> HM_DEV HM_NOINLINE void simt_luma_winner_as_single_tu(Shared *e, TU tv)
+{
+  HM_ENTRY(e); tv = hm_uni_struct(tv);
+  const TU *t = &tv; WorkSpace *ws = e->ws;
+  const Simt<L2> S(e);
+  const int won = HM_UNI(e->s8Winner), best = won & 255, z = t->cuZ + t->relZ, ps = e->stride[0], bitDepth = e->bitDepth;
+  const int mode = HM_UNI(e->rdModeList[won >> 8]), cbf = HM_UNI(sn_out_cbf(S)[best]);
+  const SimtPar p = simt_params<L2>(e, 0);
+  const int dcVal = ref_dc_val(e, 0, 1 << L2);
+  Pel *rq = ws->qtRec[5 - L2] + t->y * 64 + t->x;
+  Pel *recPic = e->fb.rec[0] + (e->ctuY * 64 + t->y) * ps + e->ctuX * 64 + t->x;
+  sn_dequant_inv1(S, p, best, cbf, ws->qtCoef[5 - L2] + z * 16, L2 == 3 ? intra_scan_type(mode) : SCAN_DIAG);
+  sn_inv2_recon(S, bitDepth, cbf, [&](int x, int y) HM_LAMBDA_INL { return pred_sample(e, mode, 1 << L2, L2, x, y, dcVal, bitDepth); },
+                [&](int x, int y, int rr) HM_LAMBDA_INL { rq[y * 64 + x] = (Pel)rr; recPic[y * ps + x] = (Pel)rr; });
+  HM_SYNC();
+  {
+    CabacR r; cabr_load(e, r, &e->cur);
+    r.frac &= 32767;
+    if (e->im) { code_skip_flag(e, &r, t->cuZ); enc_bin(e, &r, C_PRED_MODE, 1); }
+    if (L2 == 3) enc_bin(e, &r, C_PART, 1);
+    enc_bin(e, &r, C_SUBDIV + 5 - L2, 0);
+    cabr_store(r, &e->cur);
+  }
+  simt_store_contexts(S, best, &e->cur, 1);
+  e->cur.frac = (uint64_t)sn_out_frac(S)[best];
+  e->outDistY = sn_out_dist(S)[best]; e->outBits = sn_out_frac(S)[best] >> 15; e->outDist = (uint32_t)cbf;
+  HM_SYNC();
+}
diff --git a/hm-16.2_amd/csrc/hm355_simt4.h b/hm-16.2_amd/csrc/hm355_simt4.h
--- a/hm-16.2_amd/csrc/hm355_simt4.h
+++ b/hm-16.2_amd/csrc/hm355_simt4.h
@@ -35,6 +35,16 @@
   enum { JOBS = HM_SL, KEEPS_COST = 1 };
   Simt4A *A; Simt4B *B;
   HM_FINL_M explicit Simt(Shared *e) : A((Simt4A *)e->bufA), B((Simt4B *)((char *)&e->u + offsetof(RefLds, refMain))) {}
+  HM_FINL_M int32_t *tab() const { return A->tab; }
+  HM_FINL_M uint8_t &ctx(int c, int k) const { return A->ctx[c][k]; }
+  HM_FINL_M uint8_t *lps() const { return A->lps; }
+  HM_FINL_M int scan_pos(int scanType, int sp) const { return B->scan[scanType][sp]; }
+  HM_FINL_M void put_dec(int sp, int k, uint32_t level) const { B->dc[sp][k] = (int32_t)level; }
+  HM_FINL_M void mark_zeroed(int sp, int k) const { B->dc[sp][k] |= 0x40000000; }
+  HM_FINL_M int dec(int sp, int k) const { return B->dc[sp][k] & 0xffff; }
+  HM_FINL_M int zeroed(int sp, int k) const { return B->dc[sp][k] & 0x40000000; }
+  HM_FINL_M void put_lev(int sp, int k, int v) const { B->dc[sp][k] = (B->dc[sp][k] & 0xffff) | (int32_t)((uint32_t)v << 16); }
+  HM_FINL_M int lev(int sp, int k) const { return B->dc[sp][k] >> 16; }
   HM_FINL_M int cs(int sp, int k) const { return B->cs[sp][k]; }
   HM_FINL_M int cg_pos(int, int) const { return 0; }
   HM_FINL_M int sig_inc(int scanType, int, int, int sp, int) const { return B->sigIdx[scanType][sp]; }
diff --git a/hm-16.2_amd/csrc/hm355_simt8.h b/hm-16.2_amd/csrc/hm355_simt8.h
--- a/hm-16.2_amd/csrc/hm355_simt8.h
+++ b/hm-16.2_amd/csrc/hm355_simt8.h
@@ -22,6 +22,16 @@
   enum { JOBS = HM_S8, KEEPS_COST = 0 };
   Simt8A *A; Simt8B *B;
   HM_FINL_M explicit Simt(Shared *e) : A((Simt8A *)e->bufA), B((Simt8B *)((char *)&e->u + offsetof(RefLds, refMain))) {}
+  HM_FINL_M int32_t *tab() const { return A->tab; }
+  HM_FINL_M uint8_t &ctx(int c, int k) const { return A->ctx[c][k]; }
+  HM_FINL_M uint8_t *lps() const { return A->lps; }
+  HM_FINL_M int scan_pos(int scanType, int sp) const { return B->scan[scanType][sp]; }
+  HM_FINL_M void put_dec(int sp, int k, uint32_t level) const { B->dc[sp][k] = (int32_t)level; }
+  HM_FINL_M void mark_zeroed(int sp, int k) const { B->dc[sp][k] |= 0x40000000; }
+  HM_FINL_M int dec(int sp, int k) const { return B->dc[sp][k] & 0xffff; }
+  HM_FINL_M int zeroed(int sp, int k) const { return B->dc[sp][k] & 0x40000000; }
+  HM_FINL_M void put_lev(int sp, int k, int v) const { B->dc[sp][k] = (B->dc[sp][k] & 0xffff) | (int32_t)((uint32_t)v << 16); }
+  HM_FINL_M int lev(int sp, int k) const { return B->dc[sp][k] >> 16; }
   HM_FINL_M int cs(int sp, int k) const { return A->cs[sp][k]; }
   HM_FINL_M int cg_pos(int scanType, int cg) const { return B->scanCG[scanType][cg]; }
   HM_FINL_M int sig_inc(int scanType, int firstCtx, int pattern, int sp, int chroma) const { return sig_ctx_inc(pattern, firstCtx, B->scan[scanType][sp], 3, chroma); }
@@ -140,7 +150,7 @@
   for (int c = 0; c < numModes; c++) { const double v = A->outCost[c]; if (v < bestCost) { bestCost = v; best = c; } }
   best = HM_UNI(best);
   const int bestMode = e->rdModeList[best];
-  e->s8Winner = best;
+  e->s8Winner = best | (best << 8);
   HM_SYNC();
   return bestMode;
 }
@@ -221,32 +231,3 @@
   HM_SYNC();
   return bestDist;
 }
-
-HM_DEV HM_NOINLINE void simt8_luma_winner_as_single_tu(Shared *e, TU tv)
-{
-  HM_ENTRY(e); tv = hm_uni_struct(tv);
-  const TU *t = &tv; WorkSpace *ws = e->ws;
-  const Simt8 S(e); Simt8A *A = S.A;
-  const int best = HM_UNI(e->s8Winner), z = t->cuZ + t->relZ, ps = e->stride[0], bitDepth = e->bitDepth;
-  const int mode = e->rdModeList[best], cbf = A->outCbf[best];
-  const SimtPar p = simt_params<3>(e, 0);
-  const int dcVal = ref_dc_val(e, 0, 8);
-  Pel *rq = ws->qtRec[2] + t->y * 64 + t->x;
-  Pel *recPic = e->fb.rec[0] + (e->ctuY * 64 + t->y) * ps + e->ctuX * 64 + t->x;
-  s8_dequant_inv1(S, p, intra_scan_type(mode), best, cbf, ws->qtCoef[2] + z * 16);
-  s8_inv2_recon(S, bitDepth, cbf, [&](int x, int y) HM_LAMBDA_INL { return pred_sample(e, mode, 8, 3, x, y, dcVal, bitDepth); },
-                [&](int x, int y, int rr) HM_LAMBDA_INL { rq[y * 64 + x] = (Pel)rr; recPic[y * ps + x] = (Pel)rr; });
-  HM_SYNC();
-  {
-    CabacR r; cabr_load(e, r, &e->cur);
-    r.frac &= 32767;
-    if (e->im) { code_skip_flag(e, &r, t->cuZ); enc_bin(e, &r, C_PRED_MODE, 1); }
-    enc_bin(e, &r, C_PART, 1);
-    enc_bin(e, &r, C_SUBDIV + 2, 0);
-    cabr_store(r, &e->cur);
-  }
-  simt_store_contexts(S, best, &e->cur, 1);
-  e->cur.frac = (uint64_t)A->outFrac[best];
-  e->outDistY = A->outDist[best]; e->outBits = A->outFrac[best] >> 15; e->outDist = (uint32_t)cbf;
-  HM_SYNC();
-}
```

After: 25940, median of 6. 1.02x the previous value.
